# JGI-Bioinformatics/Kmernator

Measured on AMD Instinct MI355X. Metric: total k-mers/sec at k=31, 150 bp reads (spectrum build, inputs resident in HBM), higher is better.
Workload: dtype u64

## Files before the change

kmernator_amd/csrc/kmr_api.hip:

```cpp
#include <hip/hip_runtime.h>
#include <dlfcn.h>
#include <unistd.h>
#include <rccl/rccl.h>

#include <algorithm>
#include <atomic>
#include <cmath>
#include <cstdio>
#include <cstdlib>
#include <cstring>
#include <cctype>
#include <memory>
#include <mutex>
#include <string>
#include <type_traits>
#include <vector>

#include "../../include/kmernator_amd.h"
#include "kmr_kernels.hpp"
#include "kmr_partition.hpp"
#include "kmr_ingest.hpp"
#include "kmr_artifact.hpp"
#include "kmr_select.hpp"
#include "kmr_pairs.hpp"
#include "kmr_dedup.hpp"
#include "kmr_dump.hpp"
#include "kmr_superkmer.hpp"
#include "kmr_buckets.hpp"
#include "kmr_synth.hpp"
#define KMR_INSTANCES_EXTERN
#include "kmr_instances.hpp"

using namespace kmr;

namespace {

std::string g_create_error;

thread_local char g_oom_note[160] = "";
std::atomic<long long> g_blocks_live{0};
hipError_t dev_malloc(void **p, size_t bytes) {
	hipError_t e = hipMalloc(p, bytes);
	if (e == hipSuccess) { if (*p) g_blocks_live++; return e; }
	if (e != hipErrorOutOfMemory) return e;
	size_t fr = 0, tot = 0;
	for (int attempt = 0; attempt < 6; attempt++) {
		(void)hipGetLastError();
		hipDeviceSynchronize();
		if (hipMemGetInfo(&fr, &tot) != hipSuccess || bytes > tot) break;
		usleep(20000u << attempt);
		e = hipMalloc(p, bytes);
		if (e == hipSuccess && *p) g_blocks_live++;
		if (e != hipErrorOutOfMemory) return e;
	}
	(void)hipGetLastError();
	hipMemGetInfo(&fr, &tot);
	snprintf(g_oom_note, sizeof(g_oom_note), " [requested %.3f GB; device has %.3f GB free of %.3f GB]", bytes / 1e9, fr / 1e9, tot / 1e9);
	*p = nullptr;
	return hipErrorOutOfMemory;
}

class DevBuf {
public:
	DevBuf() = default;
	DevBuf(DevBuf &&o) noexcept : p_(o.p_), cap_(o.cap_) { o.p_ = nullptr; o.cap_ = 0; }
	DevBuf &operator=(DevBuf &&o) noexcept { if (this != &o) { reset(); std::swap(p_, o.p_); std::swap(cap_, o.cap_); } return *this; }
	~DevBuf() { reset(); }
	void reset() { if (p_) { hipFree(p_); g_blocks_live--; } p_ = nullptr; cap_ = 0; }
	hipError_t alloc(size_t bytes) {
		reset();
		void *p = nullptr;
		const hipError_t e = dev_malloc(&p, bytes);
		if (e == hipSuccess) { p_ = p; cap_ = bytes; }
		return e;
	}
	int reserve(kmr_handle *h, const char *what, size_t need, size_t bytes = 0);
	template <class T = void> T *get() const { return (T *)p_; }
	size_t cap() const { return cap_; }
	explicit operator bool() const { return p_ != nullptr; }
private:
	void *p_ = nullptr;
	size_t cap_ = 0;
};

struct DevMap {
	uint64_t nb = 0, n = 0;
	DevBuf start;
	DevBuf keys;
	DevBuf vals;
	DevBuf sweight;
	DevBuf spkt;
	DevBuf image;
	bool present = false;
};

struct HostPool {
	DevBuf base, chunk_list, chunk_count, head;
	uint32_t cap = 0; size_t chunk_bytes = 0;
	uint64_t used_ub = 0;
	uint64_t presize = 0;
};

struct HandleMem {
	DevBuf slots, extslots;
	DevBuf dP, dstats, derr;
	DevMap weak, sing;
	DevBuf ix_start, ix_keys, ix_counts;
	DevBuf scratch_stats;
	DevBuf adopt_buf;
	DevBuf trk;
	DevBuf scan_sums;
	DevBuf score_buf;
	DevBuf lut;
	DevBuf dPk;
	DevBuf d_uni;
	DevBuf qrange;
	DevBuf sk_fine_state;
	struct Early { bool active = false; uint64_t hi = 0; uint32_t min_depth = 0; DevBuf ue, cursor, fc, err; } early;
	DevBuf dedup_tab;
	DevBuf xo_dev;
};
struct BuildMem {
	DevBuf sk_state;
	HostPool l1;
	DevBuf work_counter;
	DevBuf l1_state; bool l1_state_dirty = false;
	DevBuf arena; size_t arena_used = 0, arena_want = 0; std::vector<DevBuf> arena_overflow;
	DevBuf linear;
	DevBuf tile_count, kcap, koff;
	DevBuf ucnt, ufirst, u_start, u_end, u_read, umax;
	DevBuf tb_bases, tb_quals, tb_rel, tb_off, tb_len;
	uint64_t tb_quals_filled = 0; int tb_quals_char = -1;
	DevBuf tb_stage[2][8];
	DevBuf uw_keys, uw_vals, us_keys, us_b8, us_pkt;
	DevBuf ue, ue2;
};
struct ExchangeMem {
	DevBuf xc_small, xc_dcounts;
	DevBuf xc_send, xc_send2, xc_recv, xc_recv2;
};

}

struct Tuning {
	uint64_t target_list = 2048;
	uint64_t sub_batch_bases = 0;
	int recycle = -1;
	int part_blocks = 0;
	double entry_share = -1.0;
	double early_entry_share = -1.0;
	uint64_t saturated_batch_bytes = 0;
	bool no_lut = false, no_narrow = false, no_l1_state = false, no_stream_lookups = false;
	uint64_t long_list_chunks = 0;
	uint64_t binned_min = 1ull << 18;
	uint64_t twobit_piece_bases = 0;
	uint64_t list_aim = 0;
	bool pow2_lists = false;
	bool no_packed_direct = false;
	bool no_uniform_count = false;
	bool no_lean_extract = false;
	bool exchange_fail_once = false;
	uint64_t dump_piece_bytes = 0;
	bool dump_timing = false;
	bool select_timing = false;
	bool pairs_timing = false;
	bool dedup_timing = false;
	uint32_t pair_hash_bits = 64;
	bool no_coarse_lists = true;
};

struct kmr_handle : HandleMem, BuildMem, ExchangeMem {
	kmr_config cfg;
	Tuning tune;
	uint32_t k = 0, kb = 0, hkb = 0, W = 0;
	bool ext = false;
	int device = 0, ncu = 0;
	hipStream_t stream = nullptr;
	std::string err;
	uint32_t log2cap = 0;
	uint64_t occupied = 0;
	uint64_t pending_kmers = 0;
	uint64_t stream_base = 0, reads = 0;
	uint64_t nb_weak = 0, nb_sing = 0;
	bool finalized = false, has_singletons = true;
	kmr_handle *subtract = nullptr;
	uint64_t subtracted = 0;
	kmr_stats stats;
	bool partition_mode = false;
	bool superkmer_mode = false;
	uint64_t ix_lists = 0, ix_gen = ~0ull;
	uint64_t trk_n = 0; std::vector<uint64_t> trk_elems;
	long trk_next = 128; uint64_t trk_raw = 0, trk_good = 0; std::vector<unsigned long long> trk_bounds; std::vector<uint64_t> trk_snap_raw, trk_snap_good;
	bool sk_fast_div = false;
	bool sender_launch = false;
	bool sk_exchange = false;
	bool auto_mode = false;
	int bits1 = 0;
	uint64_t inserted_records = 0;
	uint64_t call_bases_hint = 0;
	uint32_t lut_log2 = 0;
	uint64_t lut_gen = ~0ull, map_gen = 0;
	hipStream_t tb_copy_stream = nullptr; hipEvent_t tb_ready[2] = {nullptr, nullptr}, tb_consumed[2] = {nullptr, nullptr}; bool tb_set_used[2] = {false, false};
	const SkPacked *packed_direct = nullptr;
	int uniform_q_hint = -1;
	uint32_t sk_bits = 0, sk_m = 0, sk_off = 0, sk_win = 0;
	double hP[256], hPk[256];
	uint32_t sk_uni_w = 0xffffffffu; bool sk_uni_mixed = false; bool last_count_uniform = false;
	uint32_t peer_uni_w = 0xffffffffu; bool peer_uni_mixed = false, peers_declare = false;
	uint64_t xr_lo = 0, xr_hi = ~0ull;
	uint64_t last_early_hi = 0, last_early_entries = 0;
	bool last_early_overflowed = false;
	double last_score_ms = 0, last_select_ms = 0, last_write_ms = 0;
	double last_dump_size_ms = 0, last_dump_write_ms = 0;
	double last_pairs_ms = 0, last_pairs_parse_ms = 0, last_pairs_sort_ms = 0;
	double last_dedup_ms = 0, last_dedup_key_ms = 0, last_dedup_sort_ms = 0, last_dedup_consensus_ms = 0;
	uint64_t last_pair_hash_collisions = 0;
	uint64_t last_saturated_keys = 0, last_saturated_batches = 0;
	bool qual_mixed = false;
	uint32_t sk_fine_shift = 0;
	uint32_t sk_min_override = 0;
	uint64_t xo_segcap = 0; std::vector<uint64_t> xo_counts; const void *xo_batch = nullptr; uint64_t xo_first = 0;
	void *xc_comm = nullptr; kmr_transport xc_tr = {nullptr, nullptr, nullptr};
	uint64_t xc_job_bases = 0, xc_bytes_to_peers = 0;
	hipEvent_t ev0 = nullptr, ev1 = nullptr;
	double ms[KMR_TIME_GROUPS] = {0};
	uint64_t launches[KMR_TIME_GROUPS] = {0};
	std::vector<std::pair<hipEvent_t, hipEvent_t> > pending_events[KMR_TIME_GROUPS];
};

struct kmr_picks {
	int device = 0;
	DevBuf text, picked;
	uint64_t n = 0, n_picked = 0, bytes = 0;
};

struct kmr_pairs {
	int device = 0;
	DevBuf mate, read1, read2;
	uint64_t n = 0, n_pairs = 0, n_full = 0, n_seq = 0, n_conflicts = 0;
};

struct kmr_text {
	int device = 0;
	DevBuf text;
	uint64_t kept = 0, bytes = 0;
};

struct kmr_dedup {
	int device = 0;
	DevBuf disc, group_first, group_size, names;
	kmr_reads *cons = nullptr;
	uint64_t n = 0, n_groups = 0, affected = 0, name_bytes = 0;
	uint64_t skipped[4] = {0, 0, 0, 0};
};

struct kmr_reads {
	int device = 0;
	DevBuf bases, quals;
	DevBuf offsets;
	DevBuf name_off, name_len;
	uint64_t n = 0, total = 0, filtered = 0;
	uint32_t input_base = 0;
};

namespace {

std::string oom_note() { std::string s(g_oom_note); g_oom_note[0] = 0; return s; }

std::string hip_err_text(hipError_t e) { return std::string(hipGetErrorString(e)) + (e == hipErrorOutOfMemory ? oom_note() : std::string()); }

#define HIPCHK(h, call) do { hipError_t e_ = (call); if (e_ != hipSuccess) { \
	(h)->err = std::string(#call) + ": " + hip_err_text(e_); \
	return e_ == hipErrorOutOfMemory ? KMR_ERR_OOM : KMR_ERR_HIP; } } while (0)

int DevBuf::reserve(kmr_handle *h, const char *what, size_t need, size_t bytes) {
	if (p_ && cap_ >= need) return 0;
	if (!bytes) bytes = need;
	hipError_t e = p_ ? hipStreamSynchronize(h->stream) : hipSuccess;
	if (e == hipSuccess) e = alloc(bytes);
	if (e == hipSuccess) return 0;
	h->err = std::string("device buffer ") + what + " (" + std::to_string(bytes) + " bytes): " + hip_err_text(e);
	return e == hipErrorOutOfMemory ? KMR_ERR_OOM : KMR_ERR_HIP;
}

#ifdef KMR_DEBUG_HOOKS
bool dbg() { static const bool d = getenv("KMR_DEBUG") != nullptr; return d; }
#else
constexpr bool dbg() { return false; }
#endif

int fail(kmr_handle *h, int code, const std::string &msg) { const std::string m = code == KMR_ERR_OOM ? msg + oom_note() : msg; if (h) h->err = m; else g_create_error = m; return code; }

uint64_t min_pow2(uint64_t n) {
	uint64_t p = n;
	if (p == 0) p = 1;
	else if ((p & (p - 1)) != 0) { p--; for (size_t i = 1; i < 64; i <<= 1) p |= p >> i; p++; }
	return p;
}
uint64_t resize_buckets(uint64_t n) { if (n > 67108864ull) n = 67108864ull; return min_pow2(n); }

void quality_table(double P[256], unsigned minQ, unsigned startChar) {
	for (int raw = 0; raw < 256; raw++) {
		int i = raw - (int)startChar + 33;
		if (i < 33 + (int)minQ) P[raw] = 0.0;
		else if (i < 103) P[raw] = 1.0 - pow(10.0, ((33 - i) / 10.0));
		else P[raw] = 1.0;
	}
}

template <int N> using int_c = std::integral_constant<int, N>;
template <class F> auto with_w(const kmr_handle *h, F &&f) {
	switch (h->W) { case 1: return f(int_c<1>()); case 2: return f(int_c<2>()); case 3: return f(int_c<3>()); default: return f(int_c<4>()); }
}
template <class F> auto with_w_ext(const kmr_handle *h, F &&f) {
	return with_w(h, [&](auto W) { return h->ext ? f(W, std::true_type()) : f(W, std::false_type()); });
}
template <int W, class F> auto with_win(uint32_t win, F &&f) {
	if (W > 1 && win == 32) return f(int_c<(W > 1 ? 32 : 16)>());
	return win == 16 ? f(int_c<16>()) : (win == 8 ? f(int_c<8>()) : f(int_c<4>()));
}

size_t slot_bytes(kmr_handle *h) { return with_w(h, [](auto W) { return sizeof(Slot<W()>); }); }

ReadsView reads_view(const void *bases, const void *quals, const void *offsets, uint64_t n_reads, const void *discarded = nullptr, uint64_t stream_base = 0, uint64_t first_read_idx = 0) {
	ReadsView rv{};
	rv.bases = (const uint8_t *)bases; rv.quals = (const uint8_t *)quals; rv.offsets = (const uint64_t *)offsets; rv.discarded = (const uint8_t *)discarded;
	rv.n_reads = n_reads; rv.stream_base = stream_base; rv.first_read_idx = first_read_idx;
	return rv;
}
ReadsView reads_slice(const ReadsView &all, uint64_t r, uint64_t m) {
	ReadsView rv = all;
	rv.offsets = all.offsets + r; rv.n_reads = m; rv.discarded = all.discarded ? all.discarded + r : nullptr; rv.first_read_idx = all.first_read_idx + r;
	return rv;
}
FinalizeParams finalize_params(kmr_handle *h, uint32_t min_depth) {
	FinalizeParams f{};
	f.kb = h->hkb; f.ext_min_q = h->cfg.ext_min_quality; f.min_depth = min_depth; f.has_singletons = h->cfg.separate_singletons ? 1 : 0; f.nb_weak = h->nb_weak; f.nb_sing = h->nb_sing;
	return f;
}

DevParams dev_params(kmr_handle *h) {
	DevParams p;
	p.k = h->k; p.kb = h->hkb; p.min_weight = h->cfg.min_weight; p.fastq_start = h->cfg.fastq_start_char; p.ext_min_q = h->cfg.ext_min_quality;
	p.qzero = h->cfg.fastq_start_char + std::max<uint32_t>(1u, h->cfg.min_quality_score);
	p.subsample = h->cfg.kmer_subsample; p.rank = h->cfg.rank; p.world = h->cfg.world_size; p.num_parts = h->cfg.num_parts; p.part_idx = h->cfg.part_idx;
	p.count_sender_bad = h->sender_launch ? 1u : 0u;
	p.P = h->dP.get<double>(); p.stats = h->dstats.get<DevStats>(); p.err = h->derr.get<uint32_t>();
	p.sub_wstart = p.sub_wkeys = p.sub_sstart = p.sub_skeys = nullptr; p.sub_wvals = nullptr; p.sub_sweight = nullptr; p.sub_wnb = p.sub_snb = 0; p.sub_vw = 0;
	if (h->subtract) {
		const kmr_handle *o = h->subtract;
		if (o->weak.present && o->weak.n) { p.sub_wstart = o->weak.start.get<uint64_t>(); p.sub_wkeys = o->weak.keys.get<uint64_t>(); p.sub_wvals = o->weak.vals.get<uint32_t>(); p.sub_wnb = o->weak.nb; p.sub_vw = o->ext ? 15 : 3; }
		if (o->sing.present && o->sing.n) { p.sub_sstart = o->sing.start.get<uint64_t>(); p.sub_skeys = o->sing.keys.get<uint64_t>(); p.sub_sweight = o->sing.sweight.get<uint8_t>(); p.sub_snb = o->sing.nb; }
	}
	return p;
}

int grid_for(uint64_t n, int block = 256, int maxBlocks = 256 * 16) {
	uint64_t g = (n + block - 1) / block;
	if (g < 1) g = 1;
	if (g > (uint64_t)maxBlocks) g = maxBlocks;
	return (int)g;
}

// ... 4 lines not shown
	HIPCHK(h, hipGetLastError());
	return 0;
}
int clear_table_any(kmr_handle *h, void *slots, ExtSlot *ext, uint32_t log2cap) { return with_w(h, [&](auto W) { return clear_table<W()>(h, slots, ext, log2cap); }); }

int alloc_table(kmr_handle *h, uint32_t log2cap, DevBuf &slots, DevBuf &ext) {
	DevBuf s, x;
	HIPCHK(h, s.alloc(slot_bytes(h) << log2cap));
	if (h->ext) HIPCHK(h, x.alloc(sizeof(ExtSlot) << log2cap));
	const int rc = clear_table_any(h, s.get(), x.get<ExtSlot>(), log2cap);
	if (rc) return rc;
	slots = std::move(s); ext = std::move(x);
	return 0;
}

int sync_state(kmr_handle *h) {
	HIPCHK(h, hipStreamSynchronize(h->stream));
	for (int which = 0; which < KMR_TIME_GROUPS; which++) {
		for (auto &pr : h->pending_events[which]) {
			float ms = 0; hipEventElapsedTime(&ms, pr.first, pr.second);
			h->ms[which] += ms; h->launches[which]++;
			hipEventDestroy(pr.first); hipEventDestroy(pr.second);
		}
		h->pending_events[which].clear();
	}
	uint32_t e = 0; DevStats s;
	HIPCHK(h, hipMemcpy(&e, h->derr.get<uint32_t>(), sizeof(e), hipMemcpyDeviceToHost));
	HIPCHK(h, hipMemcpy(&s, h->dstats.get<DevStats>(), sizeof(s), hipMemcpyDeviceToHost));
#ifdef KMR_DEBUG_HOOKS
	if (h->superkmer_mode) { if (dbg()) fprintf(stderr, "sk_extract windows: %llu general, %llu fast\n", s.claimed, s.inserted); s.claimed = 0; s.inserted = 0; }
#endif
	h->stats.raw_kmers = s.raw + s.inserted + s.sender_bad; h->stats.raw_good_kmers = s.good + s.inserted; h->stats.discarded = s.raw - s.good + s.sender_bad;
	h->occupied = s.claimed; h->pending_kmers = 0; h->subtracted = s.subtracted;
	if (e & ERR_READ_TOO_LONG) return fail(h, KMR_ERR_UNSUPPORTED, "a read is longer than the per-wavefront LDS tile (" + std::to_string(TILE_SPAN) + " bases)");
	if (e & ERR_TABLE_FULL) return fail(h, KMR_ERR_CAPACITY, "device k-mer table is full; raise kmr_config.max_table_entries / estimated_raw_kmers");
	if (e & ERR_SEGMENT_OVERFLOW) return fail(h, KMR_ERR_CAPACITY, "an owner segment overflowed seg_capacity");
	if (e & ERR_POOL_FULL) return fail(h, KMR_ERR_CAPACITY, "record pool overflow (internal sizing error)");
	if (e & ERR_ENTRIES_FULL) return fail(h, KMR_ERR_CAPACITY, "entry buffer overflow (internal sizing error)");
	return 0;
}

template <int W, bool EXT> int grow_table_t(kmr_handle *h, uint32_t newlog) {
	DevBuf ns, ne;
	int rc = alloc_table(h, newlog, ns, ne);
	if (rc) return rc;
	Table<W> src = table_of<W>(h), dst; dst.slots = ns.get<Slot<W>>(); dst.ext = ne.get<ExtSlot>(); dst.log2cap = newlog;
	hipLaunchKernelGGL((rehash_kernel<W, EXT>), dim3(grid_for(1ull << h->log2cap)), dim3(256), 0, h->stream, src, dst, h->hkb, h->derr.get<uint32_t>());
	HIPCHK(h, hipGetLastError());
	HIPCHK(h, hipStreamSynchronize(h->stream));
	h->slots = std::move(ns); h->extslots = std::move(ne); h->log2cap = newlog;
	return 0;
}
int grow_table(kmr_handle *h, uint32_t newlog) { return with_w_ext(h, [&](auto W, auto EXT) { return grow_table_t<W(), EXT()>(h, newlog); }); }

int ensure_capacity(kmr_handle *h, uint64_t incoming) {
	const uint64_t cap = 1ull << h->log2cap;
	if ((double)(h->occupied + h->pending_kmers + incoming) <= 0.85 * (double)cap) { h->pending_kmers += incoming; return 0; }
	int rc = sync_state(h);
	if (rc) return rc;
	if ((double)(h->occupied + incoming) > 0.85 * (double)cap) {
		uint32_t nl = h->log2cap;
		while ((double)(h->occupied + incoming) > 0.6 * (double)(1ull << nl)) nl++;
		rc = grow_table(h, nl);
		if (rc) return rc;
	}
	h->pending_kmers = incoming;
	return 0;
}

void time_begin(kmr_handle *h, int which, hipEvent_t *a, hipEvent_t *b) {
	hipEventCreate(a); hipEventCreate(b);
	hipEventRecord(*a, h->stream);
	(void)which;
}
void time_end(kmr_handle *h, int which, hipEvent_t a, hipEvent_t b) {
	hipEventRecord(b, h->stream);
	h->pending_events[which].push_back(std::make_pair(a, b));
}

const size_t EXTRACT_SMEM = (size_t)WAVES_PER_BLOCK * 2 * TILE_BUF;

int exclusive_scan(kmr_handle *h, const uint32_t *in, uint64_t n, uint64_t *out);

int prepare_units(kmr_handle *h, ReadsView &rv, uint32_t span = (uint32_t)TILE_SPAN) {
	rv.u_start = rv.u_end = rv.u_read = nullptr; rv.n_units = 0;
	const uint64_t n = rv.n_reads;
	if (n == 0) return 0;
	int rc = h->umax.reserve(h, "umax", 4); if (rc) return rc;
	HIPCHK(h, hipMemsetAsync(h->umax.get<unsigned int>(), 0, 4, h->stream));
	rc = h->ucnt.reserve(h, "ucnt", 4 * (n + 1)); if (rc) return rc;
	hipLaunchKernelGGL(unit_count_kernel, dim3(grid_for(n)), dim3(256), 0, h->stream, rv.offsets, n, h->k, span, h->ucnt.get<uint32_t>(), h->umax.get<unsigned int>());
	HIPCHK(h, hipGetLastError());
	unsigned int mx = 0;
	HIPCHK(h, hipMemcpyAsync(&mx, h->umax.get<unsigned int>(), 4, hipMemcpyDeviceToHost, h->stream));
	HIPCHK(h, hipStreamSynchronize(h->stream));
	if (mx <= span) return 0;
	rc = h->ufirst.reserve(h, "ufirst", 8 * (n + 1)); if (rc) return rc;
	rc = exclusive_scan(h, h->ucnt.get<uint32_t>(), n, h->ufirst.get<uint64_t>()); if (rc) return rc;
	uint64_t U = 0;
	HIPCHK(h, hipMemcpy(&U, h->ufirst.get<uint64_t>() + n, 8, hipMemcpyDeviceToHost));
	if (h->u_read.cap() < 8 * U) {
		h->u_start.reset(); h->u_end.reset(); h->u_read.reset();
		HIPCHK(h, h->u_start.alloc(8 * U)); HIPCHK(h, h->u_end.alloc(8 * U)); HIPCHK(h, h->u_read.alloc(8 * U));
	}
	hipLaunchKernelGGL(unit_fill_kernel, dim3(grid_for(n)), dim3(256), 0, h->stream, rv.offsets, n, h->k, span, h->ufirst.get<uint64_t>(), h->u_start.get<uint64_t>(), h->u_end.get<uint64_t>(), h->u_read.get<uint64_t>());
	HIPCHK(h, hipGetLastError());
	rv.u_start = h->u_start.get<uint64_t>(); rv.u_end = h->u_end.get<uint64_t>(); rv.u_read = h->u_read.get<uint64_t>(); rv.n_units = U;
	return 0;
}

template <int W, bool EXT, class Op> int launch_extract(kmr_handle *h, const ReadsView &rv, const Op &op, uint64_t max_blocks = 0) {
	const DevParams dp = dev_params(h);
	const bool sub = Op::NEEDS_WEIGHT && (dp.sub_wnb | dp.sub_snb) != 0;
	auto kern = sub ? extract_kernel<W, EXT, Op, true> : extract_kernel<W, EXT, Op, false>;
	HIPCHK(h, hipFuncSetAttribute((const void *)kern, hipFuncAttributeMaxDynamicSharedMemorySize, (int)EXTRACT_SMEM));
	if (dbg()) { int nb = 0; hipOccupancyMaxActiveBlocksPerMultiprocessor(&nb, (const void *)kern, WAVES_PER_BLOCK * 64, EXTRACT_SMEM); fprintf(stderr, "extract: %d blocks of %d waves per CU (dynamic LDS %zu)\n", nb, WAVES_PER_BLOCK, EXTRACT_SMEM);
		for (size_t tr : {(size_t)79872, (size_t)65536, (size_t)52000, (size_t)38000}) { hipOccupancyMaxActiveBlocksPerMultiprocessor(&nb, (const void *)kern, WAVES_PER_BLOCK * 64, tr); fprintf(stderr, "   with %zu bytes: %d blocks\n", tr, nb); } }
	const uint64_t tiles = ((rv.u_start ? rv.n_units : rv.n_reads) + 63) / 64;
	uint64_t blocks = (tiles + WAVES_PER_BLOCK - 1) / WAVES_PER_BLOCK;
	if (blocks == 0) return 0;
	if (max_blocks && blocks > max_blocks) blocks = max_blocks;
	if (blocks > 0x7fffffffull) return fail(h, KMR_ERR_INVALID_ARG, "too many reads in one batch");
	hipLaunchKernelGGL(kern, dim3((unsigned)blocks), dim3(WAVES_PER_BLOCK * 64), EXTRACT_SMEM, h->stream, rv, dp, op);
	HIPCHK(h, hipGetLastError());
	return 0;
}

template <int W, bool EXT> int add_reads_dev_t(kmr_handle *h, const ReadsView &rvAll, uint64_t total_bases) {
	const uint64_t n = rvAll.n_reads;
	const uint64_t avg = n ? std::max<uint64_t>(1, total_bases / n) : 1;
	uint64_t chunk = std::max<uint64_t>(64, ((1ull << 27) / avg) & ~63ull);
	std::vector<uint64_t> off2(2);
	for (uint64_t r = 0; r < n; r += chunk) {
		const uint64_t m = std::min(chunk, n - r);
		HIPCHK(h, hipMemcpyAsync(&off2[0], rvAll.offsets + r, 8, hipMemcpyDeviceToHost, h->stream));
		HIPCHK(h, hipMemcpyAsync(&off2[1], rvAll.offsets + r + m, 8, hipMemcpyDeviceToHost, h->stream));
		HIPCHK(h, hipStreamSynchronize(h->stream));
		const uint64_t bases = off2[1] - off2[0];
		int rc = ensure_capacity(h, bases);
		if (rc) return rc;
		ReadsView rv = reads_slice(rvAll, r, m);
		rc = prepare_units(h, rv); if (rc) return rc;
		InsertOp<W, EXT> op; op.table = table_of<W>(h);
		hipEvent_t a, b; time_begin(h, 0, &a, &b);
		rc = launch_extract<W, EXT>(h, rv, op);
		time_end(h, 0, a, b);
		if (rc) return rc;
	}
	return 0;
}

int add_reads_dev_any(kmr_handle *h, const ReadsView &rv, uint64_t total_bases) { return with_w_ext(h, [&](auto W, auto EXT) { return add_reads_dev_t<W(), EXT()>(h, rv, total_bases); }); }

int exclusive_scan(kmr_handle *h, const uint32_t *in, uint64_t n, uint64_t *out ) {
	const uint64_t nblocks = (n + SCAN_ITEMS - 1) / SCAN_ITEMS;
	const size_t eb = sizeof(unsigned long long);
	int rc = h->scan_sums.reserve(h, "scan_sums", eb * (nblocks + 1), eb * std::max<uint64_t>(nblocks + 1, 4096)); if (rc) return rc;
	unsigned long long *sums = h->scan_sums.get<unsigned long long>(), *total = sums + nblocks;
	hipLaunchKernelGGL(scan_block_sums_kernel, dim3((unsigned)nblocks), dim3(256), 0, h->stream, in, n, sums);
	hipLaunchKernelGGL(scan_sums_kernel, dim3(1), dim3(256), 0, h->stream, sums, nblocks, total);
	hipLaunchKernelGGL(scan_apply_kernel, dim3((unsigned)nblocks), dim3(256), 0, h->stream, in, n, sums, out);
	HIPCHK(h, hipGetLastError());
	HIPCHK(h, hipStreamSynchronize(h->stream));
	return 0;
}

int arena_alloc(kmr_handle *h, void **out, size_t bytes) {
	const size_t need = (bytes + 255) & ~(size_t)255;
	if (h->arena && h->arena_used + need <= h->arena.cap()) { *out = h->arena.get<uint8_t>() + h->arena_used; h->arena_used += need; h->arena_want += need; return 0; }
	h->arena_want += need;
	DevBuf b;
	HIPCHK(h, b.alloc(std::max<size_t>(need, 256)));
	*out = b.get();
	h->arena_overflow.push_back(std::move(b));
	return 0;
}
int arena_reset(kmr_handle *h) {
	HIPCHK(h, hipStreamSynchronize(h->stream));
	h->arena_overflow.clear();
	if (h->arena_want > h->arena.cap()) {
		if (h->arena.alloc(h->arena_want + h->arena_want / 8 + (1 << 20)) != hipSuccess) (void)hipGetLastError();
	}
	h->arena_used = 0; h->arena_want = 0;
	return 0;
}
template <class T> int arena_get(kmr_handle *h, T **out, size_t count) { return arena_alloc(h, (void **)out, count * sizeof(T)); }

void clear_map(DevMap &m) { m.image.reset(); m.n = 0; m.present = false; }


template <int W> MapView<W> view_of(const DevMap &m, uint32_t vw) {
	MapView<W> v; v.start = m.start.get<uint64_t>(); v.keys = m.keys.get<uint64_t>(); v.vals = m.vals.get<uint32_t>(); v.sweight = m.sweight.get<uint8_t>(); v.nb = m.present ? m.nb : 0; v.vw = vw;
	return v;
}

template <int W, bool EXT> int finalize_t(kmr_handle *h, uint32_t min_depth) {
	int rc = sync_state(h);
	if (rc) return rc;
	hipEvent_t ea, eb; time_begin(h, 1, &ea, &eb);
	const FinalizeParams f = finalize_params(h, min_depth);
	const bool keepSing = f.has_singletons && min_depth <= 1;
	DevBuf wcb, scb, fcb;
	HIPCHK(h, wcb.alloc(4 * h->nb_weak)); HIPCHK(h, scb.alloc(4 * h->nb_sing)); HIPCHK(h, fcb.alloc(sizeof(FinalizeCounters)));
	uint32_t *wc = wcb.get<uint32_t>(), *sc = scb.get<uint32_t>(); FinalizeCounters *fc = fcb.get<FinalizeCounters>();
	HIPCHK(h, hipMemsetAsync(wc, 0, 4 * h->nb_weak, h->stream)); HIPCHK(h, hipMemsetAsync(sc, 0, 4 * h->nb_sing, h->stream)); HIPCHK(h, hipMemsetAsync(fc, 0, sizeof(FinalizeCounters), h->stream));
	Table<W> t = table_of<W>(h);
	const int g = grid_for(1ull << h->log2cap);
	hipLaunchKernelGGL(classify_kernel<W>, dim3(g), dim3(256), 0, h->stream, t, f, wc, sc, fc);
	HIPCHK(h, hipGetLastError());
	FinalizeCounters c;
	HIPCHK(h, hipMemcpyAsync(&c, fc, sizeof(c), hipMemcpyDeviceToHost, h->stream));
	HIPCHK(h, hipStreamSynchronize(h->stream));
	h->stats.unique_kmers = c.unique;
	h->stats.singleton_kmers = f.has_singletons ? c.singletons : 0;
	DevMap &wm = h->weak, &sm = h->sing;
	wm = DevMap(); sm = DevMap();
	wm.nb = h->nb_weak; wm.n = c.weak_kept; wm.present = true;
	sm.nb = h->nb_sing; sm.n = c.sing_kept; sm.present = keepSing;
	const uint32_t vw = EXT ? 15 : 3;
	HIPCHK(h, wm.start.alloc(8 * (wm.nb + 1))); HIPCHK(h, sm.start.alloc(8 * (sm.nb + 1)));
	rc = exclusive_scan(h, wc, wm.nb, wm.start.get<uint64_t>()); if (rc) return rc;
	rc = exclusive_scan(h, sc, sm.nb, sm.start.get<uint64_t>()); if (rc) return rc;
	HIPCHK(h, wm.keys.alloc(std::max<uint64_t>(8, 8ull * W * wm.n))); HIPCHK(h, wm.vals.alloc(std::max<uint64_t>(8, 4ull * vw * wm.n)));
	HIPCHK(h, sm.keys.alloc(std::max<uint64_t>(8, 8ull * W * sm.n))); HIPCHK(h, sm.sweight.alloc(std::max<uint64_t>(8, sm.n)));
	if (EXT) HIPCHK(h, sm.spkt.alloc(std::max<uint64_t>(8, 4ull * sm.n)));
	HIPCHK(h, hipMemsetAsync(wc, 0, 4 * h->nb_weak, h->stream)); HIPCHK(h, hipMemsetAsync(sc, 0, 4 * h->nb_sing, h->stream));
	hipLaunchKernelGGL((scatter_kernel<W, EXT>), dim3(g), dim3(256), 0, h->stream, t, f, wm.start.get<uint64_t>(), wc, wm.keys.get<uint64_t>(), wm.vals.get<uint32_t>(), sm.start.get<uint64_t>(), sc, sm.keys.get<uint64_t>(), sm.sweight.get<uint8_t>(), sm.spkt.get<uint32_t>());
	HIPCHK(h, hipGetLastError());
	SortView<W> sv; sv.keys = wm.keys.get<uint64_t>(); sv.vals = wm.vals.get<uint32_t>(); sv.b8 = nullptr; sv.pkt = nullptr; sv.vw = vw;
	hipLaunchKernelGGL((sort_buckets_kernel<W, EXT ? 15 : 3>), dim3(grid_for(wm.nb, 4, 1 << 20)), dim3(256), 0, h->stream, sv, wm.start.get<uint64_t>(), wm.nb);
	if (sm.n) {
		SortView<W> ss; ss.keys = sm.keys.get<uint64_t>(); ss.vals = nullptr; ss.b8 = sm.sweight.get<uint8_t>(); ss.pkt = sm.spkt.get<uint32_t>(); ss.vw = 0;
		hipLaunchKernelGGL((sort_buckets_kernel<W, 0>), dim3(grid_for(sm.nb, 4, 1 << 20)), dim3(256), 0, h->stream, ss, sm.start.get<uint64_t>(), sm.nb);
	}
	HIPCHK(h, hipGetLastError());
	time_end(h, 1, ea, eb);
	HIPCHK(h, hipStreamSynchronize(h->stream));
	h->has_singletons = keepSing;
	if (!keepSing) { sm.n = 0; }
	h->stats.weak_entries = wm.n; h->stats.singleton_entries = keepSing ? sm.n : 0;
	h->finalized = true; h->map_gen++;
	return sync_state(h);
}

template <int W> int build_image_t(kmr_handle *h, DevMap &m, bool weakMap) {
	if (m.image) return 0;
	const uint32_t vw = h->ext ? 15 : 3;
	const uint32_t vbytes = weakMap ? (h->ext ? 60 : 12) : (h->ext ? 5 : 1);
	HIPCHK(h, m.image.alloc(8 * (2 + m.nb) + 4 * m.nb + m.n * (h->kb + vbytes)));
	hipLaunchKernelGGL(image_header_kernel, dim3(grid_for(m.nb)), dim3(256), 0, h->stream, m.image.get<uint8_t>(), m.start.get<uint64_t>(), m.nb, h->kb, vbytes);
	if (m.n) hipLaunchKernelGGL(image_entries_kernel<W>, dim3(grid_for(m.n)), dim3(256), 0, h->stream, m.image.get<uint8_t>(), m.start.get<uint64_t>(), m.nb, h->kb, vbytes,
	                           m.keys.get<uint64_t>(), weakMap ? m.vals.get<uint32_t>() : nullptr, vw, m.sweight.get<uint8_t>(), m.spkt.get<uint32_t>(), m.n);
	HIPCHK(h, hipGetLastError());
	HIPCHK(h, hipStreamSynchronize(h->stream));
	return 0;
}
int build_image(kmr_handle *h, DevMap &m, bool weakMap) { return with_w(h, [&](auto W) { return build_image_t<W()>(h, m, weakMap); }); }

template <int W> int load_image_t(kmr_handle *h, DevMap &m, bool weakMap, const uint8_t *src, uint64_t len) {
	if (len < 16) return fail(h, KMR_ERR_INVALID_ARG, "image too short");
	uint64_t nb, mask; memcpy(&nb, src, 8); memcpy(&mask, src + 8, 8);
	if (nb == 0 || (nb & (nb - 1)) || mask != nb - 1 || len < 8 * (2 + nb) + 4 * nb) return fail(h, KMR_ERR_INVALID_ARG, "bad image header");
	const uint32_t vw = h->ext ? 15 : 3;
	const uint32_t vbytes = weakMap ? (h->ext ? 60 : 12) : (h->ext ? 5 : 1);
	if ((len - 8 * (2 + nb) - 4 * nb) % (h->kb + vbytes) != 0) return fail(h, KMR_ERR_INVALID_ARG, "image size does not match k / value type");
	m = DevMap();
	m.nb = nb; m.n = (len - 8 * (2 + nb) - 4 * nb) / (h->kb + vbytes); m.present = true;
	const uint64_t *offs = (const uint64_t *)(src + 16);
	uint64_t expect = 8 * (2 + nb);
	for (uint64_t b = 0; b < nb; b++) {
		if (offs[b] != expect || expect + 4 > len) return fail(h, KMR_ERR_INVALID_ARG, "image offsets are not the packed store() layout");
		uint32_t cnt; memcpy(&cnt, src + expect, 4);
		expect += 4 + (uint64_t)cnt * (h->kb + vbytes);
		if (expect > len) return fail(h, KMR_ERR_INVALID_ARG, "image bucket runs past the end");
	}
	if (expect != len) return fail(h, KMR_ERR_INVALID_ARG, "image length mismatch");
	HIPCHK(h, m.image.alloc(len));
	HIPCHK(h, hipMemcpy(m.image.get<uint8_t>(), src, len, hipMemcpyHostToDevice));
	{
		DevBuf counts; HIPCHK(h, counts.alloc(4 * nb));
		hipLaunchKernelGGL(image_counts_kernel, dim3(grid_for(nb)), dim3(256), 0, h->stream, m.image.get<uint8_t>(), nb, counts.get<uint32_t>());
		HIPCHK(h, m.start.alloc(8 * (nb + 1)));
		int rc = exclusive_scan(h, counts.get<uint32_t>(), nb, m.start.get<uint64_t>()); if (rc) return rc;
	}
	HIPCHK(h, m.keys.alloc(std::max<uint64_t>(8, 8ull * W * m.n)));
	if (weakMap) HIPCHK(h, m.vals.alloc(std::max<uint64_t>(8, 4ull * vw * m.n)));
	else { HIPCHK(h, m.sweight.alloc(std::max<uint64_t>(8, m.n))); if (h->ext) HIPCHK(h, m.spkt.alloc(std::max<uint64_t>(8, 4 * m.n))); }
	if (m.n) hipLaunchKernelGGL(image_unpack_kernel<W>, dim3(grid_for(m.n)), dim3(256), 0, h->stream, m.image.get<uint8_t>(), m.start.get<uint64_t>(), nb, h->kb, vbytes, m.keys.get<uint64_t>(), m.vals.get<uint32_t>(), vw, m.sweight.get<uint8_t>(), m.spkt.get<uint32_t>(), m.n);
	SortView<W> sv; sv.keys = m.keys.get<uint64_t>(); sv.vals = m.vals.get<uint32_t>(); sv.b8 = m.sweight.get<uint8_t>(); sv.pkt = m.spkt.get<uint32_t>(); sv.vw = weakMap ? vw : 0;
	if (!weakMap) hipLaunchKernelGGL((sort_buckets_kernel<W, 0>), dim3(grid_for(nb, 4, 1 << 20)), dim3(256), 0, h->stream, sv, m.start.get<uint64_t>(), nb);
	else if (h->ext) hipLaunchKernelGGL((sort_buckets_kernel<W, 15>), dim3(grid_for(nb, 4, 1 << 20)), dim3(256), 0, h->stream, sv, m.start.get<uint64_t>(), nb);
	else hipLaunchKernelGGL((sort_buckets_kernel<W, 3>), dim3(grid_for(nb, 4, 1 << 20)), dim3(256), 0, h->stream, sv, m.start.get<uint64_t>(), nb);
	HIPCHK(h, hipGetLastError());
	HIPCHK(h, hipStreamSynchronize(h->stream));
	m.image.reset();

	return 0;
}

template <int W, int VW> void launch_sort(kmr_handle *h, DevMap &m, bool weakMap) {
	SortView<W> sv; sv.keys = m.keys.get<uint64_t>(); sv.vals = weakMap ? m.vals.get<uint32_t>() : nullptr; sv.b8 = m.sweight.get<uint8_t>(); sv.pkt = m.spkt.get<uint32_t>(); sv.vw = weakMap ? VW : 0;
	hipLaunchKernelGGL((sort_buckets_kernel<W, VW>), dim3(grid_for(m.nb, 4, 1 << 20)), dim3(256), 0, h->stream, sv, m.start.get<uint64_t>(), m.nb);
}
template <int W> int merge_image_t(kmr_handle *h, DevMap &m, bool weakMap, const uint8_t *src, uint64_t len) {
	DevMap t;
	int rc = load_image_t<W>(h, t, weakMap, src, len);
	if (rc) return rc;
	if (t.nb != m.nb) return fail(h, KMR_ERR_INVALID_ARG, "Can not merge two maps of differing sizes (src/Kmer.h:3210)");
	const uint32_t vw = h->ext ? 15 : 3;
	DevMap d; d.nb = m.nb; d.n = m.n + t.n; d.present = true;
	DevBuf countsb, dupb;
	HIPCHK(h, countsb.alloc(4 * m.nb)); HIPCHK(h, dupb.alloc(4));
	uint32_t *counts = countsb.get<uint32_t>(), *dup = dupb.get<uint32_t>();
	HIPCHK(h, hipMemsetAsync(dup, 0, 4, h->stream));
	HIPCHK(h, d.start.alloc(8 * (m.nb + 1)));
// ... 40 lines not shown
	return 0;
}

template <int W> LutView<W> lut_of(kmr_handle *h) {
	LutView<W> v; v.slots = nullptr; v.mask = 0; v.shift = 0;
	if (h->tune.no_lut || !h->weak.present || h->weak.n == 0) return v;
	if (!(h->lut && h->lut_gen == h->map_gen)) {
		uint32_t l2 = 10; while ((1ull << l2) < 2 * h->weak.n) l2++;
		const size_t bytes = (size_t)(W + 1) * 8 << l2;
		if (h->lut.cap() < bytes) {
			if (h->lut) { hipStreamSynchronize(h->stream); h->lut.reset(); }
			size_t fr = 0, tot = 0;
			if (hipMemGetInfo(&fr, &tot) != hipSuccess || fr < bytes + (1ull << 30) || h->lut.alloc(bytes) != hipSuccess) { (void)hipGetLastError(); return v; }
		}

		const uint32_t vw = h->ext ? 15 : 3;
		hipLaunchKernelGGL(lut_clear_kernel, dim3(4096), dim3(256), 0, h->stream, h->lut.get<uint64_t>(), 1ull << l2, (uint32_t)(W + 1));
		hipLaunchKernelGGL(lut_build_kernel<W>, dim3(grid_for(h->weak.n)), dim3(256), 0, h->stream, view_of<W>(h->weak, vw), h->weak.n, h->lut.get<uint64_t>(), (1ull << l2) - 1, 64 - l2, h->hkb);
		if (hipGetLastError() != hipSuccess) return v;
		h->lut_log2 = l2; h->lut_gen = h->map_gen;
	}
	v.slots = h->lut.get<uint64_t>(); v.mask = (1ull << h->lut_log2) - 1; v.shift = 64 - h->lut_log2;
	return v;
}

template <int W> int lookup_reads_t(kmr_handle *h, const ReadsView &rv, uint32_t *dout, const uint64_t *dout_off, bool weak_only = false) {
	LookupOp<W> op; const uint32_t vw = h->ext ? 15 : 3; op.weak_only = weak_only;
	op.lut = weak_only ? lut_of<W>(h) : LutView<W>{nullptr, 0, 0};
	op.weak = view_of<W>(h->weak, vw); op.sing = view_of<W>(h->sing, vw); op.out = dout; op.out_offsets = dout_off; op.first_read_idx = rv.first_read_idx;
	return launch_extract<W, false>(h, rv, op);
}
template <int W> int lookup_reads_weighted_t(kmr_handle *h, const ReadsView &rv, double *dout, const uint64_t *dout_off) {
	LookupWeightOp<W> op; const uint32_t vw = h->ext ? 15 : 3;
	op.weak = view_of<W>(h->weak, vw); op.sing = view_of<W>(h->sing, vw); op.out = dout; op.out_offsets = dout_off; op.first_read_idx = rv.first_read_idx;
	return launch_extract<W, false>(h, rv, op);
}

int stage_reads(kmr_handle *h, const char *bases, const uint64_t *offsets, uint64_t n, DevBuf &b, DevBuf &o) {
	const uint64_t total = n ? offsets[n] - offsets[0] : 0;
	HIPCHK(h, b.alloc(total + 64)); HIPCHK(h, o.alloc(8 * (n + 1)));
	HIPCHK(h, hipMemcpyAsync(b.get(), bases + (n ? offsets[0] : 0), total, hipMemcpyHostToDevice, h->stream));
	std::vector<uint64_t> rel(n + 1);
	for (uint64_t i = 0; i <= n; i++) rel[i] = n ? offsets[i] - offsets[0] : 0;
	HIPCHK(h, hipMemcpyAsync(o.get(), rel.data(), 8 * (n + 1), hipMemcpyHostToDevice, h->stream));
	HIPCHK(h, hipStreamSynchronize(h->stream));
	return 0;
}


#define TARGET_LIST_RECORDS (h->tune.target_list)
const double MAX_LIST_DISTINCT = 600.0;
const uint64_t L2_ITEM_CHUNKS = 16384;
const uint64_t SUB_BATCH_BASES = 1ull << 30;

size_t rec_bytes(kmr_handle *h) { return h->superkmer_mode ? 16 : 8 * h->W + (h->ext ? 16 : 8); }
uint64_t key_entries(kmr_handle *h, const DevBuf &keys) { return keys.cap() / (8ull * h->W); }
uint64_t packed_entries(kmr_handle *h, const DevBuf &ue) { return ue.cap() / (8ull * (h->W + 1)); }
int max_part_bits(kmr_handle *h) { return rec_bytes(h) <= 24 ? 10 : 9; }
PoolView pool_view(kmr_handle *h, HostPool &p) { PoolView v; v.base = p.base.get<uint8_t>(); v.chunk_list = p.chunk_list.get<uint32_t>(); v.chunk_count = p.chunk_count.get<uint32_t>(); v.head = p.head.get<unsigned int>(); v.cap = p.cap; v.err = h->derr.get<uint32_t>(); return v; }
uint32_t part_rot(kmr_handle *h) { uint32_t r = 0; while ((1ull << (r + 1)) <= h->nb_weak) r++; return r; }
template <int W, bool EXT, int LEVEL> int launch_partition(kmr_handle *h, const PartSource<W> &S, HostPool &pool, int grid, int bits, int shift) {
	auto kern = partition_direct_kernel<W, EXT, LEVEL, PD_THREADS, PD_RPT, PD_LINE>;
	const size_t smem = partition_direct_smem_bytes<W, EXT, PD_THREADS, PD_RPT, PD_LINE>(bits);
	if (dbg()) fprintf(stderr, "partition level %d W=%d bits=%d shift=%d smem=%zu grid=%d\n", LEVEL, W, bits, shift, smem, grid);
	HIPCHK(h, hipFuncSetAttribute((const void *)kern, hipFuncAttributeMaxDynamicSharedMemorySize,
	                              (int)partition_direct_smem_bytes<W, EXT, PD_THREADS, PD_RPT, PD_LINE>(max_part_bits(h))));
	hipLaunchKernelGGL(kern, dim3(grid), dim3(PD_THREADS), smem, h->stream, S, pool_view(h, pool), h->work_counter.get<unsigned int>(), bits, shift);
	HIPCHK(h, hipGetLastError());
	return 0;
}

int pool_reserve(kmr_handle *h, HostPool &p, uint64_t extra, bool keep) {
	unsigned int used = 0;
	if (!keep) p.used_ub = 0;
	if (p.head && keep) {
		if (p.base && p.used_ub + extra + 64 <= p.cap) { p.used_ub += extra; return 0; }
		HIPCHK(h, hipStreamSynchronize(h->stream)); HIPCHK(h, hipMemcpy(&used, p.head.get<unsigned int>(), 4, hipMemcpyDeviceToHost)); if (used > p.cap) used = p.cap;
	}
	p.used_ub = (uint64_t)used + extra;
	const uint64_t need = (uint64_t)used + extra + 64;
	if (need >= 0xffffffffull) return fail(h, KMR_ERR_CAPACITY, "record pool would exceed 2^32 chunks");
	if (!p.head) { HIPCHK(h, p.head.alloc(4)); HIPCHK(h, hipMemset(p.head.get(), 0, 4)); }
	if (!keep) HIPCHK(h, hipMemsetAsync(p.head.get<unsigned int>(), 0, 4, h->stream));
	if (need <= p.cap) return 0;
	uint64_t ncap = keep && used ? need + need / 4 : need;
	if (p.presize && need + p.presize < 0xffffffffull) ncap = std::max(ncap, need + p.presize);
	p.presize = 0;
	p.chunk_bytes = (size_t)CH * rec_bytes(h);
	DevBuf nb, nl, nc;
	HIPCHK(h, nb.alloc(ncap * p.chunk_bytes));
	HIPCHK(h, nl.alloc(4 * ncap)); HIPCHK(h, nc.alloc(4 * ncap));
	if (used) {
		HIPCHK(h, hipMemcpy(nb.get(), p.base.get(), (size_t)used * p.chunk_bytes, hipMemcpyDeviceToDevice));
		HIPCHK(h, hipMemcpy(nl.get(), p.chunk_list.get(), 4ull * used, hipMemcpyDeviceToDevice));
		HIPCHK(h, hipMemcpy(nc.get(), p.chunk_count.get(), 4ull * used, hipMemcpyDeviceToDevice));
		HIPCHK(h, hipDeviceSynchronize());
	}
	p.base = std::move(nb); p.chunk_list = std::move(nl); p.chunk_count = std::move(nc); p.cap = (uint32_t)ncap;
	return 0;
}


int zero_work_counter(kmr_handle *h) {
	int rc = h->work_counter.reserve(h, "work_counter", 4); if (rc) return rc;
	HIPCHK(h, hipMemsetAsync(h->work_counter.get<unsigned int>(), 0, 4, h->stream));
	return 0;
}

int num_cus(kmr_handle *h) {
	if (h->ncu <= 0) {
		hipDeviceProp_t pr; h->ncu = 256;
		if (hipGetDeviceProperties(&pr, h->device) == hipSuccess) h->ncu = pr.multiProcessorCount;
	}
	return h->ncu;
}
int part_grid(kmr_handle *h) { return num_cus(h) * 2; }
int partition_blocks(kmr_handle *h) { return h->tune.part_blocks > 0 ? h->tune.part_blocks : num_cus(h); }

template <int W, bool EXT> int ensure_l1_state(kmr_handle *h) {
	const size_t stride = partition_state_bytes<W, EXT, PD_LINE>(h->bits1), need = stride * (size_t)partition_blocks(h);
	if (h->l1_state.cap() == need) return 0;
	if (h->l1_state) HIPCHK(h, hipStreamSynchronize(h->stream));
	HIPCHK(h, h->l1_state.alloc(need));
	hipLaunchKernelGGL(partition_state_init_kernel, dim3(partition_blocks(h)), dim3(256), 0, h->stream, h->l1_state.get<uint8_t>(), stride, h->bits1, (uint32_t)partition_blocks(h));
	HIPCHK(h, hipGetLastError());
	h->l1_state_dirty = false;
	return 0;
}
template <int W, bool EXT> int flush_l1_state(kmr_handle *h) {
	if (!h->l1_state || !h->l1_state_dirty) return 0;
	int rc = pool_reserve(h, h->l1, (uint64_t)partition_blocks(h) * ((1ull << h->bits1) + 512) + 64, true); if (rc) return rc;
	rc = zero_work_counter(h); if (rc) return rc;
	PartSource<W> S; memset(&S, 0, sizeof(S));
	S.kb = h->hkb; S.rot = part_rot(h); S.state = h->l1_state.get<uint8_t>(); S.state_final = 1;
	rc = launch_partition<W, EXT, 1>(h, S, h->l1, partition_blocks(h), h->bits1, 0);
	h->l1_state_dirty = false;
	return rc;
}

template <int W, bool EXT> int partition_level1(kmr_handle *h, const void *linear, const uint64_t *ext_start, const uint32_t *ext_count,
                                      uint64_t n_ext, uint32_t ext_stride, uint64_t ext_len, uint64_t total, uint64_t max_records,
                                      unsigned long long *valid_counter = nullptr, uint32_t packed_words = 0, uint64_t ordinal_base = 0) {
	if (n_ext == 0) return 0;
	const int grid = (int)std::min<uint64_t>(partition_blocks(h), n_ext);
	if (!h->l1.base) {
		const uint64_t est = std::max<uint64_t>(max_records, h->cfg.estimated_raw_kmers / std::max<uint32_t>(1, h->cfg.world_size));
		const uint64_t launches = est / std::max<uint64_t>(1, max_records) + 2;
		const uint64_t l2_allowance = (est / CH / L2_ITEM_CHUNKS + (1ull << h->bits1) + 1) * (1ull << max_part_bits(h)) + (uint64_t)part_grid(h) * 512;
		{
			const uint64_t chunks = est / CH + launches * (uint64_t)grid * ((1ull << h->bits1) + 512) + 64 + l2_allowance;
			size_t mfree = 0, mtotal = 0;
			if (hipMemGetInfo(&mfree, &mtotal) == hipSuccess && (double)mfree < (double)chunks * CH * rec_bytes(h) * 1.02 + (double)(2ull << 30)) {
				HIPCHK(h, hipStreamSynchronize(h->stream));
				h->uw_keys.reset(); h->uw_vals.reset(); h->us_keys.reset(); h->us_b8.reset(); h->us_pkt.reset(); h->ue.reset(); h->ue2.reset();
			}
		}
		uint64_t want = est / CH + launches * (uint64_t)grid * ((1ull << h->bits1) + 512) + 64 + l2_allowance;
		{
			size_t mfree = 0, mtotal = 0;
			const double twice = (double)(want + est / CH) * CH * rec_bytes(h) * 1.02;
			if (hipMemGetInfo(&mfree, &mtotal) == hipSuccess && twice + (double)(8ull << 30) < (double)mfree * 0.5) want += est / CH;
		}
		int rc0 = pool_reserve(h, h->l1, want, true);
		if (rc0) return rc0;
	}
	int rc = pool_reserve(h, h->l1, max_records / CH + (uint64_t)grid * ((1ull << h->bits1) + 512) + 64, true);
	if (rc) return rc;
	rc = zero_work_counter(h); if (rc) return rc;
	PartSource<W> S; memset(&S, 0, sizeof(S));
	S.linear = linear; S.ext_start = ext_start; S.ext_count = ext_count; S.n_ext = n_ext; S.ext_stride = ext_stride; S.ext_len = ext_len; S.total = total;
	S.valid_counter = valid_counter; S.kb = h->hkb; S.rot = part_rot(h); S.packed_words = packed_words; S.ordinal_base = ordinal_base;
	if (!h->tune.no_l1_state) {
		rc = ensure_l1_state<W, EXT>(h); if (rc) return rc;
		S.state = h->l1_state.get<uint8_t>(); S.state_final = 0; h->l1_state_dirty = true;
	}
	hipEvent_t ta, tb; time_begin(h, KMR_TIME_PARTITION1, &ta, &tb);
	rc = launch_partition<W, EXT, 1>(h, S, h->l1, grid, h->bits1, 0);
	time_end(h, KMR_TIME_PARTITION1, ta, tb);
	return rc;
}

void choose_bits1(kmr_handle *h, uint64_t records_hint) {
	uint64_t est = std::max<uint64_t>(records_hint, h->cfg.estimated_raw_kmers / std::max<uint32_t>(1, h->cfg.world_size));
	const int mb = max_part_bits(h);
	int T = 0; while (T < 2 * mb && (est >> T) > TARGET_LIST_RECORDS) T++;
	h->bits1 = std::max(0, std::min(mb, T + 2 - mb));
}

template <int W, bool EXT> int extract_by_owner_t(kmr_handle *h, const ReadsView &rvAll, uint64_t total_bases, void *dev_records, uint64_t seg_capacity, void *dev_seg_counts, uint32_t *dev_pos = nullptr) {
	const uint64_t n = rvAll.n_reads;
	const uint64_t avg = n ? std::max<uint64_t>(1, total_bases / n) : 1;
	const uint64_t chunk = std::max<uint64_t>(64, (SUB_BATCH_BASES / avg) & ~63ull);
	for (uint64_t r = 0; r < n; r += chunk) {
		const uint64_t m = std::min(chunk, n - r);
		ReadsView rv = reads_slice(rvAll, r, m);
		int rc = prepare_units(h, rv); if (rc) return rc;
		const uint64_t nu = rv.u_start ? rv.n_units : m;
		rc = h->kcap.reserve(h, "kcap", 4 * std::max<uint64_t>(nu + 1, 16)); if (rc) return rc;
		rc = h->koff.reserve(h, "koff", 8 * std::max<uint64_t>(nu + 1, 16)); if (rc) return rc;
		hipLaunchKernelGGL(kmer_capacity_kernel, dim3(grid_for(nu)), dim3(256), 0, h->stream, rv, h->k, h->kcap.get<uint32_t>());
		HIPCHK(h, hipGetLastError());
		rc = exclusive_scan(h, h->kcap.get<uint32_t>(), nu, h->koff.get<uint64_t>()); if (rc) return rc;
		uint64_t total_cap = 0;
		HIPCHK(h, hipMemcpy(&total_cap, h->koff.get<uint64_t>() + nu, 8, hipMemcpyDeviceToHost));
		const uint64_t tiles = (nu + 63) / 64;
		rc = h->linear.reserve(h, "linear", sizeof(typename PoolRec<W, EXT>::type) * std::max<uint64_t>(total_cap, 16)); if (rc) return rc;
		rc = h->tile_count.reserve(h, "tile_count", 4 * std::max<uint64_t>(tiles, 16)); if (rc) return rc;
		LinearOp<W, EXT, false> op; op.records = (typename PoolRec<W, EXT>::type *)h->linear.get(); op.koff = h->koff.get<uint64_t>(); op.tile_count = h->tile_count.get<uint32_t>(); op.first_read_idx = rv.first_read_idx;
		h->sender_launch = dev_pos == nullptr;
		rc = launch_extract<W, EXT>(h, rv, op);
		h->sender_launch = false;
		if (rc) return rc;
		rc = zero_work_counter(h); if (rc) return rc;
		const int grid = (int)std::min<uint64_t>((uint64_t)num_cus(h) * 8, tiles);
		OwnerFn of; of.m = 0; of.off = of.win = of.list_bits = 0;
		if (h->superkmer_mode && h->sk_exchange) { of.m = h->sk_m; of.off = h->sk_off; of.win = h->sk_win; of.list_bits = h->sk_bits; }
		if (dev_pos)
			hipLaunchKernelGGL((owner_scatter_kernel<W, EXT, true>), dim3(grid), dim3(OWNER_THREADS), 0, h->stream, (const typename PoolRec<W, EXT>::type *)h->linear.get(), h->koff.get<uint64_t>(), h->tile_count.get<uint32_t>(), tiles, h->hkb,
			                   h->cfg.world_size, (uint32_t *)dev_records, seg_capacity, (unsigned long long *)dev_seg_counts, h->work_counter.get<unsigned int>(), h->derr.get<uint32_t>(), dev_pos, of);
		else
			hipLaunchKernelGGL((owner_scatter_kernel<W, EXT>), dim3(grid), dim3(OWNER_THREADS), 0, h->stream, (const typename PoolRec<W, EXT>::type *)h->linear.get(), h->koff.get<uint64_t>(), h->tile_count.get<uint32_t>(), tiles, h->hkb,
			                   h->cfg.world_size, (uint32_t *)dev_records, seg_capacity, (unsigned long long *)dev_seg_counts, h->work_counter.get<unsigned int>(), h->derr.get<uint32_t>(), (uint32_t *)nullptr, of);
		HIPCHK(h, hipGetLastError());
	}
	return 0;
}

template <int W, bool EXT> int add_reads_partition_t(kmr_handle *h, const ReadsView &rvAll, uint64_t total_bases) {
	const uint64_t n = rvAll.n_reads;
	if (!h->l1.head) choose_bits1(h, total_bases);
	const uint64_t avg = n ? std::max<uint64_t>(1, total_bases / n) : 1;
	const uint64_t sub_bases = h->tune.sub_batch_bases ? h->tune.sub_batch_bases : SUB_BATCH_BASES;
	const uint64_t chunk = std::max<uint64_t>(64, (sub_bases / avg) & ~63ull);
	for (uint64_t r = 0; r < n; r += chunk) {
		const uint64_t m = std::min(chunk, n - r);
		ReadsView rv = reads_slice(rvAll, r, m);
		int rc = prepare_units(h, rv); if (rc) return rc;
		const uint64_t nu = rv.u_start ? rv.n_units : m;
		rc = h->kcap.reserve(h, "kcap", 4 * std::max<uint64_t>(nu + 1, 16)); if (rc) return rc;
		rc = h->koff.reserve(h, "koff", 8 * std::max<uint64_t>(nu + 1, 16)); if (rc) return rc;
		hipLaunchKernelGGL(kmer_capacity_kernel, dim3(grid_for(nu)), dim3(256), 0, h->stream, rv, h->k, h->kcap.get<uint32_t>());
		HIPCHK(h, hipGetLastError());
		rc = exclusive_scan(h, h->kcap.get<uint32_t>(), nu, h->koff.get<uint64_t>()); if (rc) return rc;
		uint64_t total_cap = 0;
		HIPCHK(h, hipMemcpy(&total_cap, h->koff.get<uint64_t>() + nu, 8, hipMemcpyDeviceToHost));
		const uint64_t tiles = (nu + 63) / 64;
		rc = h->linear.reserve(h, "linear", rec_bytes(h) * std::max<uint64_t>(total_cap, 16)); if (rc) return rc;
		rc = h->tile_count.reserve(h, "tile_count", 4 * std::max<uint64_t>(tiles, 16)); if (rc) return rc;
		LinearOp<W, EXT> op; op.records = (typename PoolRec<W, EXT>::type *)h->linear.get(); op.koff = h->koff.get<uint64_t>(); op.tile_count = h->tile_count.get<uint32_t>(); op.first_read_idx = rv.first_read_idx;
		hipEvent_t a, b, a2, b2; time_begin(h, KMR_TIME_BUILD, &a, &b);
		time_begin(h, KMR_TIME_EXTRACT, &a2, &b2);
		rc = launch_extract<W, EXT>(h, rv, op);
		time_end(h, KMR_TIME_EXTRACT, a2, b2);
#ifdef KMR_DEBUG_HOOKS
		if (!rc && getenv("KMR_DEBUG_SAME_TILE")) {
			const uint64_t distinct = std::max<uint64_t>(1, strtoull(getenv("KMR_DEBUG_SAME_TILE"), nullptr, 10));
			hipLaunchKernelGGL(same_tile_kernel, dim3(grid_for(tiles)), dim3(256), 0, h->stream, h->koff.get<uint64_t>(), tiles, distinct, total_cap / std::max<uint64_t>(tiles, 1));
		}
#endif
		if (!rc) rc = partition_level1<W, EXT>(h, h->linear.get(), h->koff.get<uint64_t>(), h->tile_count.get<uint32_t>(), tiles, 64, 0, 0, total_cap);
		time_end(h, KMR_TIME_BUILD, a, b);
		if (rc) return rc;
	}
	return 0;
}
int add_reads_partition(kmr_handle *h, const ReadsView &rv, uint64_t total_bases) { return with_w_ext(h, [&](auto W, auto EXT) { return add_reads_partition_t<W(), EXT()>(h, rv, total_bases); }); }

int build_csr(kmr_handle *h, HostPool &p, uint64_t nl, uint32_t first, uint64_t **list_start, uint64_t **list_chunks, uint32_t *n_chunks_out) {
	unsigned int used = 0;
	HIPCHK(h, hipStreamSynchronize(h->stream));
	HIPCHK(h, hipMemcpy(&used, p.head.get<unsigned int>(), 4, hipMemcpyDeviceToHost));
	if (used > p.cap) used = p.cap;
	used = used > first ? used - first : 0;
	uint32_t *cnt;
	{ int arc = arena_get(h, &cnt, nl); if (arc) return arc; arc = arena_get(h, list_start, nl + 1); if (arc) return arc;
	  arc = arena_get(h, list_chunks, std::max<unsigned>(used, 1)); if (arc) return arc; }
	HIPCHK(h, hipMemsetAsync(cnt, 0, 4 * nl, h->stream));
	const unsigned csr_grid = (unsigned)(((uint64_t)used + CSR_THREADS * CSR_ITEMS - 1) / (CSR_THREADS * CSR_ITEMS));
	if (used) hipLaunchKernelGGL(chunk_hist_kernel, dim3(csr_grid), dim3(CSR_THREADS), 0, h->stream, p.chunk_list.get<uint32_t>() + first, used, cnt, (uint32_t)nl);
	int rc = exclusive_scan(h, cnt, nl, *list_start); if (rc) return rc;
	HIPCHK(h, hipMemsetAsync(cnt, 0, 4 * nl, h->stream));
	if (used) hipLaunchKernelGGL(chunk_scatter_kernel, dim3(csr_grid), dim3(CSR_THREADS), 0, h->stream, p.chunk_list.get<uint32_t>() + first, p.chunk_count.get<uint32_t>() + first, used, first, *list_start, cnt, *list_chunks, (uint32_t)nl);
	HIPCHK(h, hipGetLastError());
	*n_chunks_out = used;
	if (dbg()) {
		unsigned long long hv[2] = {0, 0};
		DevBuf db; HIPCHK(h, db.alloc(16)); HIPCHK(h, hipMemset(db.get(), 0, 16));
		unsigned long long *d = db.get<unsigned long long>();
		if (used) hipLaunchKernelGGL(pool_records_kernel, dim3(grid_for(used)), dim3(256), 0, h->stream, p.chunk_list.get<uint32_t>(), p.chunk_count.get<uint32_t>(), used, d, d + 1);
		HIPCHK(h, hipStreamSynchronize(h->stream));
		HIPCHK(h, hipMemcpy(hv, d, 16, hipMemcpyDeviceToHost));
		fprintf(stderr, "build_csr: lists %llu chunks %u valid %llu records %llu (expected %llu)\n", (unsigned long long)nl, used, hv[1], hv[0], (unsigned long long)h->stats.raw_good_kmers);
		unsigned long long vv[3] = {0, 0, 0};
		int bits = 0; while ((1ull << bits) < nl) bits++;
		DevBuf vb; HIPCHK(h, vb.alloc(24)); HIPCHK(h, hipMemset(vb.get(), 0, 24));
		unsigned long long *v = vb.get<unsigned long long>();
		PoolView pvw = pool_view(h, p);
		with_w_ext(h, [&](auto W, auto EXT) { hipLaunchKernelGGL((verify_lists_kernel<W(), EXT()>), dim3(4096), dim3(256), 0, h->stream, pvw, *list_start, *list_chunks, nl, bits, h->hkb, part_rot(h), v, v + 1, v + 2); });
		HIPCHK(h, hipStreamSynchronize(h->stream));
		HIPCHK(h, hipMemcpy(vv, v, 24, hipMemcpyDeviceToHost));
		fprintf(stderr, "verify_lists: records via CSR %llu misfiled %llu zero-weight %llu\n", vv[0], vv[1], vv[2]);
	}
	return 0;
}

int finish_maps_from_entries(kmr_handle *h, uint32_t *wc, uint32_t *sc, uint64_t wslots, uint64_t sslots, uint64_t wn, uint64_t sn, bool keepSing, bool weak_uncounted = false);
CountOut count_out(kmr_handle *h, bool packed, unsigned long long *cursors, uint32_t *wc, uint32_t *sc, FinalizeCounters *fc);
// ... 34 lines not shown
		if (dbg()) fprintf(stderr, "distinct probe: %llu records, %llu distinct (%llu repeated) -> shares %.3f %.3f\n", hpr[0], hpr[1], hpr[2], distinct_share, repeated_share);
	}
	const int mb = max_part_bits(h);
	int T = 0; while (T < 40 && ((G >> T) > TARGET_LIST_RECORDS || (double)(G >> T) * distinct_share > MAX_LIST_DISTINCT)) T++;
	T = std::min(T, 28);
	int cur_bits = h->bits1;
	uint64_t *ls2 = ls1, *lc2 = lc1;
	uint32_t valid_from = 0;
	for (int level = 2; cur_bits < T; level++) {
		const int nbits = std::min(mb, T - cur_bits);
		const uint64_t nl_prev = 1ull << cur_bits;
		std::vector<uint64_t> hs(nl_prev + 1);
		HIPCHK(h, hipMemcpy(hs.data(), ls2, 8 * (nl_prev + 1), hipMemcpyDeviceToHost));
		std::vector<uint64_t> ib, ie; std::vector<uint32_t> il;
		for (uint64_t l = 0; l < nl_prev; l++) {
			const uint64_t nch = hs[l + 1] - hs[l];
			if (!nch) continue;
			const uint64_t nit = (nch + L2_ITEM_CHUNKS - 1) / L2_ITEM_CHUNKS, per = (nch + nit - 1) / nit;
			for (uint64_t c = hs[l]; c < hs[l + 1]; c += per) { ib.push_back(c); ie.push_back(std::min(hs[l + 1], c + per)); il.push_back((uint32_t)l); }
		}
		if (ib.empty()) { cur_bits += nbits; rc = build_csr(h, h->l1, 1ull << cur_bits, valid_from, &ls2, &lc2, &nch1); if (rc) return rc; continue; }
		const uint64_t partials = ib.size() * (1ull << nbits) + (uint64_t)part_grid(h) * 512 + 64;
		unsigned int head_before = 0;
		HIPCHK(h, hipMemcpy(&head_before, h->l1.head.get<unsigned int>(), 4, hipMemcpyDeviceToHost));
		const bool recycle = h->tune.recycle >= 0 ? h->tune.recycle != 0 : (uint64_t)head_before + G / CH + partials + 64 > h->l1.cap;
		h->l1.used_ub = head_before;
		rc = pool_reserve(h, h->l1, (recycle ? 0 : G / CH) + partials, true); if (rc) return rc;
		uint64_t *dib, *die; uint32_t *dil;
		rc = arena_get(h, &dib, ib.size()); if (rc) return rc; rc = arena_get(h, &die, ie.size()); if (rc) return rc; rc = arena_get(h, &dil, il.size()); if (rc) return rc;
		HIPCHK(h, hipMemcpyAsync(dib, ib.data(), 8 * ib.size(), hipMemcpyHostToDevice, h->stream)); HIPCHK(h, hipMemcpyAsync(die, ie.data(), 8 * ie.size(), hipMemcpyHostToDevice, h->stream));
		HIPCHK(h, hipMemcpyAsync(dil, il.data(), 4 * il.size(), hipMemcpyHostToDevice, h->stream));
		rc = zero_work_counter(h); if (rc) return rc;
		PartSource<W> S; memset(&S, 0, sizeof(S));
		S.src = pool_view(h, h->l1); S.list_chunks = lc2; S.item_begin = dib; S.item_end = die; S.item_list = dil; S.n_items = ib.size(); S.kb = h->hkb; S.rot = part_rot(h);
		S.recycle = recycle ? 1 : 0;
		const int grid = (int)std::min<uint64_t>(partition_blocks(h), ib.size());
		if (dbg()) fprintf(stderr, "level %d: %d bits after %d, %zu items, %s\n", level, nbits, cur_bits, ib.size(), recycle ? "recycling chunks" : "fresh chunks");
		hipEvent_t ta, tb; time_begin(h, KMR_TIME_PARTITION2, &ta, &tb);
		rc = launch_partition<W, EXT, 2>(h, S, h->l1, grid, nbits, cur_bits);
		time_end(h, KMR_TIME_PARTITION2, ta, tb);
		if (rc) return rc;
		HIPCHK(h, hipStreamSynchronize(h->stream));
		cur_bits += nbits;
		if (!recycle) valid_from = head_before;
		rc = build_csr(h, h->l1, 1ull << cur_bits, valid_from, &ls2, &lc2, &nch1); if (rc) return rc;
	}
	const uint64_t nl2 = 1ull << cur_bits;
	const int count_log2s = (!EXT && (double)(G >> cur_bits) * distinct_share > MAX_LIST_DISTINCT) ? 11 : COUNT_LOG2S;
	if (dbg()) fprintf(stderr, "count pass: %llu lists of ~%llu records, table 2^%d\n", (unsigned long long)nl2, (unsigned long long)(G >> cur_bits), count_log2s);
	const uint32_t vw = EXT ? 15 : 3;
	const uint64_t slack = (uint64_t)part_grid(h) * 8 * 8192 + 16;
	const uint64_t wbound = f.has_singletons ? G / 2 : G, sbound = keepSing ? G : 0;
	const uint64_t wmax = wbound + wbound / 8 + slack, smax = keepSing ? sbound + sbound / 8 + slack : 16;
	uint64_t wcap = std::min<uint64_t>(wmax, (uint64_t)((double)G * (f.has_singletons ? repeated_share : distinct_share) * 1.5) + G / 64 + slack);
	uint64_t scap = keepSing ? std::min<uint64_t>(smax, (uint64_t)((double)G * std::max(0.0, distinct_share - repeated_share) * 1.5) + G / 64 + slack) : 16;
	if (h->tune.entry_share >= 0) {
		const double sh = h->tune.entry_share;
		wcap = std::min<uint64_t>(wmax, (uint64_t)((double)G * sh) + 16384); if (keepSing) scap = std::min<uint64_t>(smax, (uint64_t)((double)G * sh) + 16384);
		h->uw_keys.reset(); h->uw_vals.reset(); h->us_keys.reset(); h->us_b8.reset(); h->us_pkt.reset();
	}
	wcap = std::max(wcap, key_entries(h, h->uw_keys)); scap = std::max(scap, key_entries(h, h->us_keys));
	uint32_t *wc = nullptr, *sc = nullptr; FinalizeCounters *fc = nullptr; unsigned long long *cursors = nullptr;
	rc = arena_get(h, &wc, h->nb_weak); if (rc) return rc; rc = arena_get(h, &sc, h->nb_sing); if (rc) return rc;
	rc = arena_get(h, &fc, 1); if (rc) return rc; rc = arena_get(h, &cursors, 2); if (rc) return rc;
	FinalizeCounters c; unsigned long long cur[2];
	hipEvent_t tca, tcb; time_begin(h, KMR_TIME_COUNT, &tca, &tcb);
	for (int attempt = 0; ; attempt++) {
	{
		const double need = (key_entries(h, h->uw_keys) < wcap ? (8.0 * W + 4.0 * vw) * (double)wcap : 0.0) + (key_entries(h, h->us_keys) < scap ? (8.0 * W + 1.0) * (double)scap : 0.0);
		size_t mfree = 0, mtotal = 0;
		if (need > 0 && h->linear && hipMemGetInfo(&mfree, &mtotal) == hipSuccess && (double)mfree < need + (double)G * 0.3 * (8.0 * W + 12.0) + (double)(2ull << 30)) {
			HIPCHK(h, hipStreamSynchronize(h->stream));
			h->linear.reset();
		}
	}
	if (key_entries(h, h->uw_keys) < wcap || !h->uw_vals) {
		h->uw_keys.reset(); h->uw_vals.reset();
		HIPCHK(h, h->uw_keys.alloc(8ull * W * wcap)); HIPCHK(h, h->uw_vals.alloc(4ull * vw * wcap));
	}
	if (key_entries(h, h->us_keys) < scap || !h->us_b8 || (EXT && !h->us_pkt)) {
		h->us_keys.reset(); h->us_b8.reset(); h->us_pkt.reset();
		HIPCHK(h, h->us_keys.alloc(8ull * W * scap)); HIPCHK(h, h->us_b8.alloc(scap)); if (EXT) HIPCHK(h, h->us_pkt.alloc(4 * scap));
	}
	HIPCHK(h, hipMemsetAsync(wc, 0, 4 * h->nb_weak, h->stream)); HIPCHK(h, hipMemsetAsync(sc, 0, 4 * h->nb_sing, h->stream));
	HIPCHK(h, hipMemsetAsync(fc, 0, sizeof(FinalizeCounters), h->stream)); HIPCHK(h, hipMemsetAsync(cursors, 0, 16, h->stream));
	const CountOut out = count_out(h, false, cursors, wc, sc, fc);
	rc = zero_work_counter(h); if (rc) return rc;
	#ifdef KMR_DEBUG_HOOKS
	const int count_reps = getenv("KMR_COUNT_CHECK") ? atoi(getenv("KMR_COUNT_CHECK")) : 0;
#else
	const int count_reps = 0;
#endif
	for (int cr = 0; cr <= count_reps; cr++) {
		if (cr) {
			FinalizeCounters c0; unsigned long long cur0[2];
			HIPCHK(h, hipStreamSynchronize(h->stream));
			HIPCHK(h, hipMemcpy(&c0, fc, sizeof(c0), hipMemcpyDeviceToHost)); HIPCHK(h, hipMemcpy(cur0, cursors, 16, hipMemcpyDeviceToHost));
			fprintf(stderr, "count pass %d: unique %llu singletons %llu weak_kept %llu sing_kept %llu slots %llu/%llu\n", cr - 1, (unsigned long long)c0.unique,
			        (unsigned long long)c0.singletons, (unsigned long long)c0.weak_kept, (unsigned long long)c0.sing_kept, cur0[0], cur0[1]);
			HIPCHK(h, hipMemsetAsync(wc, 0, 4 * h->nb_weak, h->stream)); HIPCHK(h, hipMemsetAsync(sc, 0, 4 * h->nb_sing, h->stream));
			HIPCHK(h, hipMemsetAsync(fc, 0, sizeof(FinalizeCounters), h->stream)); HIPCHK(h, hipMemsetAsync(cursors, 0, 16, h->stream));
			rc = zero_work_counter(h); if (rc) return rc;
		}
		const int grid = (int)std::min<uint64_t>((uint64_t)part_grid(h) * 2, nl2);
		if (count_log2s == 11) {
			rc = launch_count<W, EXT, 11>(h, grid, ls2, lc2, nl2, out, f, 0); if (rc) return rc;
		} else if (EXT && W == 1 && !h->tune.no_narrow) {
			rc = launch_count<W, EXT, COUNT_LOG2S, true>(h, grid, ls2, lc2, nl2, out, f, 1); if (rc) return rc;
			HIPCHK(h, hipGetLastError());
			rc = zero_work_counter(h); if (rc) return rc;
			hipLaunchKernelGGL(max_list_chunks_kernel, dim3(grid_for(nl2)), dim3(256), 0, h->stream, ls2, nl2, h->work_counter.get<unsigned int>());
			unsigned int longest = 0;
			HIPCHK(h, hipMemcpyAsync(&longest, h->work_counter.get<unsigned int>(), 4, hipMemcpyDeviceToHost, h->stream));
			HIPCHK(h, hipStreamSynchronize(h->stream));
			rc = zero_work_counter(h); if (rc) return rc;
			if (longest > COUNT_NARROW_CHUNKS) { rc = launch_count<W, EXT, COUNT_LOG2S>(h, std::min(grid, part_grid(h)), ls2, lc2, nl2, out, f, 2); if (rc) return rc; }
		} else {
			rc = launch_count<W, EXT, COUNT_LOG2S>(h, grid, ls2, lc2, nl2, out, f, 0); if (rc) return rc;
		}
		HIPCHK(h, hipGetLastError());
	}
	uint32_t cerr = 0;
	HIPCHK(h, hipMemcpyAsync(&c, fc, sizeof(c), hipMemcpyDeviceToHost, h->stream)); HIPCHK(h, hipMemcpyAsync(cur, cursors, 16, hipMemcpyDeviceToHost, h->stream));
	HIPCHK(h, hipMemcpyAsync(&cerr, h->derr.get<uint32_t>(), 4, hipMemcpyDeviceToHost, h->stream));
	HIPCHK(h, hipStreamSynchronize(h->stream));
	if (!(cerr & ERR_ENTRIES_FULL) || (wcap >= wmax && scap >= smax) || attempt >= 8) break;
	cerr &= ~(uint32_t)ERR_ENTRIES_FULL;
	HIPCHK(h, hipMemcpy(h->derr.get<uint32_t>(), &cerr, 4, hipMemcpyHostToDevice));
	wcap = std::min<uint64_t>(wmax, wcap * 2); if (keepSing) scap = std::min<uint64_t>(smax, scap * 2);
	if (dbg()) fprintf(stderr, "count pass: entry buffers too small, retrying with %llu / %llu\n", (unsigned long long)wcap, (unsigned long long)scap);
	}
	time_end(h, KMR_TIME_COUNT, tca, tcb);
	{
		uint32_t cerr2 = 0;
		HIPCHK(h, hipMemcpy(&cerr2, h->derr.get<uint32_t>(), 4, hipMemcpyDeviceToHost));
		if (cerr2 & ERR_ENTRIES_FULL) { time_end(h, 1, ea, eb); return fail(h, KMR_ERR_CAPACITY, "entry buffers of the count pass overflowed at their upper bound (internal sizing error)"); }
	}

	h->stats.unique_kmers = c.unique;
	h->stats.singleton_kmers = f.has_singletons ? c.singletons : 0;
	hipEvent_t tma, tmb; time_begin(h, KMR_TIME_BUCKETS, &tma, &tmb);
	rc = finish_maps_from_entries(h, wc, sc, cur[0], cur[1], c.weak_kept, c.sing_kept, keepSing);
	time_end(h, KMR_TIME_BUCKETS, tma, tmb);
	if (rc) return rc;
	time_end(h, 1, ea, eb);
	h->has_singletons = keepSing;
	h->stats.weak_entries = h->weak.n; h->stats.singleton_entries = keepSing ? h->sing.n : 0;
	h->finalized = true; h->map_gen++;
	rc = sync_state(h);
	if (!rc && !h->arena_overflow.empty()) rc = arena_reset(h);
	return rc;
}

template <int W> int binned_buckets_t(kmr_handle *h, uint64_t wslots, uint64_t wn, bool &done) {
	done = false;
	DevMap &wm = h->weak;
	const uint64_t nb = wm.nb;
	uint32_t B = 0; while ((1ull << (B + 1)) <= nb) B++;
	if (h->ext || wn < h->tune.binned_min || wn == 0 || (1ull << B) != nb || wslots >= (1ull << 40)) return 0;
	uint32_t g = 0; while (g < std::min<uint32_t>(B, BB_MAX_GROUP_BITS) && (wn >> (B - g)) < 512) g++;
	const uint32_t R = B - g;
	if (R < 1 || R > 2 * BB_MAX_BITS || (wn >> R) > 1024) return 0;
	const uint32_t bits1 = R <= (uint32_t)BB_MAX_BITS ? R : (R + 1) / 2, bits2 = R - bits1;
	const uint64_t bins1 = 1ull << bits1, groups = 1ull << R;
	uint32_t *hist1 = nullptr, *hist2 = nullptr, *pad1 = nullptr; uint64_t *start1 = nullptr, *gstart = nullptr; unsigned long long *cursor = nullptr; unsigned int *dmax = nullptr;
	int rc = arena_get(h, &hist1, bins1); if (rc) return rc;
	rc = arena_get(h, &start1, bins1 + 1); if (rc) return rc;
	rc = arena_get(h, &cursor, groups); if (rc) return rc;
	rc = arena_get(h, &dmax, 1); if (rc) return rc;
	if (bits2) { rc = arena_get(h, &hist2, groups); if (rc) return rc; rc = arena_get(h, &pad1, bins1); if (rc) return rc; rc = arena_get(h, &gstart, groups + 1); if (rc) return rc; }
	HIPCHK(h, hipMemsetAsync(hist1, 0, 4 * bins1, h->stream)); HIPCHK(h, hipMemsetAsync(dmax, 0, 4, h->stream));
	BbInput in1; in1.entries = h->ue.get<uint64_t>(); in1.seg_start = nullptr; in1.seg_count = nullptr; in1.n_seg = 1; in1.n_slots = wslots; in1.holes = 1;
	auto hist_grid = [&](uint64_t n_slots, uint32_t &tpb) { const uint64_t tiles = (n_slots + BB_TILE - 1) / BB_TILE; tpb = (uint32_t)std::max<uint64_t>(1, (tiles + 2047) / 2048); return (unsigned)((tiles + tpb - 1) / tpb); };
	auto scatter_grid = [&](uint64_t n_slots) { const uint64_t tiles = (n_slots + BB_TILE - 1) / BB_TILE; return (unsigned)std::min<uint64_t>(tiles, (uint64_t)num_cus(h) * 8); };
	auto scratch = [&](uint64_t entries) { return h->ue2.reserve(h, "ue2", 8ull * (W + 1) * entries); };
	auto group_launch = [&](const uint64_t *entries, const uint64_t *gs, const uint32_t *gc) -> int {
		int rc2 = wm.keys.reserve(h, "weak map keys", std::max<uint64_t>(8ull * W * wn, 8)); if (rc2) return rc2;
		rc2 = wm.vals.reserve(h, "weak map vals", std::max<uint64_t>(12ull * wn, 8)); if (rc2) return rc2;
		auto gk = bb_group_kernel<W>;
		HIPCHK(h, hipFuncSetAttribute((const void *)gk, hipFuncAttributeMaxDynamicSharedMemorySize, (int)bb_group_smem_bytes<W>()));
		int per_cu = 0;
		if (hipOccupancyMaxActiveBlocksPerMultiprocessor(&per_cu, (const void *)gk, BB_GROUP_THREADS, bb_group_smem_bytes<W>()) != hipSuccess || per_cu < 1) per_cu = 4;
		if (dbg()) fprintf(stderr, "bb_group<W=%d>: %d blocks per CU, %llu groups\n", W, per_cu, (unsigned long long)groups);
		hipLaunchKernelGGL(gk, dim3((unsigned)std::min<uint64_t>(groups, (uint64_t)num_cus(h) * per_cu)), dim3(BB_GROUP_THREADS), bb_group_smem_bytes<W>(), h->stream, entries, wm.keys.get<uint64_t>(), wm.vals.get<uint32_t>(), gs, gc, groups, g, h->hkb, nb, wm.start.get<uint64_t>(), wn, h->derr.get<uint32_t>());
		HIPCHK(h, hipGetLastError());
		return 0;
	};
	const uint32_t shift1 = B - bits1;
	uint32_t tpb = 1; unsigned grid = hist_grid(wslots, tpb);
	hipLaunchKernelGGL(bb_hist_kernel<W>, dim3(grid), dim3(BB_THREADS), 0, h->stream, in1, shift1, bits1, h->hkb, nb, tpb, hist1);
	unsigned int mx = 0;
	if (!bits2) {
		hipLaunchKernelGGL(bb_pad_kernel, dim3(grid_for(bins1)), dim3(256), 0, h->stream, (const uint32_t *)hist1, bins1, (uint32_t *)nullptr, dmax);
		HIPCHK(h, hipMemcpyAsync(&mx, dmax, 4, hipMemcpyDeviceToHost, h->stream));
		rc = exclusive_scan(h, hist1, bins1, start1); if (rc) return rc;
		if (mx > bb_group_cap<W>()) return 0;
		rc = scratch(wn); if (rc) return rc;
		hipLaunchKernelGGL(bb_cursor_init_kernel, dim3(grid_for(bins1)), dim3(256), 0, h->stream, (const uint64_t *)start1, bins1, cursor);
		hipLaunchKernelGGL(bb_scatter_kernel<W>, dim3(scatter_grid(wslots)), dim3(BB_THREADS), 0, h->stream, in1, shift1, bits1, h->hkb, nb, cursor, h->ue2.get<uint64_t>());
		rc = group_launch(h->ue2.get<uint64_t>(), start1, hist1); if (rc) return rc;
		done = true;
		return 0;
	}
	hipLaunchKernelGGL(bb_pad_kernel, dim3(grid_for(bins1)), dim3(256), 0, h->stream, (const uint32_t *)hist1, bins1, pad1, dmax);
	rc = exclusive_scan(h, pad1, bins1, start1); if (rc) return rc;
	uint64_t padded_total = 0;
	HIPCHK(h, hipMemcpy(&padded_total, start1 + bins1, 8, hipMemcpyDeviceToHost));
	rc = scratch(std::max(padded_total, wn)); if (rc) return rc;
	hipLaunchKernelGGL(bb_cursor_init_kernel, dim3(grid_for(bins1)), dim3(256), 0, h->stream, (const uint64_t *)start1, bins1, cursor);
	hipLaunchKernelGGL(bb_scatter_kernel<W>, dim3(scatter_grid(wslots)), dim3(BB_THREADS), 0, h->stream, in1, shift1, bits1, h->hkb, nb, cursor, h->ue2.get<uint64_t>());
	BbInput in2; in2.entries = h->ue2.get<uint64_t>(); in2.seg_start = start1; in2.seg_count = hist1; in2.n_seg = (uint32_t)bins1; in2.n_slots = padded_total; in2.holes = 0;
	const uint32_t shift2 = g;
	HIPCHK(h, hipMemsetAsync(hist2, 0, 4 * groups, h->stream)); HIPCHK(h, hipMemsetAsync(dmax, 0, 4, h->stream));
	grid = hist_grid(padded_total, tpb);
	hipLaunchKernelGGL(bb_hist_kernel<W>, dim3(grid), dim3(BB_THREADS), 0, h->stream, in2, shift2, bits2, h->hkb, nb, tpb, hist2);
	hipLaunchKernelGGL(bb_pad_kernel, dim3(grid_for(groups)), dim3(256), 0, h->stream, (const uint32_t *)hist2, groups, (uint32_t *)nullptr, dmax);
	HIPCHK(h, hipMemcpyAsync(&mx, dmax, 4, hipMemcpyDeviceToHost, h->stream));
	rc = exclusive_scan(h, hist2, groups, gstart); if (rc) return rc;
	if (mx > bb_group_cap<W>() || packed_entries(h, h->ue) < wn) return 0;
	hipLaunchKernelGGL(bb_cursor_init_kernel, dim3(grid_for(groups)), dim3(256), 0, h->stream, (const uint64_t *)gstart, groups, cursor);
	hipLaunchKernelGGL(bb_scatter_kernel<W>, dim3(scatter_grid(padded_total)), dim3(BB_THREADS), 0, h->stream, in2, shift2, bits2, h->hkb, nb, cursor, h->ue.get<uint64_t>());
	rc = group_launch(h->ue.get<uint64_t>(), gstart, hist2); if (rc) return rc;
	done = true;
	return 0;
}

template <int W> int finish_maps_t(kmr_handle *h, uint32_t *wc, uint32_t *sc, uint64_t wslots, uint64_t sslots, uint64_t wn, uint64_t sn, bool keepSing, bool weak_uncounted) {
	const uint32_t vw = h->ext ? 15 : 3;
	DevMap &wm = h->weak, &sm = h->sing;
	clear_map(wm); clear_map(sm);
	wm.nb = h->nb_weak; wm.n = wn; wm.present = true;
	sm.nb = h->nb_sing; sm.n = keepSing ? sn : 0; sm.present = keepSing;
	int rc = wm.start.reserve(h, "weak map start", 8 * (wm.nb + 1)); if (rc) return rc;
	rc = sm.start.reserve(h, "singleton map start", 8 * (sm.nb + 1)); if (rc) return rc;
	bool weakDone = false;
	if (weak_uncounted) {
		rc = binned_buckets_t<W>(h, wslots, wn, weakDone); if (rc) return rc;
		if (!weakDone) {
			if (key_entries(h, h->uw_keys) < wslots || !h->uw_vals) {
				h->uw_keys.reset(); h->uw_vals.reset();
				const uint64_t cap = std::max<uint64_t>(wslots, 16);
				HIPCHK(h, h->uw_keys.alloc(8ull * W * cap)); HIPCHK(h, h->uw_vals.alloc(12ull * cap));
			}
			HIPCHK(h, hipMemsetAsync(wc, 0, 4 * wm.nb, h->stream));
			if (wslots) hipLaunchKernelGGL(bb_unpack_kernel<W>, dim3(grid_for(wslots)), dim3(256), 0, h->stream, (const uint64_t *)h->ue.get<uint64_t>(), wslots, h->hkb, wm.nb, (uint64_t *)h->uw_keys.get(), (uint32_t *)h->uw_vals.get(), wc);
			HIPCHK(h, hipGetLastError());
		}
	}
	if (!weakDone) { rc = exclusive_scan(h, wc, wm.nb, wm.start.get<uint64_t>()); if (rc) return rc; }
	if (keepSing) { rc = exclusive_scan(h, sc, sm.nb, sm.start.get<uint64_t>()); if (rc) return rc; }
	else HIPCHK(h, hipMemsetAsync(sm.start.get<uint64_t>(), 0, 8 * (sm.nb + 1), h->stream));
	if (!weakDone) {
		rc = wm.keys.reserve(h, "weak map keys", std::max<uint64_t>(8ull * W * wm.n, 8)); if (rc) return rc;
		rc = wm.vals.reserve(h, "weak map vals", std::max<uint64_t>(4ull * vw * wm.n, 8)); if (rc) return rc;
	}
	rc = sm.keys.reserve(h, "singleton map keys", std::max<uint64_t>(8ull * W * sm.n, 8)); if (rc) return rc;
	rc = sm.sweight.reserve(h, "singleton map sweight", std::max<uint64_t>(sm.n, 8)); if (rc) return rc;
	if (h->ext) { rc = sm.spkt.reserve(h, "singleton map spkt", std::max<uint64_t>(4 * sm.n, 8)); if (rc) return rc; }
	HIPCHK(h, hipMemsetAsync(wc, 0, 4 * wm.nb, h->stream)); HIPCHK(h, hipMemsetAsync(sc, 0, 4 * sm.nb, h->stream));
	if (weakDone) {  }
	else if (wm.n && vw > 4) hipLaunchKernelGGL((entry_scatter_kernel<W, true>), dim3(grid_for(wslots)), dim3(256), 0, h->stream, (const uint64_t *)h->uw_keys.get(), (const uint32_t *)h->uw_vals.get(),
	                            (const uint8_t *)nullptr, (const uint32_t *)nullptr, wslots, vw, h->hkb, wm.nb, wm.start.get<uint64_t>(), wc, wm.keys.get<uint64_t>(), wm.vals.get<uint32_t>(), (uint8_t *)nullptr, (uint32_t *)nullptr);
	else if (wm.n) {
		unsigned long long *cur64 = nullptr;
		if (h->superkmer_mode && arena_get(h, &cur64, wm.nb) == 0) HIPCHK(h, hipMemcpyAsync(cur64, wm.start.get<uint64_t>(), 8 * wm.nb, hipMemcpyDeviceToDevice, h->stream));
		else cur64 = nullptr;
		hipLaunchKernelGGL(entry_scatter_kernel<W>, dim3(grid_for(wslots)), dim3(256), 0, h->stream, (const uint64_t *)h->uw_keys.get(), (const uint32_t *)h->uw_vals.get(),
		                            (const uint8_t *)nullptr, (const uint32_t *)nullptr, wslots, vw, h->hkb, wm.nb, wm.start.get<uint64_t>(), wc, wm.keys.get<uint64_t>(), wm.vals.get<uint32_t>(), (uint8_t *)nullptr, (uint32_t *)nullptr, cur64, 6);
	}
	if (sm.n) hipLaunchKernelGGL(entry_scatter_kernel<W>, dim3(grid_for(sslots)), dim3(256), 0, h->stream, (const uint64_t *)h->us_keys.get(), (const uint32_t *)nullptr,
	                            (const uint8_t *)h->us_b8.get(), (const uint32_t *)h->us_pkt.get(), sslots, 0u, h->hkb, sm.nb, sm.start.get<uint64_t>(), sc, sm.keys.get<uint64_t>(), (uint32_t *)nullptr, sm.sweight.get<uint8_t>(), h->ext ? sm.spkt.get<uint32_t>() : (uint32_t *)nullptr);
	HIPCHK(h, hipGetLastError());
	SortView<W> sv; sv.keys = wm.keys.get<uint64_t>(); sv.vals = wm.vals.get<uint32_t>(); sv.b8 = nullptr; sv.pkt = nullptr; sv.vw = vw;
	if (weakDone) {  }
	else if (h->ext) hipLaunchKernelGGL((sort_buckets_kernel<W, 15>), dim3(grid_for(wm.nb, 4, 1 << 20)), dim3(256), 0, h->stream, sv, wm.start.get<uint64_t>(), wm.nb);
	else hipLaunchKernelGGL((sort_buckets_kernel<W, 3>), dim3(grid_for(wm.nb, 4, 1 << 20)), dim3(256), 0, h->stream, sv, wm.start.get<uint64_t>(), wm.nb);
	if (sm.n) {
		SortView<W> ss; ss.keys = sm.keys.get<uint64_t>(); ss.vals = nullptr; ss.b8 = sm.sweight.get<uint8_t>(); ss.pkt = h->ext ? sm.spkt.get<uint32_t>() : nullptr; ss.vw = 0;
		hipLaunchKernelGGL((sort_buckets_kernel<W, 0>), dim3(grid_for(sm.nb, 4, 1 << 20)), dim3(256), 0, h->stream, ss, sm.start.get<uint64_t>(), sm.nb);
	}
	HIPCHK(h, hipGetLastError());
	HIPCHK(h, hipStreamSynchronize(h->stream));
	return 0;
}
int finish_maps_from_entries(kmr_handle *h, uint32_t *wc, uint32_t *sc, uint64_t wslots, uint64_t sslots, uint64_t wn, uint64_t sn, bool keepSing, bool weak_uncounted) {
	return with_w(h, [&](auto W) { return finish_maps_t<W()>(h, wc, sc, wslots, sslots, wn, sn, keepSing, weak_uncounted); });
}
int finalize_partition(kmr_handle *h, uint32_t min_depth) { return with_w_ext(h, [&](auto W, auto EXT) { return finalize_partition_t<W(), EXT()>(h, min_depth); }); }
template <int W, bool EXT> int insert_records_partition_t(kmr_handle *h, const void *recs, uint64_t n) {
	if (!h->l1.head) choose_bits1(h, n);
	hipEvent_t a, b; time_begin(h, 0, &a, &b);
	int rc = partition_level1<W, EXT>(h, recs, nullptr, nullptr, (n + 8191) / 8192, 0, 8192, n, n, &h->dstats.get<DevStats>()->inserted,
	                             2 * W + (h->ext ? 2 : 1), h->stream_base);
	time_end(h, 0, a, b);
	return rc;
}
int insert_records_partition(kmr_handle *h, const void *recs, uint64_t n) { return with_w_ext(h, [&](auto W, auto EXT) { return insert_records_partition_t<W(), EXT()>(h, recs, n); }); }
bool sk_geometry(uint32_t k, uint32_t m_wish, uint32_t &win, uint32_t &m, uint32_t &off, uint32_t win_max = 16) {
	for (uint32_t w : {32u, 16u, 8u, 4u}) {
		if (w > win_max) continue;
		if (w == 32u && (k < 45u || (m_wish && m_wish < 14u))) continue;
		if (k < w + 9) continue;
		uint32_t mm = std::min<uint32_t>(m_wish ? m_wish : 16u, k - w + 1);
		if (mm > 16) mm = 16;
		if (((k - mm + 1 - w) & 1u) != 0) mm--;
		if (mm < 10 && !m_wish) continue;
		if (mm < 4) continue;
		win = w; m = mm; off = (k - mm + 1 - w) / 2;
		return true;
	}
	return false;
}
const uint64_t SK_EXTRACT_WAVES_PER_CU = std::max(2 * SK_WAVES, SKL_MIN_BLOCKS * SKL_WAVES);
template <int W, int WIN, bool FILT, bool EXT = false> int launch_sk_extract(kmr_handle *h, const ReadsView &rv, const SkParams &sp, const DevParams *override_params = nullptr) {
	auto kern = sk_extract_kernel<W, WIN, FILT, EXT>;
	HIPCHK(h, hipFuncSetAttribute((const void *)kern, hipFuncAttributeMaxDynamicSharedMemorySize, (int)SK_EXTRACT_SMEM));
	const uint64_t tiles = ((rv.u_start ? rv.n_units : rv.n_reads) + 63) / 64;
	uint64_t blocks = (tiles + SK_WAVES - 1) / SK_WAVES;
	if (blocks == 0) return 0;
	blocks = std::min<uint64_t>(blocks, (uint64_t)num_cus(h) * 2);
	if (dbg()) { int nb = 0; hipOccupancyMaxActiveBlocksPerMultiprocessor(&nb, (const void *)kern, SK_WAVES * 64, SK_EXTRACT_SMEM); fprintf(stderr, "sk_extract<W=%d,WIN=%d>: %d blocks of %d waves per CU (LDS %zu), grid %llu, m=%u off=%u bits=%u\n", W, WIN, nb, SK_WAVES, SK_EXTRACT_SMEM, (unsigned long long)blocks, sp.m, sp.off, sp.list_bits); }
	hipLaunchKernelGGL(kern, dim3((unsigned)blocks), dim3(SK_WAVES * 64), SK_EXTRACT_SMEM, h->stream, rv, override_params ? *override_params : dev_params(h), sp, pool_view(h, h->l1));
	HIPCHK(h, hipGetLastError());
	return 0;
}
uint32_t sk_dbg_flags(const char *name);
bool sp_debug_extract(kmr_handle *h) { (void)h; return sk_dbg_flags("KMR_SK_EXTRACT_DBG") != 0; }
template <int W, int WIN, bool PACKED = false> int launch_sk_extract_lean(kmr_handle *h, const ReadsView &rv, const SkParams &sp, float wK, const DevParams *override_params = nullptr, const SkPacked *packed = nullptr) {
	auto kern = sk_extract_lean_kernel<W, WIN, PACKED>;
	SkPacked pkd{};
	if (PACKED) pkd = *packed;
	HIPCHK(h, hipFuncSetAttribute((const void *)kern, hipFuncAttributeMaxDynamicSharedMemorySize, (int)SKL_EXTRACT_SMEM));
	const uint64_t tiles = ((rv.u_start ? rv.n_units : rv.n_reads) + 63) / 64;
	uint64_t blocks = (tiles + SKL_WAVES - 1) / SKL_WAVES;
	if (blocks == 0) return 0;
	blocks = std::min<uint64_t>(blocks, (uint64_t)num_cus(h) * SKL_MIN_BLOCKS);
	hipLaunchKernelGGL(kern, dim3((unsigned)blocks), dim3(SKL_WAVES * 64), SKL_EXTRACT_SMEM, h->stream, rv, override_params ? *override_params : dev_params(h), sp, pool_view(h, h->l1), wK, pkd);
	HIPCHK(h, hipGetLastError());
	return 0;
}
int sk_uniform_weight(kmr_handle *h, const ReadsView &rv, bool &lean, float &wK) {
	lean = false; wK = 1.0f;
	if (h->tune.no_lean_extract) return 0;
	if (!rv.quals && h->uniform_q_hint < 0) { lean = true; return 0; }
	if (h->qual_mixed || rv.n_reads == 0) return 0;
	if (h->uniform_q_hint >= 0) {
		const unsigned int q0 = (unsigned int)h->uniform_q_hint;
		if (q0 == 127) { lean = true; wK = 1.0f; return 0; }
		if (!(h->hP[q0] > 0.0)) return 0;
		lean = true; wK = (float)h->hPk[q0];
		return 0;
	}
	{ int rc = h->qrange.reserve(h, "qrange", 8); if (rc) return rc; }
	const unsigned int init[2] = {255u, 0u};
	HIPCHK(h, hipMemcpyAsync(h->qrange.get<unsigned int>(), init, 8, hipMemcpyHostToDevice, h->stream));
	hipLaunchKernelGGL(sk_qual_range_kernel, dim3(num_cus(h) * 8), dim3(256), 0, h->stream, rv.quals, rv.offsets, rv.n_reads, h->qrange.get<unsigned int>());
	HIPCHK(h, hipGetLastError());
	unsigned int got[2] = {0, 0};
	HIPCHK(h, hipMemcpyAsync(got, h->qrange.get<unsigned int>(), 8, hipMemcpyDeviceToHost, h->stream));
	HIPCHK(h, hipStreamSynchronize(h->stream));
	if (got[0] != got[1]) { h->qual_mixed = got[0] < got[1]; return 0; }
	const unsigned int q0 = got[0];
	if (q0 == 127) { lean = true; wK = 1.0f; return 0; }
	if (!(h->hP[q0] > 0.0)) return 0;
	lean = true; wK = (float)h->hPk[q0];
	return 0;
}
uint32_t sk_dbg_flags(const char *name) {
#ifdef KMR_DEBUG_HOOKS
	const char *e = getenv(name); return e ? (uint32_t)atoi(e) : 0u;
#else
	(void)name; return 0u;
#endif
}
SkParams sk_params(kmr_handle *h) { SkParams sp; sp.dbg = sk_dbg_flags("KMR_SK_EXTRACT_DBG"); sp.keep_all_owners = h->sk_exchange ? 1u : 0u; sp.track = nullptr; sp.m = h->sk_m; sp.off = h->sk_off; sp.list_bits = h->sk_bits; sp.state = h->sk_state.get<unsigned long long>(); sp.Pk = h->dPk.get<double>(); sp.Rp = h->dPk.get<double>() + 256; sp.fast_div = h->sk_fast_div ? 1u : 0u; return sp; }
template <int W> int add_reads_superkmer_t(kmr_handle *h, const ReadsView &rvAll, uint64_t total_bases) {
	const uint64_t n = rvAll.n_reads;
	const DevParams dp = dev_params(h);
	const bool filt = dp.subsample > 1 || dp.num_parts > 1 || (dp.sub_wnb | dp.sub_snb) != 0 || (dp.world > 1 && !h->sk_exchange);
	bool lean = false; float wK = 1.0f;
	if (!filt && !h->ext && !sp_debug_extract(h)) { int rcq = sk_uniform_weight(h, rvAll, lean, wK); if (rcq) return rcq; }
	if (h->packed_direct && (!lean || h->cfg.size_tracker)) return fail(h, KMR_ERR_STATE, "internal: a packed batch handed to an extraction that wants text");
	if (rvAll.n_reads) {
		uint32_t wb; memcpy(&wb, &wK, 4);
		if (!lean) h->sk_uni_mixed = true;
		else if (h->sk_uni_w == SK_UNI_NONE) h->sk_uni_w = wb;
		else if (h->sk_uni_w != wb) h->sk_uni_mixed = true;
	}
	if (!h->sk_state) {
		const uint64_t est = h->cfg.estimated_raw_kmers ? h->cfg.estimated_raw_kmers : std::max<uint64_t>(total_bases, h->call_bases_hint) * std::max<uint32_t>(1, h->cfg.world_size);
		const uint64_t per_list = h->ext ? (W > 1 ? 400 : 600) : ((h->tune.target_list == 2048 && W > 1) ? 700 : h->tune.target_list * 3 / 4);
		uint32_t bits = 6; while (bits < 24 && (est >> bits) > per_list) bits++;
		h->sk_fine_shift = 0;
		if (h->sk_exchange && h->cfg.world_size > 1 && !h->tune.no_coarse_lists) {
			uint32_t sh = 0; while ((1u << sh) < h->cfg.world_size) sh++;
			if (bits >= 6 + sh) { h->sk_fine_shift = sh; bits -= sh; }
		}
		h->sk_bits = bits;
		if (h->cfg.world_size <= 1 && !h->sk_exchange && h->tune.target_list == 2048 && !h->tune.pow2_lists) {
			const uint64_t aim = h->tune.list_aim ? h->tune.list_aim : (W == 1 ? (h->ext ? 800 : (lean ? 1450 : 1700)) : per_list * 19 / 20);
			const uint64_t nlists = (est / aim + 63) & ~63ull;
			if (nlists > 64 && (nlists < (1ull << bits) || h->tune.list_aim) && nlists < (1ull << 31)) h->sk_bits = (uint32_t)nlists;
		}
		const uint64_t nl0 = sk_list_count(h->sk_bits);
		HIPCHK(h, h->sk_state.alloc(8 * nl0));
		hipLaunchKernelGGL(sk_state_init_kernel, dim3(grid_for(nl0)), dim3(256), 0, h->stream, h->sk_state.get<unsigned long long>(), nl0);
		HIPCHK(h, hipGetLastError());
	}
	const uint64_t avg = n ? std::max<uint64_t>(1, total_bases / n) : 1;
	const uint64_t sub_bases = h->tune.sub_batch_bases ? h->tune.sub_batch_bases : (1ull << 31);
	const uint64_t chunk = std::max<uint64_t>(64, (sub_bases / avg) & ~63ull);
	if (h->cfg.size_tracker && n) {
		h->trk_n = 0;
		{ int rc = h->trk.reserve(h, "trk", n * sizeof(SkTrackRec)); if (rc) return rc; }
		HIPCHK(h, hipMemsetAsync(h->trk.get<SkTrackRec>(), 0, n * sizeof(SkTrackRec), h->stream));
	}
	for (uint64_t r = 0; r < n; r += chunk) {
		const uint64_t m = std::min(chunk, n - r);
		ReadsView rv = reads_slice(rvAll, r, m);
		int rc = prepare_units(h, rv, h->packed_direct ? SK_PACKED_SPAN : (uint32_t)TILE_SPAN); if (rc) return rc;
		const uint64_t bases = m * avg + avg;
		if (!h->l1.base && r == 0 && h->cfg.world_size <= 1 && !h->sk_exchange && (h->cfg.estimated_raw_kmers || h->call_bases_hint > total_bases)) {
			const double job_bases = h->cfg.estimated_raw_kmers ? (double)h->cfg.estimated_raw_kmers * (double)avg / (double)(avg > h->k ? avg - h->k + 1 : 1) : (double)h->call_bases_hint;
			const double rest = job_bases - (double)total_bases;
			size_t fr = 0, tot = 0;
			if (rest > 0 && hipMemGetInfo(&fr, &tot) == hipSuccess) {
				const uint64_t want = (uint64_t)(rest * (h->ext ? 2.0 : 1.0) * (lean ? 0.3 : 0.65) / SK_CHUNK_G);
				h->l1.presize = std::min<uint64_t>(want, (uint64_t)(fr / 4) / ((size_t)CH * rec_bytes(h)));
			}
		}
		rc = pool_reserve(h, h->l1, (h->ext ? 2 : 1) * bases / SK_CHUNK_G + ((h->l1.base && !h->sk_exchange) ? 0 : sk_list_count(h->sk_bits)) + (uint64_t)num_cus(h) * SK_EXTRACT_WAVES_PER_CU * 130 + 64, true); if (rc) return rc;
		hipEvent_t a, b, a2, b2; time_begin(h, KMR_TIME_BUILD, &a, &b); time_begin(h, KMR_TIME_EXTRACT, &a2, &b2);
		SkParams sp = sk_params(h);
		if (h->cfg.size_tracker) sp.track = h->trk.get<SkTrackRec>() + r;
// ... 540 lines not shown
	h->hkb = h->kb | (cfg->hash_kind << 16);
	memset(&h->stats, 0, sizeof(h->stats));
	int rc = 0;
	do {
		if (cfg->device >= 0) { if (hipSetDevice(cfg->device) != hipSuccess) { rc = fail(nullptr, KMR_ERR_NO_DEVICE, "hipSetDevice failed"); break; } }
		if (hipGetDevice(&h->device) != hipSuccess) { rc = fail(nullptr, KMR_ERR_NO_DEVICE, "hipGetDevice failed"); break; }
		if (hipStreamCreate(&h->stream) != hipSuccess) { rc = fail(nullptr, KMR_ERR_HIP, "hipStreamCreate failed"); break; }
		uint64_t w = cfg->num_buckets_weak, s = cfg->num_buckets_singleton;
		const double depth = cfg->estimated_depth > 0 ? cfg->estimated_depth : 20.0;
		const uint32_t kpb = cfg->kmers_per_bucket ? cfg->kmers_per_bucket : 32;
		const uint64_t raw = cfg->estimated_raw_kmers / (cfg->world_size > 1 ? cfg->world_size : 1);
		if (w == 0) { unsigned long est = (unsigned long)(int)(raw / depth); w = est / kpb + 1; }
		if (s == 0) { unsigned long est = cfg->separate_singletons ? (unsigned long)(raw * cfg->estimated_error_rate) : 1; s = est / kpb + 1; }
		h->nb_weak = resize_buckets(w); h->nb_sing = resize_buckets(s);
		h->has_singletons = cfg->separate_singletons != 0;
		uint64_t want = cfg->max_table_entries ? (uint64_t)(cfg->max_table_entries / 0.7) : (uint64_t)(cfg->estimated_raw_kmers * 0.45 / 0.6);
		if (cfg->world_size > 1 && !cfg->max_table_entries) want /= cfg->world_size;
		uint32_t lg = 16; while ((1ull << lg) < want && lg < 40) lg++;
		h->log2cap = lg;
		double P[256]; quality_table(P, cfg->min_quality_score, cfg->fastq_start_char);
		if (h->dP.alloc(sizeof(P)) != hipSuccess || h->dstats.alloc(sizeof(DevStats)) != hipSuccess || h->derr.alloc(4) != hipSuccess) { rc = fail(nullptr, KMR_ERR_OOM, "hipMalloc failed"); break; }
		hipMemcpy(h->dP.get<double>(), P, sizeof(P), hipMemcpyHostToDevice); hipMemset(h->dstats.get<DevStats>(), 0, sizeof(DevStats)); hipMemset(h->derr.get<uint32_t>(), 0, 4);
		if (cfg->build_mode > 3) { rc = fail(nullptr, KMR_ERR_INVALID_ARG, "bad build_mode"); break; }
		h->partition_mode = cfg->build_mode != 1;
		uint32_t wish_w = 0, wish_m = 0, wish_o = 0;
		const bool sk_auto = cfg->build_mode == 0 && cfg->world_size <= 1 && sk_geometry(h->k, 0, wish_w, wish_m, wish_o);
		h->auto_mode = cfg->build_mode == 0;
		const bool sk_ready = sk_geometry(h->k, 0, wish_w, wish_m, wish_o);
		if (cfg->build_mode == 3 || sk_auto || sk_ready) {
			if (!sk_geometry(h->k, 0, h->sk_win, h->sk_m, h->sk_off)) { rc = fail(nullptr, KMR_ERR_UNSUPPORTED, "build_mode 3 (super-k-mer lists) needs k >= 13"); break; }
			h->superkmer_mode = cfg->build_mode == 3 || sk_auto;
			double Pk[256];
			for (int cidx = 0; cidx < 256; cidx++) { double wv = 1.0; for (uint32_t jj = 0; jj < h->k; jj++) wv *= P[cidx]; Pk[cidx] = wv; }
			memcpy(h->hPk, Pk, sizeof(Pk)); memcpy(h->hP, P, sizeof(h->hP));
			if (h->dPk.alloc(2 * sizeof(Pk)) != hipSuccess) { rc = fail(nullptr, KMR_ERR_OOM, "hipMalloc failed"); break; }
			hipMemcpy(h->dPk.get<double>(), Pk, sizeof(Pk), hipMemcpyHostToDevice);
			double Rp[256]; bool fast = true;
			for (int cidx = 0; cidx < 256; cidx++) Rp[cidx] = P[cidx] != 0.0 ? 1.0 / P[cidx] : 0.0;
			for (int a = 0; a < 256 && fast; a++) for (int b = 0; b < 256; b++) {
				if (P[a] == 0.0 || P[b] == 0.0) continue;
				const double q0 = P[a] * Rp[b];
				if (std::fma(std::fma(-q0, P[b], P[a]), Rp[b], q0) != P[a] / P[b]) { fast = false; break; }
			}
			h->sk_fast_div = fast;
			hipMemcpy(h->dPk.get<double>() + 256, Rp, sizeof(Rp), hipMemcpyHostToDevice);
		}
		if (cfg->size_tracker && (!h->superkmer_mode || h->ext || cfg->world_size > 1)) { rc = fail(nullptr, KMR_ERR_UNSUPPORTED, "size_tracker: kept by the super-k-mer build (build_mode 0 / 3, direction-counting values, k >= 13) of a single partition"); break; }
		if (!h->partition_mode) {
			rc = alloc_table(h, h->log2cap, h->slots, h->extslots);
			if (rc) { g_create_error = h->err; break; }
		}
		if (hipStreamSynchronize(h->stream) != hipSuccess) { rc = fail(nullptr, KMR_ERR_HIP, std::string("table clear failed: ") + hipGetErrorString(hipGetLastError())); break; }
	} while (0);
	if (rc) { kmr_destroy(h); return rc; }
	*out = h;
	return KMR_OK;
}

static void exchange_destroy_comm(kmr_handle *h);
void kmr_destroy(kmr_handle *h) {
	if (!h) return;
	if (h->stream) hipStreamSynchronize(h->stream);
	for (int which = 0; which < KMR_TIME_GROUPS; which++) for (auto &pr : h->pending_events[which]) { hipEventDestroy(pr.first); hipEventDestroy(pr.second); }
	release<HandleMem>(h);
	free_partition_state(h);
	exchange_destroy_comm(h);
	release<ExchangeMem>(h);
	if (h->stream) hipStreamDestroy(h->stream);
	delete h;
}

int kmr_num_buckets(const kmr_handle *h, int which, uint64_t *out) {
	if (!h || !out) return KMR_ERR_INVALID_ARG;
	if (which == KMR_MAP_WEAK) *out = h->finalized && h->weak.present ? h->weak.nb : h->nb_weak;
	else if (which == KMR_MAP_SINGLETON) *out = h->finalized && h->sing.present ? h->sing.nb : h->nb_sing;
	else return KMR_ERR_UNSUPPORTED;
	return KMR_OK;
}

int kmr_reset(kmr_handle *h) {
	if (!h) return KMR_ERR_INVALID_ARG;
	hipSetDevice(h->device);
	HIPCHK(h, hipStreamSynchronize(h->stream));
	clear_map(h->weak); clear_map(h->sing);
	int rc = 0;
	if (h->partition_mode) {
		if (h->l1.head) HIPCHK(h, hipMemsetAsync(h->l1.head.get<unsigned int>(), 0, 4, h->stream));
		h->l1.used_ub = 0;
		h->inserted_records = 0;
		h->qual_mixed = false;
		h->sk_uni_w = SK_UNI_NONE; h->sk_uni_mixed = false; h->peer_uni_w = SK_UNI_NONE; h->peer_uni_mixed = false; h->peers_declare = false;
		h->xr_lo = 0; h->xr_hi = ~0ull; h->early.active = false;
		if (h->d_uni) { const uint32_t init[2] = {SK_UNI_NONE, 0u}; HIPCHK(h, hipMemcpyAsync(h->d_uni.get<uint32_t>(), init, 8, hipMemcpyHostToDevice, h->stream)); HIPCHK(h, hipStreamSynchronize(h->stream)); }
		if (h->sk_state) hipLaunchKernelGGL(sk_state_init_kernel, dim3(grid_for(sk_list_count(h->sk_bits))), dim3(256), 0, h->stream, h->sk_state.get<unsigned long long>(), sk_list_count(h->sk_bits));
		if (h->l1_state) {
			hipLaunchKernelGGL(partition_state_init_kernel, dim3(partition_blocks(h)), dim3(256), 0, h->stream, h->l1_state.get<uint8_t>(),
			                   h->l1_state.cap() / (size_t)partition_blocks(h), h->bits1, (uint32_t)partition_blocks(h));
			h->l1_state_dirty = false;
		}
	} else {
		if (!h->slots) rc = alloc_table(h, h->log2cap, h->slots, h->extslots);
		else rc = clear_table_any(h, h->slots.get(), h->extslots.get<ExtSlot>(), h->log2cap);
		if (rc) return rc;
	}
	HIPCHK(h, hipMemsetAsync(h->dstats.get<DevStats>(), 0, sizeof(DevStats), h->stream));
	HIPCHK(h, hipMemsetAsync(h->derr.get<uint32_t>(), 0, 4, h->stream));
	memset(&h->stats, 0, sizeof(h->stats));
	h->occupied = h->pending_kmers = 0; h->stream_base = 0; h->reads = 0; h->subtracted = 0; h->xc_job_bases = 0; h->xc_bytes_to_peers = 0;
	h->trk_n = 0; h->trk_elems.clear();
	h->trk_next = 128; h->trk_raw = h->trk_good = 0; h->trk_bounds.clear(); h->trk_snap_raw.clear(); h->trk_snap_good.clear();
	h->finalized = false; h->map_gen++; h->has_singletons = h->cfg.separate_singletons != 0;
	return KMR_OK;
}
int kmr_release_table(kmr_handle *h) {
	if (!h) return KMR_ERR_INVALID_ARG;
	if (!h->finalized) return fail(h, KMR_ERR_STATE, "kmr_release_table before kmr_finalize");
	hipSetDevice(h->device);
	h->slots.reset(); h->extslots.reset();
	if (h->partition_mode) free_partition_state(h);
	return KMR_OK;
}

void *kmr_stream(kmr_handle *h) { return h ? (void *)h->stream : nullptr; }

int kmr_set_stream_origin(kmr_handle *h, uint64_t ordinal) {
	if (!h) return KMR_ERR_INVALID_ARG;
	if (h->finalized) return fail(h, KMR_ERR_STATE, "kmr_set_stream_origin after kmr_finalize");
	if (ordinal > MAX_STREAM_ORDINAL) return fail(h, KMR_ERR_CAPACITY, "stream ordinals have 40 bits");
	h->stream_base = ordinal;
	return KMR_OK;
}

int kmr_tune(kmr_handle *h, const char *knob, double value) {
	if (!h || !knob) return KMR_ERR_INVALID_ARG;
	const std::string k(knob);
	if (k == "target_list_records") h->tune.target_list = value >= 1 ? (uint64_t)value : 2048;
	else if (k == "sub_batch_bases") h->tune.sub_batch_bases = value >= 1 ? (uint64_t)value : 0;
	else if (k == "recycle_chunks") h->tune.recycle = value < 0 ? -1 : (value != 0 ? 1 : 0);
	else if (k == "partition_blocks") h->tune.part_blocks = value >= 1 ? (int)value : 0;
	else if (k == "entry_share") h->tune.entry_share = value;
	else if (k == "early_entry_share") h->tune.early_entry_share = value;
	else if (k == "saturated_batch_bytes") h->tune.saturated_batch_bytes = value >= 1 ? (uint64_t)value : 0;
	else if (k == "lookup_table") h->tune.no_lut = value == 0;
	else if (k == "stream_lookups") h->tune.no_stream_lookups = value == 0;
	else if (k == "long_list_chunks") h->tune.long_list_chunks = value < 2 ? 2 : (uint64_t)value;
	else if (k == "lean_extract") h->tune.no_lean_extract = value == 0;
	else if (k == "uniform_count") h->tune.no_uniform_count = value == 0;
	else if (k == "packed_direct") h->tune.no_packed_direct = value == 0;
	else if (k == "pow2_lists") h->tune.pow2_lists = value != 0;
	else if (k == "list_aim") h->tune.list_aim = value >= 1 ? (uint64_t)value : 0;
	else if (k == "twobit_piece_bases") h->tune.twobit_piece_bases = (uint64_t)value;
	else if (k == "exchange_fail_once") h->tune.exchange_fail_once = value != 0;
	else if (k == "binned_buckets_min") h->tune.binned_min = value >= 0 ? (uint64_t)value : ~0ull;
	else if (k == "coarse_lists") h->tune.no_coarse_lists = value == 0;
	else if (k == "select_timing") h->tune.select_timing = value != 0;
	else if (k == "dump_timing") h->tune.dump_timing = value != 0;
	else if (k == "pairs_timing") h->tune.pairs_timing = value != 0;
	else if (k == "dedup_timing") h->tune.dedup_timing = value != 0;
	else if (k == "pair_hash_bits") h->tune.pair_hash_bits = value >= 1 && value < 64 ? (uint32_t)value : 64;
	else if (k == "dump_piece_bytes") h->tune.dump_piece_bytes = value >= 1 ? (uint64_t)value : 0;
	else if (k == "narrow_tallies") h->tune.no_narrow = value == 0;
	else if (k == "keep_level1_state") h->tune.no_l1_state = value == 0;
	else if (k == "superkmer_window") {
		if (h->superkmer_mode && !h->sk_state) { uint32_t w, m, o; if (!sk_geometry(h->k, 0, w, m, o, (uint32_t)value)) return fail(h, KMR_ERR_INVALID_ARG, "no minimizer geometry under that window"); h->sk_win = w; h->sk_m = m; h->sk_off = o; }
	}
	else if (k == "superkmer_minimizer") {
		if (h->superkmer_mode && !h->sk_state) { uint32_t w, m, o; if (!sk_geometry(h->k, (uint32_t)value, w, m, o)) return fail(h, KMR_ERR_INVALID_ARG, "no minimizer geometry for that length"); h->sk_win = w; h->sk_m = m; h->sk_off = o; }
	}
	else return fail(h, KMR_ERR_INVALID_ARG, "unknown tuning knob '" + k + "'");
	return KMR_OK;
}

int kmr_build_info(kmr_handle *h, const char *what, double *value) {
	if (!h || !what || !value) return KMR_ERR_INVALID_ARG;
	const std::string k(what);
	if (k == "lists") *value = h->sk_state ? (double)sk_list_count(h->sk_bits) : 0.0;
	else if (k == "uniform_count") *value = h->last_count_uniform ? 1.0 : 0.0;
	else if (k == "chunk_pool_chunks") *value = (double)h->l1.cap;
	else if (k == "superkmer_window") *value = (double)h->sk_win;
	else if (k == "early_lists") *value = (double)h->last_early_hi;
	else if (k == "early_entries") *value = (double)h->last_early_entries;
	else if (k == "early_overflowed") *value = h->last_early_overflowed ? 1.0 : 0.0;
	else if (k == "saturated_keys") *value = (double)h->last_saturated_keys;
	else if (k == "saturated_batches") *value = (double)h->last_saturated_batches;
	else if (k == "device_blocks_live") *value = (double)g_blocks_live.load();
	else if (k == "filter_score_ms") *value = h->last_score_ms;
	else if (k == "select_ms") *value = h->last_select_ms;
	else if (k == "select_write_ms") *value = h->last_write_ms;
	else if (k == "pairs_ms") *value = h->last_pairs_ms;
	else if (k == "pairs_parse_ms") *value = h->last_pairs_parse_ms;
	else if (k == "pairs_sort_ms") *value = h->last_pairs_sort_ms;
	else if (k == "pair_hash_collisions") *value = (double)h->last_pair_hash_collisions;
	else if (k == "dedup_ms") *value = h->last_dedup_ms;
	else if (k == "dedup_key_ms") *value = h->last_dedup_key_ms;
	else if (k == "dedup_sort_ms") *value = h->last_dedup_sort_ms;
	else if (k == "dedup_consensus_ms") *value = h->last_dedup_consensus_ms;
	else if (k == "dump_size_ms") *value = h->last_dump_size_ms;
	else if (k == "dump_write_ms") *value = h->last_dump_write_ms;
	else return fail(h, KMR_ERR_INVALID_ARG, "unknown build figure '" + k + "'");
	return KMR_OK;
}

int kmr_sync(kmr_handle *h) { if (!h) return KMR_ERR_INVALID_ARG; hipSetDevice(h->device); return sync_state(h); }

int kmr_add_reads_dev(kmr_handle *h, const void *dev_bases, const void *dev_quals, const void *dev_offsets, uint64_t n_reads,
                      uint64_t total_bases, uint64_t first_global_read_idx, const void *dev_discarded) {
	if (!h) return KMR_ERR_INVALID_ARG;
	if (h->finalized) return fail(h, KMR_ERR_STATE, "kmr_add_reads after kmr_finalize");
	if (n_reads == 0) return KMR_OK;
	if (!dev_bases || !dev_offsets) return fail(h, KMR_ERR_INVALID_ARG, "null device buffer");
	hipSetDevice(h->device);
	const ReadsView rv = reads_view(dev_bases, dev_quals, dev_offsets, n_reads, dev_discarded, h->stream_base, first_global_read_idx);
	if (h->stream_base + total_bases > MAX_STREAM_ORDINAL) return fail(h, KMR_ERR_CAPACITY, "more than 2^40 input bases on one handle");
	if (h->partition_mode && !h->superkmer_mode && !h->ext && h->stream_base + total_bases > (1ull << 32))
		return fail(h, KMR_ERR_CAPACITY, "build_mode 2 orders occurrences by a 32-bit stream ordinal: at most 2^32 input bases per handle without extension values (use build_mode 0 / 3 or 1)");
	int rc = h->superkmer_mode ? add_reads_superkmer(h, rv, total_bases) : (h->partition_mode ? add_reads_partition(h, rv, total_bases) : add_reads_dev_any(h, rv, total_bases));
	h->stream_base += total_bases; h->reads += n_reads; h->stats.reads = h->reads;
	return rc;
}

static hipError_t tb_stage_copy(kmr_handle *h, int set, int which, const void *src, size_t bytes, void **dst) {
	DevBuf &buf = h->tb_stage[set][which];
	if (buf.cap() < bytes + 128) {
		if (buf) { hipError_t e0 = hipStreamSynchronize(h->stream); if (e0 != hipSuccess) return e0; }
		hipError_t e = buf.alloc(bytes + bytes / 8 + 4096); if (e != hipSuccess) return e;
	}
	*dst = buf.get();
	return bytes ? hipMemcpyAsync(buf.get(), src, bytes, hipMemcpyHostToDevice, h->tb_copy_stream) : hipSuccess;
}
static int tb_pipeline_ready(kmr_handle *h) {
	if (h->tb_copy_stream) return 0;
	HIPCHK(h, hipStreamCreateWithFlags(&h->tb_copy_stream, hipStreamNonBlocking));
	for (int i = 0; i < 2; i++) { HIPCHK(h, hipEventCreateWithFlags(&h->tb_ready[i], hipEventDisableTiming)); HIPCHK(h, hipEventCreateWithFlags(&h->tb_consumed[i], hipEventDisableTiming)); }
	return 0;
}

#define TBCHK(call) do { hipError_t e_ = (call); if (e_ != hipSuccess) { hipStreamSynchronize(h->tb_copy_stream); hipStreamSynchronize(h->stream); h->err = std::string(#call) + ": " + hip_err_text(e_); return e_ == hipErrorOutOfMemory ? KMR_ERR_OOM : KMR_ERR_HIP; } } while (0)
}
template <class Stage, class Feed> static int tb_feed_pieces(kmr_handle *h, const uint64_t *offsets, uint64_t n_reads, Stage &&stage, Feed &&feed) {
	{ int rcp = tb_pipeline_ready(h); if (rcp) return rcp; }
	const uint64_t piece_bases = h->tune.twobit_piece_bases ? h->tune.twobit_piece_bases : (1ull << 28);
	int rc = KMR_OK; int set = 0;
	h->call_bases_hint = n_reads ? offsets[n_reads] - offsets[0] : 0;
	struct HintReset { kmr_handle *h; ~HintReset() { h->call_bases_hint = 0; } } hint_reset{h};
	for (uint64_t r0 = 0; r0 < n_reads && rc == KMR_OK; set ^= 1) {
		uint64_t r1 = r0 + 1;
		while (r1 < n_reads && offsets[r1 + 1] - offsets[r0] <= piece_bases) r1++;
		if (h->tb_set_used[set]) TBCHK(hipStreamWaitEvent(h->tb_copy_stream, h->tb_consumed[set], 0));
		{ int rcs = stage(set, r0, r1); if (rcs) return rcs; }
		TBCHK(hipEventRecord(h->tb_ready[set], h->tb_copy_stream));
		TBCHK(hipStreamWaitEvent(h->stream, h->tb_ready[set], 0));
		rc = feed(r0, r1);
		TBCHK(hipEventRecord(h->tb_consumed[set], h->stream)); h->tb_set_used[set] = true;
		r0 = r1;
	}
	hipStreamSynchronize(h->tb_copy_stream);
	if (!rc) rc = sync_state(h);
	else hipStreamSynchronize(h->stream);
	return rc;
}
extern "C" {

int kmr_add_reads(kmr_handle *h, const char *bases, const char *quals, const uint64_t *offsets, uint64_t n_reads,
                  uint64_t first_global_read_idx, const uint8_t *discarded) {
	if (!h) return KMR_ERR_INVALID_ARG;
	if (h->finalized) return fail(h, KMR_ERR_STATE, "kmr_add_reads after kmr_finalize");
	if (n_reads == 0) return KMR_OK;
	if (!bases || !offsets) return fail(h, KMR_ERR_INVALID_ARG, "null buffer");
	hipSetDevice(h->device);
	void *db = nullptr, *dq = nullptr, *doff = nullptr, *dd = nullptr;
	auto stage = [&](int set, uint64_t r0, uint64_t r1) -> int {
		const uint64_t m = r1 - r0, total = offsets[r1] - offsets[r0];
		dq = nullptr; dd = nullptr;
		TBCHK(tb_stage_copy(h, set, 0, bases + offsets[r0], total, &db)); TBCHK(tb_stage_copy(h, set, 2, offsets + r0, 8 * (m + 1), &doff));
		if (quals) TBCHK(tb_stage_copy(h, set, 6, quals + offsets[r0], total, &dq));
		if (discarded) TBCHK(tb_stage_copy(h, set, 7, discarded + r0, m, &dd));
		TBCHK(hipMemsetAsync((uint8_t *)db + total, 0, 64, h->tb_copy_stream)); if (dq) TBCHK(hipMemsetAsync((uint8_t *)dq + total, 0, 64, h->tb_copy_stream));
		return KMR_OK;
	};
	auto feed = [&](uint64_t r0, uint64_t r1) {
		return kmr_add_reads_dev(h, (uint8_t *)db - offsets[r0], dq ? (uint8_t *)dq - offsets[r0] : nullptr, doff, r1 - r0, offsets[r1] - offsets[r0], first_global_read_idx + r0, dd);
	};
	return tb_feed_pieces(h, offsets, n_reads, stage, feed);
}

static bool sk_packed_direct_ok(kmr_handle *h, bool has_quals, int uniform_quality) {
	if (!h->superkmer_mode || h->ext || h->cfg.size_tracker || h->tune.no_lean_extract || h->tune.no_packed_direct || sp_debug_extract(h) || has_quals || h->qual_mixed) return false;
	const DevParams dp = dev_params(h);
	if (dp.subsample > 1 || dp.num_parts > 1 || (dp.sub_wnb | dp.sub_snb) != 0 || (dp.world > 1 && !h->sk_exchange)) return false;
	return uniform_quality == 0 || uniform_quality == 127 || h->hP[uniform_quality] > 0.0;
}
int kmr_add_reads_twobit_dev(kmr_handle *h, const void *dev_twobit, const void *dev_twobit_offsets, const void *dev_offsets,
                             const void *dev_markup_offsets, const void *dev_markup_pos, const void *dev_markup_char,
                             const void *dev_quals, int uniform_quality, uint64_t n_reads, uint64_t total_bases,
                             uint64_t first_global_read_idx, const void *dev_discarded) {
	if (!h) return KMR_ERR_INVALID_ARG;
	if (h->finalized) return fail(h, KMR_ERR_STATE, "kmr_add_reads after kmr_finalize");
	if (n_reads == 0) return KMR_OK;
	if (!dev_twobit || !dev_offsets) return fail(h, KMR_ERR_INVALID_ARG, "null device buffer");
	if (dev_markup_offsets && (!dev_markup_pos || !dev_markup_char)) return fail(h, KMR_ERR_INVALID_ARG, "markup offsets without markups");
	if (uniform_quality < 0 || uniform_quality > 255 || (dev_quals && uniform_quality)) return fail(h, KMR_ERR_INVALID_ARG, "uniform_quality: 0, or the one quality character of a batch without a quality array");
	hipSetDevice(h->device);
	const bool direct = sk_packed_direct_ok(h, dev_quals != nullptr, uniform_quality);
	if (!direct && h->tb_bases.cap() < total_bases + 64) {
		if (h->tb_bases) HIPCHK(h, hipStreamSynchronize(h->stream));
		HIPCHK(h, h->tb_bases.alloc(total_bases + 64));
		HIPCHK(h, hipMemsetAsync(h->tb_bases.get<uint8_t>(), 0, total_bases + 64, h->stream));
	}
	if (h->tb_len.cap() < 4 * (n_reads + 1)) {
		if (h->tb_len) HIPCHK(h, hipStreamSynchronize(h->stream));
		h->tb_rel.reset(); h->tb_off.reset(); h->tb_len.reset();
		HIPCHK(h, h->tb_rel.alloc(8 * (n_reads + 1))); HIPCHK(h, h->tb_off.alloc(8 * (n_reads + 1))); HIPCHK(h, h->tb_len.alloc(4 * (n_reads + 1)));
	}
	const uint64_t *tboff = (const uint64_t *)dev_twobit_offsets;
	if (!tboff) {
		hipLaunchKernelGGL(twobit_bytes_kernel, dim3(grid_for(n_reads)), dim3(256), 0, h->stream, (const uint64_t *)dev_offsets, n_reads, h->tb_len.get<uint32_t>());
		HIPCHK(h, hipGetLastError());
		int rc = exclusive_scan(h, h->tb_len.get<uint32_t>(), n_reads, h->tb_off.get<uint64_t>()); if (rc) return rc;
		tboff = h->tb_off.get<uint64_t>();
	}
	if (direct) {
		hipLaunchKernelGGL(offsets_rel_kernel, dim3(grid_for(n_reads + 1)), dim3(256), 0, h->stream, (const uint64_t *)dev_offsets, n_reads, h->tb_rel.get<uint64_t>());
		HIPCHK(h, hipGetLastError());
		if (h->stream_base + total_bases > MAX_STREAM_ORDINAL) return fail(h, KMR_ERR_CAPACITY, "more than 2^40 input bases on one handle");
		const ReadsView rv = reads_view(nullptr, nullptr, h->tb_rel.get<uint64_t>(), n_reads, dev_discarded, h->stream_base, first_global_read_idx);
		SkPacked pkd; pkd.bytes = (const uint8_t *)dev_twobit; pkd.off = tboff; pkd.mk_off = (const uint64_t *)dev_markup_offsets; pkd.mk_pos = (const uint32_t *)dev_markup_pos; pkd.mk_char = (const uint8_t *)dev_markup_char;
		h->packed_direct = &pkd; h->uniform_q_hint = uniform_quality ? uniform_quality : -1;
		const int rc = add_reads_superkmer(h, rv, total_bases);
		h->packed_direct = nullptr; h->uniform_q_hint = -1;
		h->stream_base += total_bases; h->reads += n_reads; h->stats.reads = h->reads;
		return rc;
	}
	hipLaunchKernelGGL(twobit_unpack_kernel, dim3((unsigned)std::min<uint64_t>((n_reads + 255) / 256, (uint64_t)num_cus(h) * 32)), dim3(256), 0, h->stream,
	                   (const uint8_t *)dev_twobit, tboff, (const uint64_t *)dev_offsets, n_reads, h->tb_bases.get<uint8_t>(), h->tb_rel.get<uint64_t>());
	HIPCHK(h, hipGetLastError());
	if (dev_markup_offsets) {
		hipLaunchKernelGGL(twobit_markup_kernel, dim3(grid_for(n_reads)), dim3(256), 0, h->stream, (const uint64_t *)dev_markup_offsets, (const uint32_t *)dev_markup_pos,
		                   (const uint8_t *)dev_markup_char, (const uint64_t *)h->tb_rel.get<uint64_t>(), n_reads, h->tb_bases.get<uint8_t>());
		HIPCHK(h, hipGetLastError());
	}
	const void *q = dev_quals;
	if (!dev_quals && uniform_quality) {
		if (h->tb_quals.cap() < total_bases + 64) {
			if (h->tb_quals) HIPCHK(h, hipStreamSynchronize(h->stream));
			HIPCHK(h, h->tb_quals.alloc(total_bases + 64)); h->tb_quals_filled = 0; h->tb_quals_char = -1;
		}
		if (h->tb_quals_char != uniform_quality || h->tb_quals_filled < total_bases) {
			HIPCHK(h, hipMemsetAsync(h->tb_quals.get(), uniform_quality, h->tb_quals.cap(), h->stream));
			h->tb_quals_char = uniform_quality; h->tb_quals_filled = h->tb_quals.cap();
		}
		q = h->tb_quals.get<uint8_t>();
	}
	h->uniform_q_hint = (!dev_quals && uniform_quality) ? uniform_quality : -1;
	const int rc = kmr_add_reads_dev(h, h->tb_bases.get<uint8_t>(), q, h->tb_rel.get<uint64_t>(), n_reads, total_bases, first_global_read_idx, dev_discarded);
	h->uniform_q_hint = -1;
	return rc;
}

int kmr_add_reads_twobit(kmr_handle *h, const uint8_t *twobit, const uint64_t *twobit_offsets, const uint64_t *offsets,
                         const uint64_t *markup_offsets, const uint32_t *markup_pos, const char *markup_char,
                         const char *quals, int uniform_quality, uint64_t n_reads, uint64_t first_global_read_idx, const uint8_t *discarded) {
	if (!h) return KMR_ERR_INVALID_ARG;
	if (h->finalized) return fail(h, KMR_ERR_STATE, "kmr_add_reads after kmr_finalize");
	if (n_reads == 0) return KMR_OK;
	if (!twobit || !twobit_offsets || !offsets) return fail(h, KMR_ERR_INVALID_ARG, "null buffer");
	hipSetDevice(h->device);
	void *dtb = nullptr, *dto = nullptr, *doff = nullptr, *dmo = nullptr, *dmp = nullptr, *dmc = nullptr, *dq = nullptr, *dd = nullptr;
	auto stage = [&](int set, uint64_t r0, uint64_t r1) -> int {
		const uint64_t m = r1 - r0, total = offsets[r1] - offsets[r0], tbytes = twobit_offsets[r1] - twobit_offsets[r0];
		const uint64_t nm = markup_offsets ? markup_offsets[r1] - markup_offsets[r0] : 0;
		dmo = dmp = dmc = dq = dd = nullptr;
		TBCHK(tb_stage_copy(h, set, 0, twobit + twobit_offsets[r0], tbytes, &dtb)); TBCHK(tb_stage_copy(h, set, 1, twobit_offsets + r0, 8 * (m + 1), &dto)); TBCHK(tb_stage_copy(h, set, 2, offsets + r0, 8 * (m + 1), &doff));
		dtb = (uint8_t *)dtb - twobit_offsets[r0];
		if (nm) {
			TBCHK(tb_stage_copy(h, set, 3, markup_offsets + r0, 8 * (m + 1), &dmo)); TBCHK(tb_stage_copy(h, set, 4, markup_pos + markup_offsets[r0], 4 * nm, &dmp)); TBCHK(tb_stage_copy(h, set, 5, markup_char + markup_offsets[r0], nm, &dmc));
			dmp = (uint32_t *)dmp - markup_offsets[r0]; dmc = (uint8_t *)dmc - markup_offsets[r0];
		}
		if (quals) TBCHK(tb_stage_copy(h, set, 6, quals + offsets[r0], total, &dq));
		if (discarded) TBCHK(tb_stage_copy(h, set, 7, discarded + r0, m, &dd));
		return KMR_OK;
	};
	auto feed = [&](uint64_t r0, uint64_t r1) {
		return kmr_add_reads_twobit_dev(h, dtb, dto, doff, dmo, dmp, dmc, dq, quals ? 0 : uniform_quality, r1 - r0, offsets[r1] - offsets[r0], first_global_read_idx + r0, dd);
	};
	return tb_feed_pieces(h, offsets, n_reads, stage, feed);
}

int kmr_finalize(kmr_handle *h, uint32_t min_depth) {
	if (!h) return KMR_ERR_INVALID_ARG;
	if (h->finalized) return fail(h, KMR_ERR_STATE, "already finalized");
	hipSetDevice(h->device);
	{ int src_ = sync_state(h); if (src_) return src_; }
	h->subtract = nullptr;
	if (h->superkmer_mode) return finalize_superkmer(h, min_depth);
	if (h->partition_mode) return finalize_partition(h, min_depth);
	return with_w_ext(h, [&](auto W, auto EXT) { return finalize_t<W(), EXT()>(h, min_depth); });
}

int kmr_get_stats(kmr_handle *h, kmr_stats *out) {
	if (!h || !out) return KMR_ERR_INVALID_ARG;
	hipSetDevice(h->device);
	if (!h->finalized) { int rc = sync_state(h); if (rc) return rc; h->stats.unique_kmers = h->partition_mode ? 0 : h->occupied; }
	h->stats.reads = h->reads;
	*out = h->stats;
	return KMR_OK;
}

int kmr_lookup(kmr_handle *h, const uint8_t *packed, uint64_t n, uint32_t *counts) {
	if (!h || (n && (!packed || !counts))) return KMR_ERR_INVALID_ARG;
	if (!h->finalized) return fail(h, KMR_ERR_STATE, "kmr_lookup before kmr_finalize");
	if (n == 0) return KMR_OK;
	hipSetDevice(h->device);
	return with_w(h, [&](auto W) { return lookup_t<W()>(h, packed, n, counts); });
}

static int lookup_reads_host(kmr_handle *h, const char *bases, const uint64_t *offsets, uint64_t n_reads, void *out, const uint64_t *out_offsets, bool weighted) {
	hipSetDevice(h->device);
	DevBuf sb, so;
	int rc = stage_reads(h, bases, offsets, n_reads, sb, so); if (rc) return rc;
	uint64_t outN = 0;
	for (uint64_t r = 0; r < n_reads; r++) { uint64_t L = offsets[r + 1] - offsets[r]; uint64_t nk = L >= h->k ? L - h->k + 1 : 0; outN = std::max(outN, out_offsets[r] + nk); }
	const uint64_t eb = weighted ? 8 : 4;
	DevBuf doutb, doffb;
	HIPCHK(h, doutb.alloc(std::max<uint64_t>(8, eb * outN))); HIPCHK(h, doffb.alloc(8 * n_reads));
	void *dout = doutb.get(); uint64_t *doff = doffb.get<uint64_t>();
	HIPCHK(h, hipMemsetAsync(dout, 0, eb * outN, h->stream));
	HIPCHK(h, hipMemcpyAsync(doff, out_offsets, 8 * n_reads, hipMemcpyHostToDevice, h->stream));
	ReadsView rv = reads_view(sb.get(), nullptr, so.get(), n_reads);
	rc = prepare_units(h, rv); if (rc) return rc;
	rc = with_w(h, [&](auto W) { return weighted ? lookup_reads_weighted_t<W()>(h, rv, (double *)dout, doff) : lookup_reads_t<W()>(h, rv, (uint32_t *)dout, doff); });
	if (!rc) { HIPCHK(h, hipMemcpyAsync(out, dout, eb * outN, hipMemcpyDeviceToHost, h->stream)); rc = sync_state(h); }
	else hipStreamSynchronize(h->stream);
	return rc;
}
int kmr_lookup_reads(kmr_handle *h, const char *bases, const uint64_t *offsets, uint64_t n_reads, uint32_t *counts_out, const uint64_t *out_offsets) {
	if (!h || !bases || !offsets || !counts_out || !out_offsets) return KMR_ERR_INVALID_ARG;
	if (!h->finalized) return fail(h, KMR_ERR_STATE, "kmr_lookup_reads before kmr_finalize");
	if (n_reads == 0) return KMR_OK;
	return lookup_reads_host(h, bases, offsets, n_reads, counts_out, out_offsets, false);
}

int kmr_lookup_weighted(kmr_handle *h, const uint8_t *packed, uint64_t n, double *weights) {
	if (!h || (n && (!packed || !weights))) return KMR_ERR_INVALID_ARG;
	if (!h->finalized) return fail(h, KMR_ERR_STATE, "kmr_lookup_weighted before kmr_finalize");
	if (n == 0) return KMR_OK;
	hipSetDevice(h->device);
	return with_w(h, [&](auto W) { return lookup_t<W()>(h, packed, n, nullptr, weights); });
}

int kmr_lookup_reads_weighted(kmr_handle *h, const char *bases, const uint64_t *offsets, uint64_t n_reads, double *weights_out, const uint64_t *out_offsets) {
	if (!h || !bases || !offsets || !weights_out || !out_offsets) return KMR_ERR_INVALID_ARG;
	if (!h->finalized) return fail(h, KMR_ERR_STATE, "kmr_lookup_reads_weighted before kmr_finalize");
	if (n_reads == 0) return KMR_OK;
	return lookup_reads_host(h, bases, offsets, n_reads, weights_out, out_offsets, true);
}

}
bool stream_lookups_possible(kmr_handle *h) {
	return h->dPk && !h->tune.no_stream_lookups && h->weak.present && h->weak.n > 0 && h->cfg.size_tracker == 0 && !h->sk_exchange;
}
template <int W> int sk_index_t(kmr_handle *h) {
	if (h->ix_gen == h->map_gen && h->ix_start) return 0;
	const uint64_t nl = sk_list_count(h->sk_bits), n = h->weak.n;
	const uint32_t vw = h->ext ? 15 : 3;
	if (h->ix_lists != nl) { h->ix_lists = 0; HIPCHK(h, h->ix_start.alloc(8 * (nl + 1))); h->ix_lists = nl; }
	if (h->ix_counts.cap() < 4 * n) {
		h->ix_keys.reset(); h->ix_counts.reset();
		HIPCHK(h, h->ix_keys.alloc(8ull * W * n)); HIPCHK(h, h->ix_counts.alloc(4 * n));
	}
	uint32_t *elist = nullptr, *hist = nullptr;
	int rc = arena_get(h, &elist, n); if (rc) return rc;
	rc = arena_get(h, &hist, nl); if (rc) return rc;
	HIPCHK(h, hipMemsetAsync(hist, 0, 4 * nl, h->stream));
	hipLaunchKernelGGL(sk_index_hist_kernel<W>, dim3(grid_for(n)), dim3(256), 0, h->stream, (const uint64_t *)h->weak.keys.get<uint64_t>(), n, h->sk_m, h->sk_off, h->sk_win, h->sk_bits, elist, hist);
	HIPCHK(h, hipGetLastError());
	rc = exclusive_scan(h, hist, nl, h->ix_start.get<uint64_t>()); if (rc) return rc;
	HIPCHK(h, hipMemsetAsync(hist, 0, 4 * nl, h->stream));
	hipLaunchKernelGGL(sk_index_scatter_kernel<W>, dim3(grid_for(n)), dim3(256), 0, h->stream, (const uint64_t *)h->weak.keys.get<uint64_t>(), (const uint32_t *)h->weak.vals.get<uint32_t>(), vw, n, elist, h->ix_start.get<uint64_t>(), hist, h->ix_keys.get<uint64_t>(), h->ix_counts.get<uint32_t>());
	HIPCHK(h, hipGetLastError());
	h->ix_gen = h->map_gen;
	return 0;
}
template <int W> int lookup_stream_t(kmr_handle *h, const ReadsView &rvAll, uint64_t total_bases, uint32_t *position_counts, uint64_t out_n) {
	int rc = arena_reset(h); if (rc) return rc;
	if (!h->sk_state) {
		uint32_t bits = 6; while (bits < 24 && (total_bases >> bits) > h->tune.target_list / 2 + 200) bits++;
		h->sk_bits = bits;
		HIPCHK(h, h->sk_state.alloc(8ull << bits));
	}
	rc = h->scratch_stats.reserve(h, "scratch_stats", sizeof(DevStats)); if (rc) return rc;
	rc = sk_index_t<W>(h); if (rc) return rc;
	const uint64_t nl = sk_list_count(h->sk_bits);
	hipLaunchKernelGGL(sk_state_init_kernel, dim3(grid_for(nl)), dim3(256), 0, h->stream, h->sk_state.get<unsigned long long>(), nl);
	if (h->l1.head) HIPCHK(h, hipMemsetAsync(h->l1.head.get<unsigned int>(), 0, 4, h->stream));
	h->l1.used_ub = 0;
	ReadsView rv = rvAll;
	rc = prepare_units(h, rv); if (rc) return rc;
	rc = pool_reserve(h, h->l1, total_bases / SK_CHUNK_G + nl + (uint64_t)num_cus(h) * SK_EXTRACT_WAVES_PER_CU * 130 + 64, true); if (rc) return rc;
	DevParams dp = dev_params(h);
	dp.min_weight = 0.5f; dp.subsample = 1; dp.world = 1; dp.num_parts = 1; dp.sub_wnb = 0; dp.sub_snb = 0; dp.stats = h->scratch_stats.get<DevStats>();
	SkParams sp = sk_params(h); sp.keep_all_owners = 1; sp.track = nullptr;
	rc = with_win<W>(h->sk_win, [&](auto WIN) { return (!rv.quals && !h->tune.no_lean_extract) ? launch_sk_extract_lean<W, WIN()>(h, rv, sp, 1.0f, &dp) : launch_sk_extract<W, WIN(), false>(h, rv, sp, &dp); });
	if (rc) return rc;
	hipLaunchKernelGGL(sk_close_kernel, dim3(grid_for(nl)), dim3(256), 0, h->stream, h->sk_state.get<unsigned long long>(), nl, h->l1.chunk_count.get<uint32_t>(), h->l1.cap);
	HIPCHK(h, hipGetLastError());
	uint64_t *ls = nullptr, *lc = nullptr; uint32_t nch = 0;
	rc = build_csr(h, h->l1, nl, 0, &ls, &lc, &nch); if (rc) return rc;
	rc = zero_work_counter(h); if (rc) return rc;
	const int grid = (int)std::min<uint64_t>((uint64_t)num_cus(h) * 4, (nl + SK_LBATCH - 1) / SK_LBATCH);
	auto kern = sk_lookup_kernel<W>;
	const size_t smem = sk_lookup_smem_bytes<W>();
	HIPCHK(h, hipFuncSetAttribute((const void *)kern, hipFuncAttributeMaxDynamicSharedMemorySize, (int)smem));
	const uint64_t LONG_CHUNKS = h->tune.long_list_chunks ? h->tune.long_list_chunks : 1024, PIECE = std::max<uint64_t>(1, LONG_CHUNKS / 2);
	uint64_t n_items = 0; uint64_t *ic0 = nullptr, *ic1 = nullptr; uint32_t *il = nullptr;
	if (nch > LONG_CHUNKS) {
		const uint64_t cap = (uint64_t)nch / PIECE + 2 * 1024 + 16;
		unsigned long long *dn = nullptr;
		rc = arena_get(h, &ic0, cap); if (rc) return rc; rc = arena_get(h, &ic1, cap); if (rc) return rc; rc = arena_get(h, &il, cap); if (rc) return rc; rc = arena_get(h, &dn, 1); if (rc) return rc;
		HIPCHK(h, hipMemsetAsync(dn, 0, 8, h->stream));
		hipLaunchKernelGGL(sk_long_items_kernel, dim3(grid_for(nl)), dim3(256), 0, h->stream, ls, nl, LONG_CHUNKS, PIECE, ic0, ic1, cap, dn, il);
		HIPCHK(h, hipGetLastError());
		unsigned long long hn = 0;
		HIPCHK(h, hipMemcpyAsync(&hn, dn, 8, hipMemcpyDeviceToHost, h->stream)); HIPCHK(h, hipStreamSynchronize(h->stream));
		if (hn > cap) return fail(h, KMR_ERR_CAPACITY, "long-list work items (internal sizing error)");
		n_items = hn;
	}
	hipLaunchKernelGGL(kern, dim3(grid), dim3(COUNT_THREADS), smem, h->stream, pool_view(h, h->l1), ls, lc, nl, h->k, h->ix_start.get<uint64_t>(), h->ix_keys.get<uint64_t>(), h->ix_counts.get<uint32_t>(), position_counts, out_n, h->work_counter.get<unsigned int>(),
	                   (const uint64_t *)nullptr, (const uint64_t *)nullptr, (const uint32_t *)nullptr, (uint64_t)0, n_items ? LONG_CHUNKS : (uint64_t)0);
	HIPCHK(h, hipGetLastError());
	if (n_items) {
		rc = zero_work_counter(h); if (rc) return rc;
		hipLaunchKernelGGL(kern, dim3((unsigned)std::min<uint64_t>((uint64_t)num_cus(h) * 4, n_items)), dim3(COUNT_THREADS), smem, h->stream, pool_view(h, h->l1), ls, lc, nl, h->k, h->ix_start.get<uint64_t>(), h->ix_keys.get<uint64_t>(), h->ix_counts.get<uint32_t>(),
		                   position_counts, out_n, h->work_counter.get<unsigned int>(), (const uint64_t *)ic0, (const uint64_t *)ic1, (const uint32_t *)il, n_items, (uint64_t)0);
		HIPCHK(h, hipGetLastError());
	}
	return 0;
}
int lookup_stream(kmr_handle *h, const ReadsView &rv, uint64_t total_bases, uint32_t *position_counts, uint64_t out_n) {
	return with_w(h, [&](auto W) { return lookup_stream_t<W()>(h, rv, total_bases, position_counts, out_n); });
}

extern "C" {
struct ScoreDev { uint32_t *trim_offset, *trim_length; float *score; uint8_t *was_trimmed; };
static int score_reads_core(kmr_handle *h, const uint8_t *s_b, const uint64_t *s_o, uint64_t n_reads, double minimum_kmer_score, int scoring_type,
                            uint32_t *trim_offset, uint32_t *trim_length, float *score, uint8_t *was_trimmed, ScoreDev *keep = nullptr) {
	int rc = 0;
// ... 1698 lines not shown
```

kmernator_amd/csrc/kmr_buckets.hpp:

```cpp
#ifndef KMR_BUCKETS_HPP_
#define KMR_BUCKETS_HPP_

#include "kmr_partition.hpp"

namespace kmr {

int sort_pairs_u64_u32(void *tmp, size_t *tmp_bytes, const unsigned long long *keys_in, unsigned long long *keys_out, const unsigned int *vals_in, unsigned int *vals_out, size_t n, hipStream_t stream);

static const int BB_TILE = 8192;
static const int BB_THREADS = 512;
static const int BB_GROUP_THREADS = 256;
static const int BB_PER_THREAD = BB_TILE / BB_THREADS;
static const int BB_MAX_BITS = 10;
static const int BB_MAX_GROUP_BITS = 8;
static const uint32_t BB_GROUP_CAP = 1536;
template <int W> __host__ __device__ constexpr uint32_t bb_group_cap() { return W == 1 ? BB_GROUP_CAP : 1344u; }

__host__ __device__ __forceinline__ uint64_t bb_pack_value(uint32_t count, uint32_t weighted_bits, uint32_t dir) { return (uint64_t)(count | (dir << 16)) | ((uint64_t)weighted_bits << 32); }

struct BbInput {
	const uint64_t *entries;
	const uint64_t *seg_start;
	const uint32_t *seg_count;
	uint32_t n_seg;
	uint64_t n_slots;
	uint32_t holes;
};

template <int W> __device__ __forceinline__ void bb_load_entry(const uint64_t *entries, uint64_t e, uint64_t (&w)[W + 1]) {
	if constexpr (W == 1) { const uint4 v = ((const uint4 *)entries)[e]; w[0] = (uint64_t)v.x | ((uint64_t)v.y << 32); w[1] = (uint64_t)v.z | ((uint64_t)v.w << 32); }
	else {
#pragma unroll
		for (int q = 0; q <= W; q++) w[q] = entries[e * (W + 1) + q];
	}
}
template <int W> __device__ __forceinline__ void bb_store_entry(uint64_t *entries, uint64_t e, const uint64_t (&w)[W + 1]) {
	if constexpr (W == 1) ((uint4 *)entries)[e] = make_uint4((uint32_t)w[0], (uint32_t)(w[0] >> 32), (uint32_t)w[1], (uint32_t)(w[1] >> 32));
	else {
#pragma unroll
		for (int q = 0; q <= W; q++) entries[e * (W + 1) + q] = w[q];
	}
}

__device__ __forceinline__ uint32_t bb_segment_of(const BbInput &in, uint64_t s0) {
	if (!in.seg_start) return 0;
	uint32_t lo = 0, hi = in.n_seg;
	while (hi - lo > 1) { const uint32_t mid = (lo + hi) >> 1; if (in.seg_start[mid] <= s0) lo = mid; else hi = mid; }
	return lo;
}

template <int W>
__global__ __launch_bounds__(BB_THREADS)
void bb_hist_kernel(BbInput in, uint32_t shift, uint32_t bits, uint32_t kb, uint64_t nb, uint32_t tiles_per_block, uint32_t *hist) {
	__shared__ uint32_t lh[1 << BB_MAX_BITS];
	__shared__ uint32_t s_seg;
	const int t = threadIdx.x;
	const uint32_t bins = 1u << bits, mask = bins - 1;
	const uint64_t n_tiles = (in.n_slots + BB_TILE - 1) / BB_TILE;
	const uint64_t tile0 = (uint64_t)blockIdx.x * tiles_per_block;
	uint32_t curSeg = 0xffffffffu;
	for (uint32_t i = t; i < bins; i += BB_THREADS) lh[i] = 0;
	__syncthreads();
	for (uint64_t tile = tile0; tile < tile0 + tiles_per_block && tile < n_tiles; tile++) {
		const uint64_t s0 = tile * BB_TILE;
		if (t == 0) s_seg = bb_segment_of(in, s0);
		__syncthreads();
		const uint32_t seg = s_seg;
		if (seg != curSeg) {
			if (curSeg != 0xffffffffu) {
				for (uint32_t i = t; i < bins; i += BB_THREADS) { const uint32_t c = lh[i]; if (c) { atomicAdd(&hist[((uint64_t)curSeg << bits) + i], c); lh[i] = 0; } }
				__syncthreads();
			}
			curSeg = seg;
		}
		const uint64_t segEnd = in.seg_start ? in.seg_start[seg] + in.seg_count[seg] : in.n_slots;
#pragma unroll 4
		for (int i = 0; i < BB_PER_THREAD; i++) {
			const uint64_t e = s0 + (uint64_t)i * BB_THREADS + t;
			if (e >= segEnd) continue;
			uint64_t ew[W + 1];
			bb_load_entry<W>(in.entries, e, ew);
			if (in.holes && ew[W] == 0) continue;
			Key<W> key;
#pragma unroll
			for (int q = 0; q < W; q++) key.w[q] = ew[q];
			const uint64_t b = key_hash<W>(key, kb) & (nb - 1);
			atomicAdd(&lh[(uint32_t)(b >> shift) & mask], 1u);
		}
		__syncthreads();
	}
	if (curSeg != 0xffffffffu) for (uint32_t i = t; i < bins; i += BB_THREADS) { const uint32_t c = lh[i]; if (c) atomicAdd(&hist[((uint64_t)curSeg << bits) + i], c); }
}

#ifndef KMR_INSTANCE_TU
__global__ void bb_pad_kernel(const uint32_t *hist, uint64_t n, uint32_t *padded, unsigned int *max_count) {
	unsigned int m = 0;
	for (uint64_t i = blockIdx.x * (uint64_t)blockDim.x + threadIdx.x; i < n; i += (uint64_t)gridDim.x * blockDim.x) {
		const uint32_t c = hist[i];
		if (padded) padded[i] = (c + BB_TILE - 1) / BB_TILE * BB_TILE;
		m = c > m ? c : m;
	}
	for (int o = 32; o > 0; o >>= 1) { const unsigned int x = (unsigned int)__shfl_xor((int)m, o, 64); m = x > m ? x : m; }
	if ((threadIdx.x & 63) == 0 && m) atomicMax(max_count, m);
}
__global__ void bb_cursor_init_kernel(const uint64_t *start, uint64_t n, unsigned long long *cursor) {
	for (uint64_t i = blockIdx.x * (uint64_t)blockDim.x + threadIdx.x; i < n; i += (uint64_t)gridDim.x * blockDim.x) cursor[i] = start[i];
}
#endif

template <int W>
__global__ __launch_bounds__(BB_THREADS)
void bb_scatter_kernel(BbInput in, uint32_t shift, uint32_t bits, uint32_t kb, uint64_t nb, unsigned long long *cursor, uint64_t *out_entries) {
	__shared__ uint32_t lh[1 << BB_MAX_BITS];
	__shared__ unsigned long long lbase[1 << BB_MAX_BITS];
	__shared__ uint32_t s_seg;
	const int t = threadIdx.x;
	const uint32_t bins = 1u << bits, mask = bins - 1;
	const uint64_t n_tiles = (in.n_slots + BB_TILE - 1) / BB_TILE;
	for (uint64_t tile = blockIdx.x; tile < n_tiles; tile += gridDim.x) {
		const uint64_t s0 = tile * BB_TILE;
		__syncthreads();
		if (t == 0) s_seg = bb_segment_of(in, s0);
		for (uint32_t i = t; i < bins; i += BB_THREADS) lh[i] = 0;
		__syncthreads();
		const uint32_t seg = s_seg;
		const uint64_t segEnd = in.seg_start ? in.seg_start[seg] + in.seg_count[seg] : in.n_slots;
		uint32_t where[BB_PER_THREAD];
#pragma unroll
		for (int i = 0; i < BB_PER_THREAD; i++) {
			const uint64_t e = s0 + (uint64_t)i * BB_THREADS + t;
			where[i] = 0xffffffffu;
			if (e >= segEnd) continue;
			uint64_t ew[W + 1];
			bb_load_entry<W>(in.entries, e, ew);
			if (in.holes && ew[W] == 0) continue;
			Key<W> key;
#pragma unroll
			for (int q = 0; q < W; q++) key.w[q] = ew[q];
			const uint32_t bin = (uint32_t)((key_hash<W>(key, kb) & (nb - 1)) >> shift) & mask;
			where[i] = (bin << 16) | atomicAdd(&lh[bin], 1u);
		}
		__syncthreads();
		for (uint32_t i = t; i < bins; i += BB_THREADS) { const uint32_t c = lh[i]; if (c) lbase[i] = atomicAdd(&cursor[((uint64_t)seg << bits) + i], (unsigned long long)c); }
		__syncthreads();
#pragma unroll
		for (int i = 0; i < BB_PER_THREAD; i++) {
			if (where[i] == 0xffffffffu) continue;
			const uint64_t e = s0 + (uint64_t)i * BB_THREADS + t;
			uint64_t ew[W + 1];
			bb_load_entry<W>(in.entries, e, ew);
			bb_store_entry<W>(out_entries, lbase[where[i] >> 16] + (where[i] & 0xffffu), ew);
		}
	}
}

static const int BB_GROUP_PER_THREAD = (BB_GROUP_CAP + BB_GROUP_THREADS - 1) / BB_GROUP_THREADS;
template <int W> __host__ __device__ constexpr size_t bb_group_smem_bytes() { return (size_t)bb_group_cap<W>() * (8 * W + 8 + 2 + 2); }

template <int W>
__global__ __launch_bounds__(BB_GROUP_THREADS, W <= 2 ? 4 : 1)
void bb_group_kernel(const uint64_t *entries, uint64_t *keys, uint32_t *vals, const uint64_t *gstart, const uint32_t *gcount, uint64_t n_groups, uint32_t gbits, uint32_t kb, uint64_t nb,
                     uint64_t *start, uint64_t n_total, uint32_t *err) {
	extern __shared__ __attribute__((aligned(16))) uint8_t gsm[];
	uint64_t *skeys = (uint64_t *)gsm;
	constexpr uint32_t CAP = bb_group_cap<W>();
	uint64_t *svalw = skeys + (size_t)CAP * W;
	uint16_t *sbucket = (uint16_t *)(svalw + CAP);
	uint16_t *final_ = sbucket + CAP;
	__shared__ uint32_t bcnt[1 << BB_MAX_GROUP_BITS], bstart[(1 << BB_MAX_GROUP_BITS) + 1], bscan[BB_GROUP_THREADS / 64];
	const int t = threadIdx.x;
	const uint32_t nbk = 1u << gbits;
	for (uint64_t G = blockIdx.x; G < n_groups; G += gridDim.x) {
		const uint64_t base = gstart[G];
		const uint32_t n = gcount[G];
		__syncthreads();
		if ((uint32_t)t < nbk) bcnt[t] = 0;
		if (n > CAP) { if (t == 0) atomicOr(err, (uint32_t)ERR_ENTRIES_FULL); continue; }
		__syncthreads();
		uint64_t ew[BB_GROUP_PER_THREAD][W + 1]; uint32_t lb[BB_GROUP_PER_THREAD];
#pragma unroll
		for (int u = 0; u < BB_GROUP_PER_THREAD; u++) {
			const uint32_t i = (uint32_t)u * BB_GROUP_THREADS + t;
			lb[u] = 0xffffffffu;
			if (i < n) bb_load_entry<W>(entries, base + i, ew[u]);
		}
#pragma unroll
		for (int u = 0; u < BB_GROUP_PER_THREAD; u++) {
			const uint32_t i = (uint32_t)u * BB_GROUP_THREADS + t;
			if (i >= n) continue;
			Key<W> key;
#pragma unroll
			for (int q = 0; q < W; q++) key.w[q] = ew[u][q];
			lb[u] = (uint32_t)(key_hash<W>(key, kb) & (nb - 1)) & (nbk - 1);
			atomicAdd(&bcnt[lb[u]], 1u);
		}
		__syncthreads();
		{
			const uint32_t c = (uint32_t)t < nbk ? bcnt[t] : 0u;
			uint32_t incl = c;
#pragma unroll
			for (int o = 1; o < 64; o <<= 1) { const uint32_t x = (uint32_t)__shfl_up((int)incl, o, 64); if ((t & 63) >= o) incl += x; }
			if ((t & 63) == 63) bscan[t >> 6] = incl;
			__syncthreads();
			uint32_t before = 0;
			for (int w = 0; w < (t >> 6); w++) before += bscan[w];
			if ((uint32_t)t < nbk) { bstart[t] = before + incl - c; start[G * nbk + t] = base + before + incl - c; bcnt[t] = 0; }
			if (t == 0) { bstart[nbk] = n; if (G == n_groups - 1) start[nb] = n_total; }
		}
		__syncthreads();
#pragma unroll
		for (int u = 0; u < BB_GROUP_PER_THREAD; u++) {
			if (lb[u] == 0xffffffffu) continue;
			const uint32_t pos = bstart[lb[u]] + atomicAdd(&bcnt[lb[u]], 1u);
#pragma unroll
			for (int q = 0; q < W; q++) skeys[(size_t)pos * W + q] = ew[u][q];
			svalw[pos] = ew[u][W];
			sbucket[pos] = (uint16_t)lb[u];
		}
		__syncthreads();
		for (uint32_t p = t; p < n; p += BB_GROUP_THREADS) {
			const uint32_t b = sbucket[p];
			const uint32_t s = bstart[b], e = bstart[b + 1];
			Key<W> mine;
#pragma unroll
			for (int q = 0; q < W; q++) mine.w[q] = skeys[(size_t)p * W + q];
			uint32_t rank = 0;
#pragma unroll 4
			for (uint32_t qx = s; qx < e; qx++) {
				Key<W> other;
#pragma unroll
				for (int q = 0; q < W; q++) other.w[q] = skeys[(size_t)qx * W + q];
				rank += (key_lt<W>(other, mine) || (key_eq<W>(other, mine) && qx < p)) ? 1u : 0u;
			}
			final_[s + rank] = (uint16_t)p;
		}
		__syncthreads();
		for (uint32_t p = t; p < n; p += BB_GROUP_THREADS) {
			const uint32_t i = final_[p];
#pragma unroll
			for (int q = 0; q < W; q++) keys[(base + p) * W + q] = skeys[(size_t)i * W + q];
			const uint64_t vw_ = svalw[i];
			vals[(base + p) * 3] = (uint32_t)vw_ & 0xffffu; vals[(base + p) * 3 + 1] = (uint32_t)(vw_ >> 32); vals[(base + p) * 3 + 2] = ((uint32_t)vw_ >> 16) & 0xffffu;
		}
	}
}

template <int W>
__global__ __launch_bounds__(256)
void bb_unpack_kernel(const uint64_t *entries, uint64_t n_slots, uint32_t kb, uint64_t nb, uint64_t *keys, uint32_t *vals, uint32_t *counts) {
	for (uint64_t e = blockIdx.x * (uint64_t)blockDim.x + threadIdx.x; e < n_slots; e += (uint64_t)gridDim.x * blockDim.x) {
		uint64_t ew[W + 1];
		bb_load_entry<W>(entries, e, ew);
		Key<W> key;
#pragma unroll
		for (int q = 0; q < W; q++) { key.w[q] = ew[q]; keys[e * W + q] = ew[q]; }
		vals[e * 3] = (uint32_t)ew[W] & 0xffffu; vals[e * 3 + 1] = (uint32_t)(ew[W] >> 32); vals[e * 3 + 2] = ((uint32_t)ew[W] >> 16) & 0xffffu;
		if (ew[W] != 0) atomicAdd(&counts[key_hash<W>(key, kb) & (nb - 1)], 1u);
	}
}

}
#endif
```

Before: 55.79 billion.

## Bucket weak map into fixed-capacity regions without histogram passes or host syncs

Adds a region-based bucketing path that scatters entries into fixed-capacity regions sized from a mean plus several sigmas. This drops the histogram, padding and host-synchronized scan passes, and count and scan work is queued asynchronously. Overflow is flagged on the device so later kernels exit early, with fallback to the histogram path when a region overflows. The scatter kernel now keeps loaded entries in registers for narrow keys instead of reloading them, uses a smaller per-thread tile for W=2, and gains an occupancy hint. The cost is extra scratch memory for the padded regions and a possible redo when a region overflows.

```diff
diff --git a/kmernator_amd/csrc/kmr_api.hip b/kmernator_amd/csrc/kmr_api.hip
--- a/kmernator_amd/csrc/kmr_api.hip
+++ b/kmernator_amd/csrc/kmr_api.hip
@@ -134,6 +134,7 @@
 	DevBuf tb_stage[2][8];
 	DevBuf uw_keys, uw_vals, us_keys, us_b8, us_pkt;
 	DevBuf ue, ue2;
+	DevBuf ue3;
 };
 struct ExchangeMem {
 	DevBuf xc_small, xc_dcounts;
@@ -152,6 +153,8 @@
 	uint64_t saturated_batch_bytes = 0;
 	bool no_lut = false, no_narrow = false, no_l1_state = false, no_stream_lookups = false;
 	uint64_t long_list_chunks = 0;
+	uint32_t bb_group_limit = 0;
+	double bb_margin_l1 = 8, bb_margin_l2 = 8;
 	uint64_t binned_min = 1ull << 18;
 	uint64_t twobit_piece_bases = 0;
 	uint64_t list_aim = 0;
@@ -209,6 +212,7 @@
 	uint32_t peer_uni_w = 0xffffffffu; bool peer_uni_mixed = false, peers_declare = false;
 	uint64_t xr_lo = 0, xr_hi = ~0ull;
 	uint64_t last_early_hi = 0, last_early_entries = 0;
+	int last_bucket_path = 0;
 	bool last_early_overflowed = false;
 	double last_score_ms = 0, last_select_ms = 0, last_write_ms = 0;
 	double last_dump_size_ms = 0, last_dump_write_ms = 0;
@@ -519,7 +523,7 @@
 
 int add_reads_dev_any(kmr_handle *h, const ReadsView &rv, uint64_t total_bases) { return with_w_ext(h, [&](auto W, auto EXT) { return add_reads_dev_t<W(), EXT()>(h, rv, total_bases); }); }
 
-int exclusive_scan(kmr_handle *h, const uint32_t *in, uint64_t n, uint64_t *out ) {
+int exclusive_scan_async(kmr_handle *h, const uint32_t *in, uint64_t n, uint64_t *out ) {
 	const uint64_t nblocks = (n + SCAN_ITEMS - 1) / SCAN_ITEMS;
 	const size_t eb = sizeof(unsigned long long);
 	int rc = h->scan_sums.reserve(h, "scan_sums", eb * (nblocks + 1), eb * std::max<uint64_t>(nblocks + 1, 4096)); if (rc) return rc;
@@ -528,6 +532,10 @@
 	hipLaunchKernelGGL(scan_sums_kernel, dim3(1), dim3(256), 0, h->stream, sums, nblocks, total);
 	hipLaunchKernelGGL(scan_apply_kernel, dim3((unsigned)nblocks), dim3(256), 0, h->stream, in, n, sums, out);
 	HIPCHK(h, hipGetLastError());
+	return 0;
+}
+int exclusive_scan(kmr_handle *h, const uint32_t *in, uint64_t n, uint64_t *out ) {
+	int rc = exclusive_scan_async(h, in, n, out); if (rc) return rc;
 	HIPCHK(h, hipStreamSynchronize(h->stream));
 	return 0;
 }
@@ -874,7 +882,7 @@
 			size_t mfree = 0, mtotal = 0;
 			if (hipMemGetInfo(&mfree, &mtotal) == hipSuccess && (double)mfree < (double)chunks * CH * rec_bytes(h) * 1.02 + (double)(2ull << 30)) {
 				HIPCHK(h, hipStreamSynchronize(h->stream));
-				h->uw_keys.reset(); h->uw_vals.reset(); h->us_keys.reset(); h->us_b8.reset(); h->us_pkt.reset(); h->ue.reset(); h->ue2.reset();
+				h->uw_keys.reset(); h->uw_vals.reset(); h->us_keys.reset(); h->us_b8.reset(); h->us_pkt.reset(); h->ue.reset(); h->ue2.reset(); h->ue3.reset();
 			}
 		}
 		uint64_t want = est / CH + launches * (uint64_t)grid * ((1ull << h->bits1) + 512) + 64 + l2_allowance;
@@ -1215,17 +1223,106 @@
 	return rc;
 }
 
-template <int W> int binned_buckets_t(kmr_handle *h, uint64_t wslots, uint64_t wn, bool &done) {
-	done = false;
-	DevMap &wm = h->weak;
-	const uint64_t nb = wm.nb;
-	uint32_t B = 0; while ((1ull << (B + 1)) <= nb) B++;
-	if (h->ext || wn < h->tune.binned_min || wn == 0 || (1ull << B) != nb || wslots >= (1ull << 40)) return 0;
+enum { BB_PATH_SORT = 0, BB_PATH_REGIONS = 1, BB_PATH_REDO_L1 = 2, BB_PATH_REDO_L2 = 3, BB_PATH_HISTOGRAMS = 4 };
+enum : uint32_t { BB_OVF_L1 = 1u, BB_OVF_LAST = 2u };
+static inline int bb_redo_path(bool two_levels, uint32_t ovf) { return two_levels && (ovf & BB_OVF_L1) ? BB_PATH_REDO_L1 : BB_PATH_REDO_L2; }
+struct BbPlan {
+	uint64_t wslots = 0, wn = 0, nb = 0;
+	uint32_t B = 0, g = 0, R = 0, bits1 = 0, bits2 = 0;
+	uint64_t bins1 = 0, groups = 0;
+	uint32_t *ovf = nullptr;
+	unsigned long long *cursor1 = nullptr;
+	uint64_t cap1 = 0, cap2 = 0;
+	uint64_t *out2 = nullptr;
+};
+bool bb_plan(kmr_handle *h, uint64_t wslots, uint64_t wn, BbPlan &p) {
+	p.wslots = wslots; p.wn = wn; p.nb = h->weak.nb;
+	uint32_t B = 0; while ((1ull << (B + 1)) <= p.nb) B++;
+	if (h->ext || wn < h->tune.binned_min || wn == 0 || (1ull << B) != p.nb || wslots >= (1ull << 40)) return false;
 	uint32_t g = 0; while (g < std::min<uint32_t>(B, BB_MAX_GROUP_BITS) && (wn >> (B - g)) < 512) g++;
 	const uint32_t R = B - g;
-	if (R < 1 || R > 2 * BB_MAX_BITS || (wn >> R) > 1024) return 0;
-	const uint32_t bits1 = R <= (uint32_t)BB_MAX_BITS ? R : (R + 1) / 2, bits2 = R - bits1;
-	const uint64_t bins1 = 1ull << bits1, groups = 1ull << R;
+	if (R < 1 || R > 2 * BB_MAX_BITS || (wn >> R) > 1024) return false;
+	p.B = B; p.g = g; p.R = R;
+	p.bits1 = R <= (uint32_t)BB_MAX_BITS ? R : (R + 1) / 2; p.bits2 = R - p.bits1;
+	p.bins1 = 1ull << p.bits1; p.groups = 1ull << R;
+	return true;
+}
+uint64_t bb_region_room(uint64_t mean, double sigmas) { return std::max<uint64_t>(1, mean + (uint64_t)std::ceil(sigmas * std::sqrt((double)mean))); }
+template <int W> unsigned bb_scatter_grid(kmr_handle *h, uint64_t n_slots) { const uint64_t tiles = (n_slots + bb_scatter_step<W>() - 1) / bb_scatter_step<W>(); return (unsigned)std::min<uint64_t>(std::max<uint64_t>(tiles, 1), (uint64_t)num_cus(h) * 8); }
+template <int W> int bb_group_launch(kmr_handle *h, const BbPlan &p, const uint64_t *entries, const uint64_t *gs, const uint32_t *gc, uint64_t in_stride, const uint32_t *ovf) {
+	DevMap &wm = h->weak;
+	int rc2 = wm.keys.reserve(h, "weak map keys", std::max<uint64_t>(8ull * W * p.wn, 8)); if (rc2) return rc2;
+	rc2 = wm.vals.reserve(h, "weak map vals", std::max<uint64_t>(12ull * p.wn, 8)); if (rc2) return rc2;
+	auto gk = bb_group_kernel<W>;
+	HIPCHK(h, hipFuncSetAttribute((const void *)gk, hipFuncAttributeMaxDynamicSharedMemorySize, (int)bb_group_smem_bytes<W>()));
+	int per_cu = 0;
+	if (hipOccupancyMaxActiveBlocksPerMultiprocessor(&per_cu, (const void *)gk, BB_GROUP_THREADS, bb_group_smem_bytes<W>()) != hipSuccess || per_cu < 1) per_cu = 4;
+	if (dbg()) fprintf(stderr, "bb_group<W=%d>: %d blocks per CU, %llu groups\n", W, per_cu, (unsigned long long)p.groups);
+	hipLaunchKernelGGL(gk, dim3((unsigned)std::min<uint64_t>(p.groups, (uint64_t)num_cus(h) * per_cu)), dim3(BB_GROUP_THREADS), bb_group_smem_bytes<W>(), h->stream, entries, wm.keys.get<uint64_t>(), wm.vals.get<uint32_t>(), gs, gc, p.groups, p.g, h->hkb, p.nb, wm.start.get<uint64_t>(), p.wn, h->derr.get<uint32_t>(), in_stride, ovf);
+	HIPCHK(h, hipGetLastError());
+	return 0;
+}
+
+template <int W> int bb_by_regions(kmr_handle *h, BbPlan &p, bool &queued) {
+	queued = false;
+	const bool two = p.bits2 != 0;
+	const uint64_t mean2 = (p.wn + p.groups - 1) >> p.R;
+	if (mean2 < 16) return 0;
+	p.cap2 = (bb_region_room(mean2, 8) + 7) / 8 * 8;
+	if (p.cap2 > bb_group_cap<W>()) return 0;
+	const uint64_t room2 = h->tune.bb_margin_l2 >= 8 ? p.cap2 : bb_region_room(mean2, h->tune.bb_margin_l2);
+	uint64_t room1 = 0;
+	if (two) {
+		const uint64_t mean1 = (p.wn + p.bins1 - 1) >> p.bits1;
+		p.cap1 = (bb_region_room(mean1, 8) + BB_TILE + BB_TILE - 1) / BB_TILE * BB_TILE;
+		room1 = h->tune.bb_margin_l1 >= 8 ? p.cap1 : bb_region_room(mean1, h->tune.bb_margin_l1);
+	}
+	const size_t eb = 8ull * (W + 1);
+	auto have = [&](DevBuf &b, size_t need) -> bool {
+		if (b.cap() >= need) return true;
+		size_t mfree = 0, mtotal = 0;
+		if (hipMemGetInfo(&mfree, &mtotal) != hipSuccess) { (void)hipGetLastError(); return false; }
+		if (mfree + b.cap() < need) return false;
+		if (hipStreamSynchronize(h->stream) != hipSuccess) return false;
+		if (b.alloc(need) == hipSuccess) return true;
+		(void)hipGetLastError();
+		return false;
+	};
+	const size_t need2 = eb * p.groups * p.cap2;
+	if (!two) { if (!have(h->ue2, need2)) return 0; p.out2 = h->ue2.get<uint64_t>(); }
+	else {
+		if (!have(h->ue2, eb * p.bins1 * p.cap1)) return 0;
+		if (h->ue.cap() >= need2) p.out2 = h->ue.get<uint64_t>();
+		else { if (!have(h->ue3, need2)) return 0; p.out2 = h->ue3.get<uint64_t>(); }
+	}
+	unsigned long long *cursor2 = nullptr; uint32_t *gcount = nullptr; uint64_t *gstart = nullptr;
+	int rc = arena_get(h, &p.ovf, 1); if (rc) return rc;
+	rc = arena_get(h, &cursor2, p.groups); if (rc) return rc;
+	rc = arena_get(h, &gcount, p.groups); if (rc) return rc;
+	rc = arena_get(h, &gstart, p.groups + 1); if (rc) return rc;
+	if (two) { rc = arena_get(h, &p.cursor1, p.bins1); if (rc) return rc; }
+	HIPCHK(h, hipMemsetAsync(p.ovf, 0, 4, h->stream));
+	BbInput in1; in1.entries = h->ue.get<uint64_t>(); in1.seg_start = nullptr; in1.seg_count = nullptr; in1.n_seg = 1; in1.n_slots = p.wslots; in1.holes = 1; in1.seg_cursor = nullptr; in1.seg_cap = 0;
+	BbInput last = in1;
+	if (two) {
+		hipLaunchKernelGGL(bb_region_init_kernel, dim3(grid_for(p.bins1)), dim3(256), 0, h->stream, p.bins1, p.cap1, p.cursor1);
+		hipLaunchKernelGGL(bb_scatter_kernel<W>, dim3(bb_scatter_grid<W>(h, p.wslots)), dim3(BB_THREADS), 0, h->stream, in1, p.B - p.bits1, p.bits1, h->hkb, p.nb, p.cursor1, h->ue2.get<uint64_t>(), p.cap1, room1, p.ovf, (uint32_t)BB_OVF_L1);
+		last.entries = h->ue2.get<uint64_t>(); last.n_seg = (uint32_t)p.bins1; last.n_slots = p.bins1 * p.cap1; last.holes = 0; last.seg_cursor = p.cursor1; last.seg_cap = p.cap1;
+	}
+	hipLaunchKernelGGL(bb_region_init_kernel, dim3(grid_for(p.groups)), dim3(256), 0, h->stream, p.groups, p.cap2, cursor2);
+	hipLaunchKernelGGL(bb_scatter_kernel<W>, dim3(bb_scatter_grid<W>(h, last.n_slots)), dim3(BB_THREADS), 0, h->stream, last, p.g, two ? p.bits2 : p.bits1, h->hkb, p.nb, cursor2, p.out2, p.cap2, room2, p.ovf, (uint32_t)BB_OVF_LAST);
+	hipLaunchKernelGGL(bb_region_count_kernel, dim3(grid_for(p.groups)), dim3(256), 0, h->stream, (const unsigned long long *)cursor2, p.groups, p.cap2, gcount, (const uint32_t *)p.ovf);
+	HIPCHK(h, hipGetLastError());
+	rc = exclusive_scan_async(h, gcount, p.groups, gstart); if (rc) return rc;
+	rc = bb_group_launch<W>(h, p, p.out2, gstart, gcount, p.cap2, p.ovf); if (rc) return rc;
+	queued = true;
+	return 0;
+}
+
+template <int W> int bb_by_histograms(kmr_handle *h, BbPlan &p, bool last_only, bool &done) {
+	done = false;
+	const uint64_t nb = p.nb, wn = p.wn, wslots = p.wslots, bins1 = p.bins1, groups = p.groups;
+	const uint32_t bits1 = p.bits1, bits2 = p.bits2, g = p.g;
 	uint32_t *hist1 = nullptr, *hist2 = nullptr, *pad1 = nullptr; uint64_t *start1 = nullptr, *gstart = nullptr; unsigned long long *cursor = nullptr; unsigned int *dmax = nullptr;
 	int rc = arena_get(h, &hist1, bins1); if (rc) return rc;
 	rc = arena_get(h, &start1, bins1 + 1); if (rc) return rc;
@@ -1233,57 +1330,53 @@
 	rc = arena_get(h, &dmax, 1); if (rc) return rc;
 	if (bits2) { rc = arena_get(h, &hist2, groups); if (rc) return rc; rc = arena_get(h, &pad1, bins1); if (rc) return rc; rc = arena_get(h, &gstart, groups + 1); if (rc) return rc; }
 	HIPCHK(h, hipMemsetAsync(hist1, 0, 4 * bins1, h->stream)); HIPCHK(h, hipMemsetAsync(dmax, 0, 4, h->stream));
-	BbInput in1; in1.entries = h->ue.get<uint64_t>(); in1.seg_start = nullptr; in1.seg_count = nullptr; in1.n_seg = 1; in1.n_slots = wslots; in1.holes = 1;
+	BbInput in1; in1.entries = h->ue.get<uint64_t>(); in1.seg_start = nullptr; in1.seg_count = nullptr; in1.n_seg = 1; in1.n_slots = wslots; in1.holes = 1; in1.seg_cursor = nullptr; in1.seg_cap = 0;
 	auto hist_grid = [&](uint64_t n_slots, uint32_t &tpb) { const uint64_t tiles = (n_slots + BB_TILE - 1) / BB_TILE; tpb = (uint32_t)std::max<uint64_t>(1, (tiles + 2047) / 2048); return (unsigned)((tiles + tpb - 1) / tpb); };
-	auto scatter_grid = [&](uint64_t n_slots) { const uint64_t tiles = (n_slots + BB_TILE - 1) / BB_TILE; return (unsigned)std::min<uint64_t>(tiles, (uint64_t)num_cus(h) * 8); };
 	auto scratch = [&](uint64_t entries) { return h->ue2.reserve(h, "ue2", 8ull * (W + 1) * entries); };
-	auto group_launch = [&](const uint64_t *entries, const uint64_t *gs, const uint32_t *gc) -> int {
-		int rc2 = wm.keys.reserve(h, "weak map keys", std::max<uint64_t>(8ull * W * wn, 8)); if (rc2) return rc2;
-		rc2 = wm.vals.reserve(h, "weak map vals", std::max<uint64_t>(12ull * wn, 8)); if (rc2) return rc2;
-		auto gk = bb_group_kernel<W>;
-		HIPCHK(h, hipFuncSetAttribute((const void *)gk, hipFuncAttributeMaxDynamicSharedMemorySize, (int)bb_group_smem_bytes<W>()));
-		int per_cu = 0;
-		if (hipOccupancyMaxActiveBlocksPerMultiprocessor(&per_cu, (const void *)gk, BB_GROUP_THREADS, bb_group_smem_bytes<W>()) != hipSuccess || per_cu < 1) per_cu = 4;
-		if (dbg()) fprintf(stderr, "bb_group<W=%d>: %d blocks per CU, %llu groups\n", W, per_cu, (unsigned long long)groups);
-		hipLaunchKernelGGL(gk, dim3((unsigned)std::min<uint64_t>(groups, (uint64_t)num_cus(h) * per_cu)), dim3(BB_GROUP_THREADS), bb_group_smem_bytes<W>(), h->stream, entries, wm.keys.get<uint64_t>(), wm.vals.get<uint32_t>(), gs, gc, groups, g, h->hkb, nb, wm.start.get<uint64_t>(), wn, h->derr.get<uint32_t>());
-		HIPCHK(h, hipGetLastError());
-		return 0;
-	};
-	const uint32_t shift1 = B - bits1;
-	uint32_t tpb = 1; unsigned grid = hist_grid(wslots, tpb);
-	hipLaunchKernelGGL(bb_hist_kernel<W>, dim3(grid), dim3(BB_THREADS), 0, h->stream, in1, shift1, bits1, h->hkb, nb, tpb, hist1);
+	const uint32_t shift1 = p.B - bits1;
+	const uint32_t group_limit = h->tune.bb_group_limit ? std::min<uint32_t>(h->tune.bb_group_limit, bb_group_cap<W>()) : bb_group_cap<W>();
+	uint32_t tpb = 1; unsigned grid = 0;
 	unsigned int mx = 0;
-	if (!bits2) {
-		hipLaunchKernelGGL(bb_pad_kernel, dim3(grid_for(bins1)), dim3(256), 0, h->stream, (const uint32_t *)hist1, bins1, (uint32_t *)nullptr, dmax);
-		HIPCHK(h, hipMemcpyAsync(&mx, dmax, 4, hipMemcpyDeviceToHost, h->stream));
-		rc = exclusive_scan(h, hist1, bins1, start1); if (rc) return rc;
-		if (mx > bb_group_cap<W>()) return 0;
-		rc = scratch(wn); if (rc) return rc;
+	BbInput in2;
+	uint64_t *out2 = h->ue.get<uint64_t>();
+	if (!last_only) {
+		grid = hist_grid(wslots, tpb);
+		hipLaunchKernelGGL(bb_hist_kernel<W>, dim3(grid), dim3(BB_THREADS), 0, h->stream, in1, shift1, bits1, h->hkb, nb, tpb, hist1);
+		if (!bits2) {
+			hipLaunchKernelGGL(bb_pad_kernel, dim3(grid_for(bins1)), dim3(256), 0, h->stream, (const uint32_t *)hist1, bins1, (uint32_t *)nullptr, dmax);
+			HIPCHK(h, hipMemcpyAsync(&mx, dmax, 4, hipMemcpyDeviceToHost, h->stream));
+			rc = exclusive_scan(h, hist1, bins1, start1); if (rc) return rc;
+			if (mx > group_limit) return 0;
+			rc = scratch(wn); if (rc) return rc;
+			hipLaunchKernelGGL(bb_cursor_init_kernel, dim3(grid_for(bins1)), dim3(256), 0, h->stream, (const uint64_t *)start1, bins1, cursor);
+			hipLaunchKernelGGL(bb_scatter_kernel<W>, dim3(bb_scatter_grid<W>(h, wslots)), dim3(BB_THREADS), 0, h->stream, in1, shift1, bits1, h->hkb, nb, cursor, h->ue2.get<uint64_t>(), (uint64_t)0, (uint64_t)0, (uint32_t *)nullptr, 0u);
+			rc = bb_group_launch<W>(h, p, h->ue2.get<uint64_t>(), start1, hist1, 0, nullptr); if (rc) return rc;
+			done = true;
+			return 0;
+		}
+		hipLaunchKernelGGL(bb_pad_kernel, dim3(grid_for(bins1)), dim3(256), 0, h->stream, (const uint32_t *)hist1, bins1, pad1, dmax);
+		rc = exclusive_scan(h, pad1, bins1, start1); if (rc) return rc;
+		uint64_t padded_total = 0;
+		HIPCHK(h, hipMemcpy(&padded_total, start1 + bins1, 8, hipMemcpyDeviceToHost));
+		rc = scratch(std::max(padded_total, wn)); if (rc) return rc;
 		hipLaunchKernelGGL(bb_cursor_init_kernel, dim3(grid_for(bins1)), dim3(256), 0, h->stream, (const uint64_t *)start1, bins1, cursor);
-		hipLaunchKernelGGL(bb_scatter_kernel<W>, dim3(scatter_grid(wslots)), dim3(BB_THREADS), 0, h->stream, in1, shift1, bits1, h->hkb, nb, cursor, h->ue2.get<uint64_t>());
-		rc = group_launch(h->ue2.get<uint64_t>(), start1, hist1); if (rc) return rc;
-		done = true;
-		return 0;
-	}
-	hipLaunchKernelGGL(bb_pad_kernel, dim3(grid_for(bins1)), dim3(256), 0, h->stream, (const uint32_t *)hist1, bins1, pad1, dmax);
-	rc = exclusive_scan(h, pad1, bins1, start1); if (rc) return rc;
-	uint64_t padded_total = 0;
-	HIPCHK(h, hipMemcpy(&padded_total, start1 + bins1, 8, hipMemcpyDeviceToHost));
-	rc = scratch(std::max(padded_total, wn)); if (rc) return rc;
-	hipLaunchKernelGGL(bb_cursor_init_kernel, dim3(grid_for(bins1)), dim3(256), 0, h->stream, (const uint64_t *)start1, bins1, cursor);
-	hipLaunchKernelGGL(bb_scatter_kernel<W>, dim3(scatter_grid(wslots)), dim3(BB_THREADS), 0, h->stream, in1, shift1, bits1, h->hkb, nb, cursor, h->ue2.get<uint64_t>());
-	BbInput in2; in2.entries = h->ue2.get<uint64_t>(); in2.seg_start = start1; in2.seg_count = hist1; in2.n_seg = (uint32_t)bins1; in2.n_slots = padded_total; in2.holes = 0;
+		hipLaunchKernelGGL(bb_scatter_kernel<W>, dim3(bb_scatter_grid<W>(h, wslots)), dim3(BB_THREADS), 0, h->stream, in1, shift1, bits1, h->hkb, nb, cursor, h->ue2.get<uint64_t>(), (uint64_t)0, (uint64_t)0, (uint32_t *)nullptr, 0u);
+		in2.entries = h->ue2.get<uint64_t>(); in2.seg_start = start1; in2.seg_count = hist1; in2.n_seg = (uint32_t)bins1; in2.n_slots = padded_total; in2.holes = 0; in2.seg_cursor = nullptr; in2.seg_cap = 0;
+	} else {
+		in2.entries = h->ue2.get<uint64_t>(); in2.seg_start = nullptr; in2.seg_count = nullptr; in2.n_seg = (uint32_t)bins1; in2.n_slots = bins1 * p.cap1; in2.holes = 0; in2.seg_cursor = p.cursor1; in2.seg_cap = p.cap1;
+		out2 = p.out2;
+	}
 	const uint32_t shift2 = g;
 	HIPCHK(h, hipMemsetAsync(hist2, 0, 4 * groups, h->stream)); HIPCHK(h, hipMemsetAsync(dmax, 0, 4, h->stream));
-	grid = hist_grid(padded_total, tpb);
+	grid = hist_grid(in2.n_slots, tpb);
 	hipLaunchKernelGGL(bb_hist_kernel<W>, dim3(grid), dim3(BB_THREADS), 0, h->stream, in2, shift2, bits2, h->hkb, nb, tpb, hist2);
 	hipLaunchKernelGGL(bb_pad_kernel, dim3(grid_for(groups)), dim3(256), 0, h->stream, (const uint32_t *)hist2, groups, (uint32_t *)nullptr, dmax);
 	HIPCHK(h, hipMemcpyAsync(&mx, dmax, 4, hipMemcpyDeviceToHost, h->stream));
 	rc = exclusive_scan(h, hist2, groups, gstart); if (rc) return rc;
-	if (mx > bb_group_cap<W>() || packed_entries(h, h->ue) < wn) return 0;
+	if (mx > group_limit || (!last_only && packed_entries(h, h->ue) < wn)) return 0;
 	hipLaunchKernelGGL(bb_cursor_init_kernel, dim3(grid_for(groups)), dim3(256), 0, h->stream, (const uint64_t *)gstart, groups, cursor);
-	hipLaunchKernelGGL(bb_scatter_kernel<W>, dim3(scatter_grid(padded_total)), dim3(BB_THREADS), 0, h->stream, in2, shift2, bits2, h->hkb, nb, cursor, h->ue.get<uint64_t>());
-	rc = group_launch(h->ue.get<uint64_t>(), gstart, hist2); if (rc) return rc;
+	hipLaunchKernelGGL(bb_scatter_kernel<W>, dim3(bb_scatter_grid<W>(h, in2.n_slots)), dim3(BB_THREADS), 0, h->stream, in2, shift2, bits2, h->hkb, nb, cursor, out2, (uint64_t)0, (uint64_t)0, (uint32_t *)nullptr, 0u);
+	rc = bb_group_launch<W>(h, p, out2, gstart, hist2, 0, nullptr); if (rc) return rc;
 	done = true;
 	return 0;
 }
@@ -1296,53 +1389,78 @@
 	sm.nb = h->nb_sing; sm.n = keepSing ? sn : 0; sm.present = keepSing;
 	int rc = wm.start.reserve(h, "weak map start", 8 * (wm.nb + 1)); if (rc) return rc;
 	rc = sm.start.reserve(h, "singleton map start", 8 * (sm.nb + 1)); if (rc) return rc;
-	bool weakDone = false;
-	if (weak_uncounted) {
-		rc = binned_buckets_t<W>(h, wslots, wn, weakDone); if (rc) return rc;
-		if (!weakDone) {
-			if (key_entries(h, h->uw_keys) < wslots || !h->uw_vals) {
+	bool weakDone = false, bbQueued = false;
+	BbPlan bb;
+	auto weak_by_sort = [&](const uint64_t *packed, uint64_t slots) -> int {
+		if (weak_uncounted) {
+			if (key_entries(h, h->uw_keys) < slots || !h->uw_vals) {
 				h->uw_keys.reset(); h->uw_vals.reset();
-				const uint64_t cap = std::max<uint64_t>(wslots, 16);
+				const uint64_t cap = std::max<uint64_t>(slots, 16);
 				HIPCHK(h, h->uw_keys.alloc(8ull * W * cap)); HIPCHK(h, h->uw_vals.alloc(12ull * cap));
 			}
 			HIPCHK(h, hipMemsetAsync(wc, 0, 4 * wm.nb, h->stream));
-			if (wslots) hipLaunchKernelGGL(bb_unpack_kernel<W>, dim3(grid_for(wslots)), dim3(256), 0, h->stream, (const uint64_t *)h->ue.get<uint64_t>(), wslots, h->hkb, wm.nb, (uint64_t *)h->uw_keys.get(), (uint32_t *)h->uw_vals.get(), wc);
+			if (slots) hipLaunchKernelGGL(bb_unpack_kernel<W>, dim3(grid_for(slots)), dim3(256), 0, h->stream, packed, slots, h->hkb, wm.nb, (uint64_t *)h->uw_keys.get(), (uint32_t *)h->uw_vals.get(), wc);
 			HIPCHK(h, hipGetLastError());
 		}
-	}
-	if (!weakDone) { rc = exclusive_scan(h, wc, wm.nb, wm.start.get<uint64_t>()); if (rc) return rc; }
+		int rc2 = exclusive_scan(h, wc, wm.nb, wm.start.get<uint64_t>()); if (rc2) return rc2;
+		rc2 = wm.keys.reserve(h, "weak map keys", std::max<uint64_t>(8ull * W * wm.n, 8)); if (rc2) return rc2;
+		rc2 = wm.vals.reserve(h, "weak map vals", std::max<uint64_t>(4ull * vw * wm.n, 8)); if (rc2) return rc2;
+		HIPCHK(h, hipMemsetAsync(wc, 0, 4 * wm.nb, h->stream));
+		if (wm.n && vw > 4) hipLaunchKernelGGL((entry_scatter_kernel<W, true>), dim3(grid_for(slots)), dim3(256), 0, h->stream, (const uint64_t *)h->uw_keys.get(), (const uint32_t *)h->uw_vals.get(),
+		                            (const uint8_t *)nullptr, (const uint32_t *)nullptr, slots, vw, h->hkb, wm.nb, wm.start.get<uint64_t>(), wc, wm.keys.get<uint64_t>(), wm.vals.get<uint32_t>(), (uint8_t *)nullptr, (uint32_t *)nullptr);
+		else if (wm.n) {
+			unsigned long long *cur64 = nullptr;
+			if (h->superkmer_mode && arena_get(h, &cur64, wm.nb) == 0) HIPCHK(h, hipMemcpyAsync(cur64, wm.start.get<uint64_t>(), 8 * wm.nb, hipMemcpyDeviceToDevice, h->stream));
+			else cur64 = nullptr;
+			hipLaunchKernelGGL(entry_scatter_kernel<W>, dim3(grid_for(slots)), dim3(256), 0, h->stream, (const uint64_t *)h->uw_keys.get(), (const uint32_t *)h->uw_vals.get(),
+			                            (const uint8_t *)nullptr, (const uint32_t *)nullptr, slots, vw, h->hkb, wm.nb, wm.start.get<uint64_t>(), wc, wm.keys.get<uint64_t>(), wm.vals.get<uint32_t>(), (uint8_t *)nullptr, (uint32_t *)nullptr, cur64, 6);
+		}
+		HIPCHK(h, hipGetLastError());
+		SortView<W> sv; sv.keys = wm.keys.get<uint64_t>(); sv.vals = wm.vals.get<uint32_t>(); sv.b8 = nullptr; sv.pkt = nullptr; sv.vw = vw;
+		if (h->ext) hipLaunchKernelGGL((sort_buckets_kernel<W, 15>), dim3(grid_for(wm.nb, 4, 1 << 20)), dim3(256), 0, h->stream, sv, wm.start.get<uint64_t>(), wm.nb);
+		else hipLaunchKernelGGL((sort_buckets_kernel<W, 3>), dim3(grid_for(wm.nb, 4, 1 << 20)), dim3(256), 0, h->stream, sv, wm.start.get<uint64_t>(), wm.nb);
+		HIPCHK(h, hipGetLastError());
+		return 0;
+	};
+	h->last_bucket_path = BB_PATH_SORT;
+	if (weak_uncounted && bb_plan(h, wslots, wn, bb)) {
+		rc = bb_by_regions<W>(h, bb, bbQueued); if (rc) return rc;
+		if (bbQueued) { weakDone = true; h->last_bucket_path = BB_PATH_REGIONS; }
+		else { rc = bb_by_histograms<W>(h, bb, false, weakDone); if (rc) return rc; if (weakDone) h->last_bucket_path = BB_PATH_HISTOGRAMS; }
+	}
+	if (!weakDone) { rc = weak_by_sort(h->ue.get<uint64_t>(), wslots); if (rc) return rc; }
 	if (keepSing) { rc = exclusive_scan(h, sc, sm.nb, sm.start.get<uint64_t>()); if (rc) return rc; }
 	else HIPCHK(h, hipMemsetAsync(sm.start.get<uint64_t>(), 0, 8 * (sm.nb + 1), h->stream));
-	if (!weakDone) {
-		rc = wm.keys.reserve(h, "weak map keys", std::max<uint64_t>(8ull * W * wm.n, 8)); if (rc) return rc;
-		rc = wm.vals.reserve(h, "weak map vals", std::max<uint64_t>(4ull * vw * wm.n, 8)); if (rc) return rc;
-	}
 	rc = sm.keys.reserve(h, "singleton map keys", std::max<uint64_t>(8ull * W * sm.n, 8)); if (rc) return rc;
 	rc = sm.sweight.reserve(h, "singleton map sweight", std::max<uint64_t>(sm.n, 8)); if (rc) return rc;
 	if (h->ext) { rc = sm.spkt.reserve(h, "singleton map spkt", std::max<uint64_t>(4 * sm.n, 8)); if (rc) return rc; }
-	HIPCHK(h, hipMemsetAsync(wc, 0, 4 * wm.nb, h->stream)); HIPCHK(h, hipMemsetAsync(sc, 0, 4 * sm.nb, h->stream));
-	if (weakDone) {  }
-	else if (wm.n && vw > 4) hipLaunchKernelGGL((entry_scatter_kernel<W, true>), dim3(grid_for(wslots)), dim3(256), 0, h->stream, (const uint64_t *)h->uw_keys.get(), (const uint32_t *)h->uw_vals.get(),
-	                            (const uint8_t *)nullptr, (const uint32_t *)nullptr, wslots, vw, h->hkb, wm.nb, wm.start.get<uint64_t>(), wc, wm.keys.get<uint64_t>(), wm.vals.get<uint32_t>(), (uint8_t *)nullptr, (uint32_t *)nullptr);
-	else if (wm.n) {
-		unsigned long long *cur64 = nullptr;
-		if (h->superkmer_mode && arena_get(h, &cur64, wm.nb) == 0) HIPCHK(h, hipMemcpyAsync(cur64, wm.start.get<uint64_t>(), 8 * wm.nb, hipMemcpyDeviceToDevice, h->stream));
-		else cur64 = nullptr;
-		hipLaunchKernelGGL(entry_scatter_kernel<W>, dim3(grid_for(wslots)), dim3(256), 0, h->stream, (const uint64_t *)h->uw_keys.get(), (const uint32_t *)h->uw_vals.get(),
-		                            (const uint8_t *)nullptr, (const uint32_t *)nullptr, wslots, vw, h->hkb, wm.nb, wm.start.get<uint64_t>(), wc, wm.keys.get<uint64_t>(), wm.vals.get<uint32_t>(), (uint8_t *)nullptr, (uint32_t *)nullptr, cur64, 6);
-	}
+	if (weakDone) HIPCHK(h, hipMemsetAsync(wc, 0, 4 * wm.nb, h->stream));
+	HIPCHK(h, hipMemsetAsync(sc, 0, 4 * sm.nb, h->stream));
 	if (sm.n) hipLaunchKernelGGL(entry_scatter_kernel<W>, dim3(grid_for(sslots)), dim3(256), 0, h->stream, (const uint64_t *)h->us_keys.get(), (const uint32_t *)nullptr,
 	                            (const uint8_t *)h->us_b8.get(), (const uint32_t *)h->us_pkt.get(), sslots, 0u, h->hkb, sm.nb, sm.start.get<uint64_t>(), sc, sm.keys.get<uint64_t>(), (uint32_t *)nullptr, sm.sweight.get<uint8_t>(), h->ext ? sm.spkt.get<uint32_t>() : (uint32_t *)nullptr);
 	HIPCHK(h, hipGetLastError());
-	SortView<W> sv; sv.keys = wm.keys.get<uint64_t>(); sv.vals = wm.vals.get<uint32_t>(); sv.b8 = nullptr; sv.pkt = nullptr; sv.vw = vw;
-	if (weakDone) {  }
-	else if (h->ext) hipLaunchKernelGGL((sort_buckets_kernel<W, 15>), dim3(grid_for(wm.nb, 4, 1 << 20)), dim3(256), 0, h->stream, sv, wm.start.get<uint64_t>(), wm.nb);
-	else hipLaunchKernelGGL((sort_buckets_kernel<W, 3>), dim3(grid_for(wm.nb, 4, 1 << 20)), dim3(256), 0, h->stream, sv, wm.start.get<uint64_t>(), wm.nb);
 	if (sm.n) {
 		SortView<W> ss; ss.keys = sm.keys.get<uint64_t>(); ss.vals = nullptr; ss.b8 = sm.sweight.get<uint8_t>(); ss.pkt = h->ext ? sm.spkt.get<uint32_t>() : nullptr; ss.vw = 0;
 		hipLaunchKernelGGL((sort_buckets_kernel<W, 0>), dim3(grid_for(sm.nb, 4, 1 << 20)), dim3(256), 0, h->stream, ss, sm.start.get<uint64_t>(), sm.nb);
 	}
 	HIPCHK(h, hipGetLastError());
+	uint32_t ovf = 0;
+	if (bbQueued) HIPCHK(h, hipMemcpyAsync(&ovf, bb.ovf, 4, hipMemcpyDeviceToHost, h->stream));
+	HIPCHK(h, hipStreamSynchronize(h->stream));
+	if (!ovf) return 0;
+	const bool last_only = bb.bits2 != 0 && !(ovf & BB_OVF_L1);
+	h->last_bucket_path = bb_redo_path(bb.bits2 != 0, ovf);
+	if (dbg()) fprintf(stderr, "bucket partition: a region overflowed (%u), redoing %s by histograms\n", ovf, last_only ? "the second level" : "the partition");
+	rc = bb_by_histograms<W>(h, bb, last_only, weakDone); if (rc) return rc;
+	if (!weakDone) {
+		h->last_bucket_path = BB_PATH_SORT;
+		const uint64_t *src = h->ue.get<uint64_t>(); uint64_t slots = wslots;
+		if (last_only) {
+			src = h->ue2.get<uint64_t>(); slots = bb.bins1 * bb.cap1;
+			hipLaunchKernelGGL(bb_region_holes_kernel, dim3(grid_for(slots)), dim3(256), 0, h->stream, h->ue2.get<uint64_t>(), (uint32_t)(W + 1), (const unsigned long long *)bb.cursor1, bb.bins1, bb.cap1);
+		}
+		rc = weak_by_sort(src, slots); if (rc) return rc;
+	}
 	HIPCHK(h, hipStreamSynchronize(h->stream));
 	return 0;
 }
@@ -2189,6 +2307,9 @@
 	else if (k == "twobit_piece_bases") h->tune.twobit_piece_bases = (uint64_t)value;
 	else if (k == "exchange_fail_once") h->tune.exchange_fail_once = value != 0;
 	else if (k == "binned_buckets_min") h->tune.binned_min = value >= 0 ? (uint64_t)value : ~0ull;
+	else if (k == "bb_margin_l1") h->tune.bb_margin_l1 = std::min(std::max(value, 0.0), 8.0);
+	else if (k == "bb_margin_l2") h->tune.bb_margin_l2 = std::min(std::max(value, 0.0), 8.0);
+	else if (k == "bb_group_limit") h->tune.bb_group_limit = value >= 1 ? (uint32_t)value : 0;
 	else if (k == "coarse_lists") h->tune.no_coarse_lists = value == 0;
 	else if (k == "select_timing") h->tune.select_timing = value != 0;
 	else if (k == "dump_timing") h->tune.dump_timing = value != 0;
@@ -2215,6 +2336,7 @@
 	else if (k == "uniform_count") *value = h->last_count_uniform ? 1.0 : 0.0;
 	else if (k == "chunk_pool_chunks") *value = (double)h->l1.cap;
 	else if (k == "superkmer_window") *value = (double)h->sk_win;
+	else if (k == "bucket_path") *value = (double)h->last_bucket_path;
 	else if (k == "early_lists") *value = (double)h->last_early_hi;
 	else if (k == "early_entries") *value = (double)h->last_early_entries;
 	else if (k == "early_overflowed") *value = h->last_early_overflowed ? 1.0 : 0.0;
@@ -2429,6 +2551,7 @@
 	hipSetDevice(h->device);
 	{ int src_ = sync_state(h); if (src_) return src_; }
 	h->subtract = nullptr;
+	h->last_bucket_path = 0;
 	if (h->superkmer_mode) return finalize_superkmer(h, min_depth);
 	if (h->partition_mode) return finalize_partition(h, min_depth);
 	return with_w_ext(h, [&](auto W, auto EXT) { return finalize_t<W(), EXT()>(h, min_depth); });
diff --git a/kmernator_amd/csrc/kmr_buckets.hpp b/kmernator_amd/csrc/kmr_buckets.hpp
--- a/kmernator_amd/csrc/kmr_buckets.hpp
+++ b/kmernator_amd/csrc/kmr_buckets.hpp
@@ -25,6 +25,8 @@
 	uint32_t n_seg;
 	uint64_t n_slots;
 	uint32_t holes;
+	const unsigned long long *seg_cursor;
+	uint64_t seg_cap;
 };
 
 template <int W> __device__ __forceinline__ void bb_load_entry(const uint64_t *entries, uint64_t e, uint64_t (&w)[W + 1]) {
@@ -43,10 +45,15 @@
 }
 
 __device__ __forceinline__ uint32_t bb_segment_of(const BbInput &in, uint64_t s0) {
+	if (in.seg_cursor) return (uint32_t)(s0 / in.seg_cap);
 	if (!in.seg_start) return 0;
 	uint32_t lo = 0, hi = in.n_seg;
 	while (hi - lo > 1) { const uint32_t mid = (lo + hi) >> 1; if (in.seg_start[mid] <= s0) lo = mid; else hi = mid; }
 	return lo;
+}
+__device__ __forceinline__ uint64_t bb_segment_end(const BbInput &in, uint32_t seg) {
+	if (in.seg_cursor) { const uint64_t c = in.seg_cursor[seg], lim = (uint64_t)(seg + 1) * in.seg_cap; return c < lim ? c : lim; }
+	return in.seg_start ? in.seg_start[seg] + in.seg_count[seg] : in.n_slots;
 }
 
 template <int W>
@@ -73,7 +80,7 @@
 			}
 			curSeg = seg;
 		}
-		const uint64_t segEnd = in.seg_start ? in.seg_start[seg] + in.seg_count[seg] : in.n_slots;
+		const uint64_t segEnd = bb_segment_end(in, seg);
 #pragma unroll 4
 		for (int i = 0; i < BB_PER_THREAD; i++) {
 			const uint64_t e = s0 + (uint64_t)i * BB_THREADS + t;
@@ -103,53 +110,90 @@
 	for (int o = 32; o > 0; o >>= 1) { const unsigned int x = (unsigned int)__shfl_xor((int)m, o, 64); m = x > m ? x : m; }
 	if ((threadIdx.x & 63) == 0 && m) atomicMax(max_count, m);
 }
+__global__ void bb_region_init_kernel(uint64_t n, uint64_t cap, unsigned long long *cursor) {
+	for (uint64_t i = blockIdx.x * (uint64_t)blockDim.x + threadIdx.x; i < n; i += (uint64_t)gridDim.x * blockDim.x) cursor[i] = i * cap;
+}
+__global__ void bb_region_count_kernel(const unsigned long long *cursor, uint64_t n, uint64_t cap, uint32_t *count, const uint32_t *ovf) {
+	if (*ovf) return;
+	for (uint64_t i = blockIdx.x * (uint64_t)blockDim.x + threadIdx.x; i < n; i += (uint64_t)gridDim.x * blockDim.x) count[i] = (uint32_t)(cursor[i] - i * cap);
+}
+__global__ void bb_region_holes_kernel(uint64_t *entries, uint32_t words, const unsigned long long *cursor, uint64_t n, uint64_t cap) {
+	for (uint64_t e = blockIdx.x * (uint64_t)blockDim.x + threadIdx.x; e < n * cap; e += (uint64_t)gridDim.x * blockDim.x)
+		if (e >= cursor[e / cap]) entries[e * words + words - 1] = 0;
+}
 __global__ void bb_cursor_init_kernel(const uint64_t *start, uint64_t n, unsigned long long *cursor) {
 	for (uint64_t i = blockIdx.x * (uint64_t)blockDim.x + threadIdx.x; i < n; i += (uint64_t)gridDim.x * blockDim.x) cursor[i] = start[i];
 }
 #endif
 
+template <int W> __host__ __device__ constexpr int bb_scatter_per_thread() { return W == 2 ? BB_PER_THREAD / 2 : BB_PER_THREAD; }
+template <int W> __host__ __device__ constexpr int bb_scatter_step() { return bb_scatter_per_thread<W>() * BB_THREADS; }
+
 template <int W>
-__global__ __launch_bounds__(BB_THREADS)
-void bb_scatter_kernel(BbInput in, uint32_t shift, uint32_t bits, uint32_t kb, uint64_t nb, unsigned long long *cursor, uint64_t *out_entries) {
+__global__ __launch_bounds__(BB_THREADS, 4)
+void bb_scatter_kernel(BbInput in, uint32_t shift, uint32_t bits, uint32_t kb, uint64_t nb, unsigned long long *cursor, uint64_t *out_entries,
+                       uint64_t region_cap, uint64_t region_room, uint32_t *ovf, uint32_t ovf_bit) {
+	constexpr int PT = bb_scatter_per_thread<W>();
+	constexpr int STEP = bb_scatter_step<W>();
+	constexpr bool HOLD = W <= 2;
 	__shared__ uint32_t lh[1 << BB_MAX_BITS];
 	__shared__ unsigned long long lbase[1 << BB_MAX_BITS];
-	__shared__ uint32_t s_seg;
+	__shared__ uint32_t s_seg, s_ovf;
 	const int t = threadIdx.x;
+	if (t == 0) s_ovf = ovf ? *ovf : 0u;
+	__syncthreads();
+	if (s_ovf) return;
 	const uint32_t bins = 1u << bits, mask = bins - 1;
-	const uint64_t n_tiles = (in.n_slots + BB_TILE - 1) / BB_TILE;
+	const uint64_t n_tiles = (in.n_slots + STEP - 1) / STEP;
 	for (uint64_t tile = blockIdx.x; tile < n_tiles; tile += gridDim.x) {
-		const uint64_t s0 = tile * BB_TILE;
+		const uint64_t s0 = tile * STEP;
 		__syncthreads();
 		if (t == 0) s_seg = bb_segment_of(in, s0);
 		for (uint32_t i = t; i < bins; i += BB_THREADS) lh[i] = 0;
 		__syncthreads();
 		const uint32_t seg = s_seg;
-		const uint64_t segEnd = in.seg_start ? in.seg_start[seg] + in.seg_count[seg] : in.n_slots;
-		uint32_t where[BB_PER_THREAD];
-#pragma unroll
-		for (int i = 0; i < BB_PER_THREAD; i++) {
+		const uint64_t segEnd = bb_segment_end(in, seg);
+		if (s0 >= segEnd) continue;
+		uint64_t ew[HOLD ? PT : 1][W + 1];
+		if constexpr (HOLD) {
+#pragma unroll
+			for (int i = 0; i < PT; i++) {
+				const uint64_t e = s0 + (uint64_t)i * BB_THREADS + t;
+				bb_load_entry<W>(in.entries, e < segEnd ? e : segEnd - 1, ew[i]);
+			}
+		}
+		uint32_t where[PT];
+#pragma unroll
+		for (int i = 0; i < PT; i++) {
 			const uint64_t e = s0 + (uint64_t)i * BB_THREADS + t;
 			where[i] = 0xffffffffu;
 			if (e >= segEnd) continue;
-			uint64_t ew[W + 1];
-			bb_load_entry<W>(in.entries, e, ew);
-			if (in.holes && ew[W] == 0) continue;
+			if constexpr (!HOLD) bb_load_entry<W>(in.entries, e, ew[0]);
+			const uint64_t (&w)[W + 1] = ew[HOLD ? i : 0];
+			if (in.holes && w[W] == 0) continue;
 			Key<W> key;
 #pragma unroll
-			for (int q = 0; q < W; q++) key.w[q] = ew[q];
+			for (int q = 0; q < W; q++) key.w[q] = w[q];
 			const uint32_t bin = (uint32_t)((key_hash<W>(key, kb) & (nb - 1)) >> shift) & mask;
 			where[i] = (bin << 16) | atomicAdd(&lh[bin], 1u);
 		}
 		__syncthreads();
-		for (uint32_t i = t; i < bins; i += BB_THREADS) { const uint32_t c = lh[i]; if (c) lbase[i] = atomicAdd(&cursor[((uint64_t)seg << bits) + i], (unsigned long long)c); }
-		__syncthreads();
-#pragma unroll
-		for (int i = 0; i < BB_PER_THREAD; i++) {
+		for (uint32_t i = t; i < bins; i += BB_THREADS) {
+			const uint32_t c = lh[i];
+			if (!c) continue;
+			const uint64_t r = ((uint64_t)seg << bits) + i;
+			unsigned long long base = atomicAdd(&cursor[r], (unsigned long long)c);
+			if (region_cap && base + c > r * region_cap + region_room) { base = ~0ull; atomicOr(ovf, ovf_bit); }
+			lbase[i] = base;
+		}
+		__syncthreads();
+#pragma unroll
+		for (int i = 0; i < PT; i++) {
 			if (where[i] == 0xffffffffu) continue;
-			const uint64_t e = s0 + (uint64_t)i * BB_THREADS + t;
-			uint64_t ew[W + 1];
-			bb_load_entry<W>(in.entries, e, ew);
-			bb_store_entry<W>(out_entries, lbase[where[i] >> 16] + (where[i] & 0xffffu), ew);
+			const unsigned long long base = lbase[where[i] >> 16];
+			if (base == ~0ull) continue;
+			if constexpr (!HOLD) bb_load_entry<W>(in.entries, s0 + (uint64_t)i * BB_THREADS + t, ew[0]);
+			bb_store_entry<W>(out_entries, base + (where[i] & 0xffffu), ew[HOLD ? i : 0]);
 		}
 	}
 }
@@ -160,7 +204,11 @@
 template <int W>
 __global__ __launch_bounds__(BB_GROUP_THREADS, W <= 2 ? 4 : 1)
 void bb_group_kernel(const uint64_t *entries, uint64_t *keys, uint32_t *vals, const uint64_t *gstart, const uint32_t *gcount, uint64_t n_groups, uint32_t gbits, uint32_t kb, uint64_t nb,
-                     uint64_t *start, uint64_t n_total, uint32_t *err) {
+                     uint64_t *start, uint64_t n_total, uint32_t *err, uint64_t in_stride, const uint32_t *ovf) {
+	__shared__ uint32_t s_ovf;
+	if (threadIdx.x == 0) s_ovf = ovf ? *ovf : 0u;
+	__syncthreads();
+	if (s_ovf) return;
 	extern __shared__ __attribute__((aligned(16))) uint8_t gsm[];
 	uint64_t *skeys = (uint64_t *)gsm;
 	constexpr uint32_t CAP = bb_group_cap<W>();
@@ -171,7 +219,7 @@
 	const int t = threadIdx.x;
 	const uint32_t nbk = 1u << gbits;
 	for (uint64_t G = blockIdx.x; G < n_groups; G += gridDim.x) {
-		const uint64_t base = gstart[G];
+		const uint64_t base = gstart[G], in_base = in_stride ? G * in_stride : base;
 		const uint32_t n = gcount[G];
 		__syncthreads();
 		if ((uint32_t)t < nbk) bcnt[t] = 0;
@@ -182,7 +230,7 @@
 		for (int u = 0; u < BB_GROUP_PER_THREAD; u++) {
 			const uint32_t i = (uint32_t)u * BB_GROUP_THREADS + t;
 			lb[u] = 0xffffffffu;
-			if (i < n) bb_load_entry<W>(entries, base + i, ew[u]);
+			if (i < n) bb_load_entry<W>(entries, in_base + i, ew[u]);
 		}
 #pragma unroll
 		for (int u = 0; u < BB_GROUP_PER_THREAD; u++) {
```

Result: faster. 58.57 billion, median of 6 (+5.0%).
